# Stardust-lf/fhe-reliability-gpu

Measured on AMD Instinct MI355X. Metric: forward negacyclic NTT/s at N=2^16 (limb-polynomials per second), higher is better.
Workload: dtype f64

## Files before the change

fhe_reliability_gpu_amd/csrc/capi.cpp:

```cpp
#include "capi_internal.hpp"

int build_tables(fhe_ctx *ctx, int log_n, const u64 *q, int count, const u64 *fwd_rows, bool want_inverse, int force_path,
                 const u64 *psi_or_null, fhe_ntt_tables **out, const u64 *gs_scale)
{
    if (!ctx || !q || !out || count < 1 || log_n < 1 || log_n > NTT_MAX_LOGN) return fail(FHE_ERR_INVALID, "bad table arguments");
    const size_t N = (size_t)1 << log_n;
    std::unique_ptr<fhe_ntt_tables> t(new fhe_ntt_tables);
    t->ctx = ctx;
    t->log_n = log_n;
    t->count = count;
    t->q.assign(q, q + count);
    t->psi.assign(count, 0);
    t->path.resize(count);
    t->h_lp.resize(count);
    t->has_inverse = want_inverse;
    std::vector<Tw> tw((size_t)count * 2 * N);
    HIP_TRY(hipSetDevice(ctx->device));
    HIP_TRY(t->d_tw.alloc(tw.size() * sizeof(Tw)));
    std::vector<u64> inv;
    for (int l = 0; l < count; l++) {
        const int path = force_path >= 0 ? force_path : path_for(q[l]);
        if (path < 0 || (path == PATH_F64 && q[l] >= ((u64)1 << 50)) || q[l] >= ((u64)1 << 61) || q[l] < 2)
            return fail(FHE_ERR_UNSUPPORTED, "modulus must satisfy 2 <= q < 2^61 (FP64 path: q < 2^50)");
        t->path[l] = path;
        const u64 *row = fwd_rows + (size_t)l * N;
        Tw *f = tw.data() + (size_t)l * 2 * N, *b = f + N;
        for (size_t k = 0; k < N; k++) f[tw_stored_index(log_n, (u32)k)] = encode(path, row[k] % q[l], q[l]);
        bool inv_ok = false;
        if (gs_scale) {
            const u64 sc = gs_scale[l] % q[l];
            for (size_t k = 1; k < N; k++) b[tw_stored_index(log_n, (u32)k)] = encode(path, row[k] % q[l], q[l]);
            b[tw_stored_index(log_n, 0)] = encode(path, host::mul_mod(sc, row[1 % N] % q[l], q[l]), q[l]);
        } else if (want_inverse) inv_ok = batch_inverse(row, N, q[l], inv);
        if (gs_scale) {
        } else if (inv_ok) {
            inv[0] = host::mul_mod(host::inv_mod((u64)(N % q[l]), q[l]), inv[1 % N], q[l]);
            for (size_t k = 0; k < N; k++) b[tw_stored_index(log_n, (u32)k)] = encode(path, inv[k], q[l]);
        } else {
            for (size_t k = 0; k < N; k++) b[k] = f[k];
            t->has_inverse = false;
        }
        LimbParams &p = t->h_lp[l];
        std::memset(&p, 0, sizeof p);
        p.q = q[l];
        p.two_q = 2 * q[l];
        p.n = (double)q[l];
        p.ninv = 1.0 / p.n;
        const u64 ninv = gs_scale ? gs_scale[l] % q[l] : host::inv_mod((u64)(N % q[l]), q[l]);
        if (!ninv && want_inverse) t->has_inverse = false;
        p.inv_n = encode(path, ninv, q[l]);
        p.fwd = t->d_tw.as<Tw>() + (size_t)l * 2 * N;
        p.inv = p.fwd + N;
        u64 cr[3];
        host::const_ratio(q[l], cr);
        p.barrett_lo = cr[0];
        p.barrett_hi = cr[1];
        p.path = path;
        if (psi_or_null) t->psi[l] = psi_or_null[l];
    }
    HIP_TRY(hipMemcpy(t->d_tw.p, tw.data(), tw.size() * sizeof(Tw), hipMemcpyHostToDevice));
    HIP_TRY(t->d_lp.upload(t->h_lp));
    *out = t.release();
    return FHE_OK;
}

SubBatchCut sub_batch_cut(const fhe_ctx *ctx, int log_n, size_t n_poly, size_t len, size_t bufs)
{
    const size_t unit_bytes = ((size_t)8 << log_n) * bufs, total = n_poly * len * unit_bytes, chunk_bytes = ((size_t)ctx->chunk_mib << 20) * (bufs > 1 ? 2 : 1);
    const size_t floor_bytes = ((size_t)ctx->chunk_floor_mib << 20) * (bufs > 1 ? 3 : 1);
    if (!chunk_bytes || log_n < 13 || n_poly * len < 2 || total <= std::max(chunk_bytes + (chunk_bytes >> 1), floor_bytes)) return SubBatchCut{0, 0};
    const size_t pc = std::min(n_poly, std::max<size_t>(1, chunk_bytes / unit_bytes));
    const size_t lc = std::min(len, std::max<size_t>(1, chunk_bytes / (unit_bytes * pc)));
    if (pc == n_poly && lc == len) return SubBatchCut{0, 0};
    return SubBatchCut{pc, lc};
}
size_t sub_batch_polys(const fhe_ctx *ctx, int log_n, size_t n_poly, size_t len)
{
    const size_t unit_bytes = (size_t)8 << log_n, total = n_poly * len * unit_bytes, chunk_bytes = (size_t)ctx->chunk_mib << 20;
    if (!chunk_bytes || log_n < 13 || n_poly < 2 || total <= std::max(chunk_bytes + (chunk_bytes >> 1), (size_t)ctx->chunk_floor_mib << 20)) return 0;
    const size_t per = std::max<size_t>(1, chunk_bytes / (unit_bytes * len));
    return per < n_poly ? per : 0;
}

hipError_t handoff_scratch(fhe_ctx *ctx, hipStream_t st, size_t bytes, u64 **out)
{
    DevBuf *b;
    {
        std::lock_guard<std::mutex> lock(ctx->mu);
        auto &slot = ctx->pp_tmp[st];
        if (!slot) slot.reset(new DevBuf);
        b = slot.get();
    }
    *out = nullptr;
    if (b->bytes < bytes) {
        hipStreamCaptureStatus cap = hipStreamCaptureStatusNone;
        (void)hipStreamIsCapturing(st, &cap);
        if (cap != hipStreamCaptureStatusNone) return hipSuccess;
        hipError_t e = b->p ? hipStreamSynchronize(st) : hipSuccess;
        if (e == hipSuccess) e = b->alloc(bytes);
        if (e != hipSuccess) return e;
    }
    *out = b->as<u64>();
    return hipSuccess;
}

int side_stream(fhe_ctx *ctx, hipStream_t st, fhe_ctx::Side **out)
{
    *out = nullptr;
    hipStreamCaptureStatus cap = hipStreamCaptureStatusNone;
    if (hipStreamIsCapturing(st, &cap) != hipSuccess || cap != hipStreamCaptureStatusNone) return FHE_OK;
    fhe_ctx::Side *sd;
    {
        std::lock_guard<std::mutex> lock(ctx->mu);
        auto &slot = ctx->side[st];
        if (!slot) slot.reset(new fhe_ctx::Side);
        sd = slot.get();
    }
    if (!sd->s) {
        HIP_TRY(hipStreamCreateWithFlags(&sd->s, hipStreamNonBlocking));
        HIP_TRY(hipEventCreateWithFlags(&sd->fork, hipEventDisableTiming));
        HIP_TRY(hipEventCreateWithFlags(&sd->join, hipEventDisableTiming));
    }
    *out = sd;
    return FHE_OK;
}

int for_pieces(fhe_ctx *ctx, hipStream_t st, size_t n_pieces, size_t side_tmp_bytes, const std::function<hipError_t(hipStream_t, size_t, u64 *)> &fn)
{
    fhe_ctx::Side *sd = nullptr;
    hipStreamCaptureStatus cap = hipStreamCaptureStatusNone;
    if (ctx->split && n_pieces > 1 && hipStreamIsCapturing(st, &cap) == hipSuccess && cap == hipStreamCaptureStatusNone) {
        {
            std::lock_guard<std::mutex> lock(ctx->mu);
            auto &slot = ctx->side[st];
            if (!slot) slot.reset(new fhe_ctx::Side);
            sd = slot.get();
        }
        if (!sd->s) {
            HIP_TRY(hipStreamCreateWithFlags(&sd->s, hipStreamNonBlocking));
            HIP_TRY(hipEventCreateWithFlags(&sd->fork, hipEventDisableTiming));
            HIP_TRY(hipEventCreateWithFlags(&sd->join, hipEventDisableTiming));
        }
        if (sd->tmp.bytes < side_tmp_bytes) {
            HIP_TRY(hipStreamSynchronize(sd->s));
            HIP_TRY(sd->tmp.alloc(side_tmp_bytes));
        }
        HIP_TRY(hipEventRecord(sd->fork, st));
        HIP_TRY(hipStreamWaitEvent(sd->s, sd->fork, 0));
    }
    hipError_t e = hipSuccess;
    for (size_t i = 0; i < n_pieces && e == hipSuccess; ++i) {
        const bool on_side = sd && (i & 1);
        e = fn(on_side ? sd->s : st, i, on_side && side_tmp_bytes ? sd->tmp.as<u64>() : nullptr);
    }
    if (sd) {
        HIP_TRY(hipEventRecord(sd->join, sd->s));
        HIP_TRY(hipStreamWaitEvent(st, sd->join, 0));
    }
    return e == hipSuccess ? FHE_OK : hip_fail(e, "sub-batch launch");
}
int for_sub_batches(fhe_ctx *ctx, hipStream_t st, size_t n_poly, size_t per, size_t side_tmp_bytes,
                    const std::function<hipError_t(hipStream_t, size_t, size_t, u64 *)> &fn)
{
    return for_pieces(ctx, st, (n_poly + per - 1) / per, side_tmp_bytes,
                      [&](hipStream_t s, size_t i, u64 *side_tmp) { return fn(s, i * per, std::min(per, n_poly - i * per), side_tmp); });
}

int ntt_batch(fhe_ctx *ctx, u64 *d, const fhe_ntt_tables *t, size_t n_poly, size_t limbs, size_t start_idx, void *stream,
              bool inverse, const u64 *d_src, u32 galois, u64 *d_galois_copy)
{
    if (!ctx || !d) return fail(FHE_ERR_INVALID, "null argument");
    if (galois) {
        if (!inverse || !d_src || d_src == d || !(galois & 1)) return fail(FHE_ERR_INVALID, "the Galois map rides on an out-of-place inverse transform");
        if (ctx->mode == 1 || ctx->fault_idx >= 0 || ctx->packed_on || ctx->only_pass >= 0 || ctx->resident || t->log_n < 5) {
            HIP_TRY(hipSetDevice(ctx->device));
            u64 *to = d_galois_copy ? d_galois_copy : d;
            hipError_t e = launch_automorphism_ntt(pick(ctx, stream), to, d_src, (u32)(n_poly * limbs), t->log_n, galois);
            if (e != hipSuccess) return hip_fail(e, "launch_automorphism_ntt");
            d_src = d_galois_copy;
            galois = 0;
            d_galois_copy = nullptr;
        }
    }
    if (d_src && (ctx->mode == 1 || ctx->fault_idx >= 0 || ctx->packed_on || ctx->only_pass >= 0 || ctx->resident)) {
        HIP_TRY(hipSetDevice(ctx->device));
        if (d_src != d) HIP_TRY(hipMemcpyAsync(d, d_src, (n_poly * limbs << t->log_n) * 8, hipMemcpyDeviceToDevice, pick(ctx, stream)));
        d_src = nullptr;
    }
    int rc = check_range(t, n_poly, limbs, start_idx);
    if (rc) return rc;
    if (inverse && !t->has_inverse) return fail(FHE_ERR_UNSUPPORTED, "table set has no inverse (twiddle or N not invertible)");
    if (!n_poly || !limbs) return FHE_OK;
    HIP_TRY(hipSetDevice(ctx->device));
    hipStream_t st = pick(ctx, stream);
    const size_t N = (size_t)1 << t->log_n;
    TraceScope tr(ctx, st, "NTT");
    return for_each_run(t, limbs, start_idx, [&](size_t off, size_t len, int path) -> int {
        PassArgs a{d + off * N, t->d_lp.as<LimbParams>(), (u32)(start_idx + off), (u32)len, (u32)(n_poly * len), (u32)limbs};
        if (d_src) a.src = d_src + off * N;
        a.galois = galois;
        if (d_galois_copy) a.galois_copy = d_galois_copy + off * N;
        hipError_t e;
        if (ctx->mode == 1 && fused_supported(t->log_n)) {
            DevBuf *ctl;
            {
                std::lock_guard<std::mutex> lock(ctx->mu);
                auto &slot = ctx->fused_ctl[st];
                if (!slot) slot.reset(new DevBuf);
                ctl = slot.get();
            }
            const size_t need = fused_ctl_bytes(a.units);
            if (ctl->bytes < need) {
                HIP_TRY(hipStreamSynchronize(st));
                u32 carried = 0;
                if (ctl->p) HIP_TRY(hipMemcpy(&carried, ctl->as<u32>() + fused_error_word(), sizeof carried, hipMemcpyDeviceToHost));
                HIP_TRY(ctl->alloc(need * 2));
                HIP_TRY(hipMemset(ctl->p, 0, need * 2));
                if (carried) HIP_TRY(hipMemcpy(ctl->as<u32>() + fused_error_word(), &carried, sizeof carried, hipMemcpyHostToDevice));
            }
            e = launch_ntt_fused(st, a, t->log_n, inverse, path, ctl->as<u32>(), ctx->fused_dist, ctx->fused_wgs, ctx->fused_variant, ctx->fused_skip_teams);
        } else if (ctx->fault_idx >= 0 && t->log_n >= 13) {
            e = launch_ntt(st, a, t->log_n, inverse, path, ctx->geo, 0);
            if (e == hipSuccess) e = launch_flip_bit(st, d, (u64)ctx->fault_idx, ctx->fault_bit);
            if (e == hipSuccess) e = launch_ntt(st, a, t->log_n, inverse, path, ctx->geo, 1);
            ctx->fault_idx = -1;
        } else {
            if (ctx->packed_on && ctx->only_pass < 0 && ctx->geo == 1 && ntt_packed_supported(t->log_n, inverse, path)) {
                DevBuf *sc;
                {
                    std::lock_guard<std::mutex> lock(ctx->mu);
                    auto &slot = ctx->packed[st];
                    if (!slot) slot.reset(new DevBuf);
                    sc = slot.get();
                }
                const size_t need = (size_t)a.units * ntt_packed_scratch_words() * 8;
                if (sc->bytes < need) {
                    HIP_TRY(hipStreamSynchronize(st));
                    HIP_TRY(sc->alloc(need));
                }
                a.scratch = sc->as<u64>();
            }
            const bool plain = t->log_n >= 13 && ctx->only_pass < 0 && !a.scratch;
            const SubBatchCut cut = plain ? sub_batch_cut(ctx, t->log_n, n_poly, len) : SubBatchCut{0, 0};
            u64 *pp = nullptr;
            const bool want_pp = !galois && (ctx->pingpong < 0 ? cut.pc != 0 : ctx->pingpong != 0);
            const size_t pp_bytes = (cut.pc ? cut.pc * cut.lc : n_poly * limbs) * N * 8;
            if (want_pp && plain) HIP_TRY(handoff_scratch(ctx, st, pp_bytes, &pp));
            if (cut.pc) {
                const size_t npp = (n_poly + cut.pc - 1) / cut.pc, npl = (len + cut.lc - 1) / cut.lc;
                return for_pieces(ctx, st, npp * npl, pp ? pp_bytes : 0, [&](hipStream_t s, size_t i, u64 *side_tmp) {
                    const size_t l0 = (i / npp) * cut.lc, p0 = (i % npp) * cut.pc;
                    const size_t lc = std::min(cut.lc, len - l0), pc = std::min(cut.pc, n_poly - p0);
                    PassArgs c = a;
                    c.data = a.data + (p0 * limbs + l0) * N;
                    if (a.src) c.src = a.src + (p0 * limbs + l0) * N;
                    if (a.galois_copy) c.galois_copy = a.galois_copy + (p0 * limbs + l0) * N;
                    c.limb0 = a.limb0 + (u32)l0;
                    c.limbs = (u32)lc;
                    c.units = (u32)(pc * lc);
                    c.tmp = side_tmp ? side_tmp : pp;
                    c.tmp_stride = (u32)lc;
                    c.stream_hint = ctx->stream_hint != 0;
                    return launch_ntt(s, c, t->log_n, inverse, path, ctx->geo, -1, false);
                });
            } else {
                a.tmp = pp ? pp + off * N : nullptr;
                const bool streams = t->log_n < 13 && t->log_n >= 5 && ctx->stream_hint < 0 && ctx->only_pass < 0 &&
                                     (size_t)a.units * N * 8 > ((size_t)ctx->chunk_floor_mib << 20);
                a.stream_hint = ctx->stream_hint > 0 || streams;
                e = launch_ntt(st, a, t->log_n, inverse, path, ctx->geo, ctx->only_pass, ctx->resident);
            }
        }
        if (e != hipSuccess) return hip_fail(e, "launch_ntt");
        return FHE_OK;
    });
}

int pointwise(fhe_ctx *ctx, u64 *c, const u64 *a, const u64 *b, const fhe_ntt_tables *t, size_t n_poly, size_t limbs,
              size_t start_idx, void *stream, bool acc)
{
    if (!ctx || !c || !a || !b) return fail(FHE_ERR_INVALID, "null argument");
    int rc = check_range(t, n_poly, limbs, start_idx);
    if (rc) return rc;
    HIP_TRY(hipSetDevice(ctx->device));
    PointwiseArgs p{c, a, b, t->d_lp.as<LimbParams>(), (u32)start_idx, (u32)limbs, (u32)(n_poly * limbs), (u32)limbs, t->log_n};
    hipError_t e = launch_modmul(pick(ctx, stream), p, acc);
    if (e != hipSuccess) return hip_fail(e, "launch_modmul");
    return FHE_OK;
}

int cyclic_tables(fhe_ctx *ctx, int log_n, u64 mod, u64 root, int convention, u64 scale, fhe_ntt_tables **out)
{
    std::lock_guard<std::mutex> lock(ctx->mu);
    auto key = std::make_tuple(log_n, mod, root, convention * 2 + 1, scale);
    auto it = ctx->cyclic.find(key);
    if (it == ctx->cyclic.end()) {
        const u64 n = (u64)1 << log_n;
        std::vector<u64> tw(n);
        host::cyclic_table(mod, log_n, root, convention == 1, tw.data());
        fhe_ntt_tables *nt = nullptr;
        int rc = build_tables(ctx, log_n, &mod, 1, tw.data(), false, -1, nullptr, &nt, &scale);
        if (rc) return rc;
        it = ctx->cyclic.emplace(key, std::unique_ptr<fhe_ntt_tables>(nt)).first;
    }
    *out = it->second.get();
    return FHE_OK;
}

static bool cyclic_tower(u64 mod, int log_n, u64 root, bool nth_root_convention)
{
    const u64 n = (u64)1 << log_n;
    u64 prev = 0;
    for (int s = 0; s < log_n; s++) {
        const u64 len = (u64)2 << s;
        const u64 w = nth_root_convention ? host::pow_mod(root, n / len, mod) : host::pow_mod(root, (mod - 1) / len, mod);
        if (s == 0 ? w != (mod - 1) % mod : host::mul_mod(w, w, mod) != prev) return false;
        prev = w;
    }
    return true;
}
static bool cyclic_tower_cached(fhe_ctx *ctx, u64 mod, int log_n, u64 root, int convention)
{
    std::lock_guard<std::mutex> lock(ctx->mu);
    const auto key = std::make_tuple(log_n, mod, root, convention);
    auto it = ctx->cyclic_tower.find(key);
    if (it == ctx->cyclic_tower.end()) it = ctx->cyclic_tower.emplace(key, cyclic_tower(mod, log_n, root, convention == 1)).first;
    return it->second;
}

static int cyclic_small(fhe_ctx *ctx, u64 *d_data, u64 *d_scratch, int log_n, size_t n_vec, u64 mod, u64 root, int convention, u64 scale, bool do_scale,
                        void *stream)
{
    fhe_ntt_tables *t = nullptr;
    {
        std::lock_guard<std::mutex> lock(ctx->mu);
        auto key = std::make_tuple(log_n, mod, root, convention * 2, (u64)0);
        auto it = ctx->cyclic.find(key);
        if (it == ctx->cyclic.end()) {
            std::vector<u64> tw((size_t)1 << log_n);
            host::cyclic_table(mod, log_n, root, convention == 1, tw.data());
            fhe_ntt_tables *nt = nullptr;
            int rc = build_tables(ctx, log_n, &mod, 1, tw.data(), false, -1, nullptr, &nt);
            if (rc) return rc;
            it = ctx->cyclic.emplace(key, std::unique_ptr<fhe_ntt_tables>(nt)).first;
        }
        t = it->second.get();
    }
    HIP_TRY(hipSetDevice(ctx->device));
    hipStream_t st = pick(ctx, stream);
    PassArgs a{d_data, t->d_lp.as<LimbParams>(), 0u, 1u, (u32)n_vec, 1u};
    hipError_t e = launch_ntt(st, a, log_n, false, t->path[0]);
    if (e != hipSuccess) return hip_fail(e, "launch_ntt(cyclic)");
    e = launch_bitrev_scale(st, d_scratch, d_data, log_n, (u32)n_vec, mod_const(mod), scale, do_scale);
    if (e != hipSuccess) return hip_fail(e, "launch_bitrev_scale");
    HIP_TRY(hipMemcpyAsync(d_data, d_scratch, (n_vec << log_n) * sizeof(u64), hipMemcpyDeviceToDevice, st));
    return FHE_OK;
}

extern "C" {

int fhe_version(void) { return 100; }
const char *fhe_last_error(void) { return g_err.c_str(); }

int fhe_ctx_create(int device, fhe_ctx **out)
{
    if (!out) return fail(FHE_ERR_INVALID, "null out");
    int n = 0;
    HIP_TRY(hipGetDeviceCount(&n));
    if (device < 0 || device >= n) return fail(FHE_ERR_INVALID, "no such HIP device");
    HIP_TRY(hipSetDevice(device));
    std::unique_ptr<fhe_ctx> c(new fhe_ctx);
    c->device = device;
    HIP_TRY(hipStreamCreateWithFlags(&c->stream, hipStreamNonBlocking));
    if (const char *m = getenv("FHE_NTT_MODE")) c->mode = std::strcmp(m, "fused") == 0 ? 1 : 0;
    if (const char *v = getenv("FHE_FUSED_DIST")) c->fused_dist = (unsigned)std::max(1, atoi(v));
    if (const char *v = getenv("FHE_FUSED_WGS")) c->fused_wgs = (unsigned)std::max(1, atoi(v));
    if (const char *v = getenv("FHE_NTT_RESIDENT")) c->resident = atoi(v) != 0;
    if (const char *v = getenv("FHE_NTT_PACKED")) c->packed_on = atoi(v) != 0;
    if (const char *v = getenv("FHE_NTT_PINGPONG")) c->pingpong = atoi(v) < 0 ? -1 : atoi(v) ? 1 : 0;
    if (const char *v = getenv("FHE_NTT_SPLIT")) c->split = atoi(v) < 0 ? -1 : atoi(v) ? 1 : 0;
    if (const char *v = getenv("FHE_NTT_CHUNK_MIB")) c->chunk_mib = (unsigned)std::max(0, atoi(v));
    if (const char *v = getenv("FHE_KS_FUSED")) c->ks_fused = atoi(v) < 0 ? -1 : atoi(v) ? 1 : 0;
    if (const char *v = getenv("FHE_HMULT_FUSED_RESCALE")) c->hmult_fused_rescale = atoi(v) != 0;
    *out = c.release();
    return FHE_OK;
}

int fhe_ctx_destroy(fhe_ctx *ctx)
{
    if (!ctx) return FHE_OK;
    (void)hipSetDevice(ctx->device);
    (void)hipStreamSynchronize(ctx->stream);
    ctx->cyclic.clear();
    ctx->garner.clear();
    ctx->fused_ctl.clear();
    ctx->packed.clear();
    ctx->pp_tmp.clear();
    for (auto &kv : ctx->side)
        if (kv.second && kv.second->s) {
            (void)hipStreamSynchronize(kv.second->s);
            (void)hipEventDestroy(kv.second->fork);
            (void)hipEventDestroy(kv.second->join);
            (void)hipStreamDestroy(kv.second->s);
        }
    ctx->side.clear();
    (void)hipStreamDestroy(ctx->stream);
    delete ctx;
    return FHE_OK;
}

int fhe_ctx_set_option(fhe_ctx *ctx, const char *name, long value)
{
    if (!ctx || !name) return fail(FHE_ERR_INVALID, "null argument");
    if (!std::strcmp(name, "ntt_mode")) ctx->mode = value ? 1 : 0;
    else if (!std::strcmp(name, "fused_dist")) ctx->fused_dist = (unsigned)std::max(1l, value);
    else if (!std::strcmp(name, "fused_wgs")) ctx->fused_wgs = (unsigned)std::max(1l, value);
    else if (!std::strcmp(name, "fused_variant")) ctx->fused_variant = (int)value;
    else if (!std::strcmp(name, "tile_geo")) ctx->geo = value ? 1 : 0;
    else if (!std::strcmp(name, "ntt_resident")) ctx->resident = value != 0;
    else if (!std::strcmp(name, "ntt_packed")) ctx->packed_on = value != 0;
    else if (!std::strcmp(name, "ntt_stream")) ctx->stream_hint = value < 0 ? -1 : value ? 1 : 0;
    else if (!std::strcmp(name, "ntt_chunk_floor_mib")) ctx->chunk_floor_mib = (unsigned)std::max(0l, value);
    else if (!std::strcmp(name, "ntt_split")) ctx->split = value < 0 ? -1 : value ? 1 : 0;
    else if (!std::strcmp(name, "ntt_pingpong")) ctx->pingpong = value < 0 ? -1 : value ? 1 : 0;
    else if (!std::strcmp(name, "ntt_chunk_mib")) ctx->chunk_mib = (unsigned)std::max(0l, value);
    else if (!std::strcmp(name, "ks_fused")) ctx->ks_fused = value < 0 ? -1 : value ? 1 : 0;
    else if (!std::strcmp(name, "hmult_fused_rescale")) ctx->hmult_fused_rescale = value != 0;
    else if (!std::strcmp(name, "ntt_only_pass")) ctx->only_pass = value == 0 ? 0 : value == 1 ? 1 : -1;
    else if (!std::strcmp(name, "fused_skip_teams")) ctx->fused_skip_teams = (unsigned)value;
    else return fail(FHE_ERR_INVALID, "unknown option");
    return FHE_OK;
}

int fhe_ctx_check(fhe_ctx *ctx)
{
    if (!ctx) return fail(FHE_ERR_INVALID, "null ctx");
    HIP_TRY(hipSetDevice(ctx->device));
    std::lock_guard<std::mutex> lock(ctx->mu);
    for (auto &kv : ctx->fused_ctl) {
        if (!kv.second || !kv.second->p) continue;
        HIP_TRY(hipStreamSynchronize(kv.first));
        u32 flag = 0;
        HIP_TRY(hipMemcpy(&flag, kv.second->as<u32>() + fused_error_word(), sizeof flag, hipMemcpyDeviceToHost));
        if (flag) {
            HIP_TRY(hipMemset(kv.second->as<u32>() + fused_error_word(), 0, sizeof flag));
            return fail(FHE_ERR_HIP, "fused NTT: a bounded wait ran out in a launch since the last check (its results are invalid)");
        }
    }
    return FHE_OK;
}

int fhe_ctx_stream(fhe_ctx *ctx, void **stream_out)
{
    if (!ctx || !stream_out) return fail(FHE_ERR_INVALID, "null argument");
    *stream_out = ctx->stream;
    return FHE_OK;
}

int fhe_sync(fhe_ctx *ctx, void *stream)
{
    if (!ctx) return fail(FHE_ERR_INVALID, "null ctx");
    HIP_TRY(hipSetDevice(ctx->device));
    HIP_TRY(hipStreamSynchronize(pick(ctx, stream)));
    return FHE_OK;
}

int fhe_alloc(fhe_ctx *ctx, size_t bytes, void **dptr)
{
    if (!ctx || !dptr) return fail(FHE_ERR_INVALID, "null argument");
    HIP_TRY(hipSetDevice(ctx->device));
    hipError_t e = hipMalloc(dptr, bytes ? bytes : 16);
    if (e == hipErrorOutOfMemory) return fail(FHE_ERR_NOMEM, "hipMalloc: out of device memory");
    if (e != hipSuccess) return hip_fail(e, "hipMalloc");
    return FHE_OK;
}

int fhe_free(fhe_ctx *ctx, void *dptr)
{
    if (!ctx) return fail(FHE_ERR_INVALID, "null ctx");
    if (!dptr) return FHE_OK;
    HIP_TRY(hipSetDevice(ctx->device));
    HIP_TRY(hipFree(dptr));
    return FHE_OK;
}

int fhe_h2d(fhe_ctx *ctx, void *dst, const void *src, size_t bytes, void *stream)
{
    if (!ctx || (!dst && bytes) || (!src && bytes)) return fail(FHE_ERR_INVALID, "null argument");
    HIP_TRY(hipSetDevice(ctx->device));
    HIP_TRY(hipMemcpyAsync(dst, src, bytes, hipMemcpyHostToDevice, pick(ctx, stream)));
    return FHE_OK;
}
int fhe_d2h(fhe_ctx *ctx, void *dst, const void *src, size_t bytes, void *stream)
{
    if (!ctx || (!dst && bytes) || (!src && bytes)) return fail(FHE_ERR_INVALID, "null argument");
    HIP_TRY(hipSetDevice(ctx->device));
    HIP_TRY(hipMemcpyAsync(dst, src, bytes, hipMemcpyDeviceToHost, pick(ctx, stream)));
    return FHE_OK;
}
int fhe_d2d(fhe_ctx *ctx, void *dst, const void *src, size_t bytes, void *stream)
{
    if (!ctx || (!dst && bytes) || (!src && bytes)) return fail(FHE_ERR_INVALID, "null argument");
    HIP_TRY(hipSetDevice(ctx->device));
    HIP_TRY(hipMemcpyAsync(dst, src, bytes, hipMemcpyDeviceToDevice, pick(ctx, stream)));
    return FHE_OK;
}
int fhe_memset(fhe_ctx *ctx, void *dst, int byte, size_t bytes, void *stream)
{
    if (!ctx || (!dst && bytes)) return fail(FHE_ERR_INVALID, "null argument");
    HIP_TRY(hipSetDevice(ctx->device));
    HIP_TRY(hipMemsetAsync(dst, byte, bytes, pick(ctx, stream)));
    return FHE_OK;
}

int fhe_moduli_create(uint64_t N, const int *bits, int count, uint64_t *out_q)
{
    if (!bits || !out_q || count < 1 || N < 1 || (N & (N - 1)) || N > ((u64)1 << 59)) return fail(FHE_ERR_INVALID, "bad arguments");
    for (int i = 0; i < count; i++)
        if (bits[i] < 2 || bits[i] > 61) return fail(FHE_ERR_UNSUPPORTED, "bit sizes must be in [2, 61]");
    if (!host::create_moduli(N, bits, count, out_q)) return fail(FHE_ERR_INVALID, "not enough primes of the requested size");
    return FHE_OK;
}

int fhe_modulus_const_ratio(uint64_t q, uint64_t out[3])
{
    if (q < 2 || !out) return fail(FHE_ERR_INVALID, "bad arguments");
    host::const_ratio(q, out);
    return FHE_OK;
}

int fhe_min_primitive_root(uint64_t q, uint64_t order, uint64_t *out)
{
    if (!out) return fail(FHE_ERR_INVALID, "null out");
    if (order > ((u64)1 << 31)) return fail(FHE_ERR_UNSUPPORTED, "order above 2^31");
    if (!host::min_primitive_root(q, order, *out)) return fail(FHE_ERR_INVALID, "no primitive root of that order");
    return FHE_OK;
}

int fhe_root_powers(uint64_t q, int log_n, uint64_t *rp, uint64_t *rp_shoup)
{
    if (log_n < 1 || log_n > 30 || q < 2) return fail(FHE_ERR_INVALID, "bad arguments");
    u64 psi;
    if (!host::min_primitive_root(q, (u64)2 << log_n, psi)) return fail(FHE_ERR_INVALID, "q is not 1 mod 2N (or not prime)");
    const size_t N = (size_t)1 << log_n;
    std::vector<u64> t(N);
    host::root_powers(q, log_n, psi, t.data());
    for (size_t k = 0; k < N; k++) {
        if (rp) rp[k] = t[k];
        if (rp_shoup) rp_shoup[k] = (u64)(((unsigned __int128)t[k] << 64) / q);
    }
    return FHE_OK;
}

int fhe_ntt_tables_create(fhe_ctx *ctx, int log_n, const uint64_t *q, int count, fhe_ntt_tables **out)
{
    if (!ctx || !q || !out || count < 1 || log_n < 1 || log_n > NTT_MAX_LOGN) return fail(FHE_ERR_INVALID, "bad table arguments");
    const size_t N = (size_t)1 << log_n;
    std::vector<u64> rows((size_t)count * N), psi(count);
    for (int l = 0; l < count; l++) {
        if (q[l] < 2 || q[l] >= ((u64)1 << 61)) return fail(FHE_ERR_UNSUPPORTED, "modulus " + std::to_string(q[l]) + " outside [2, 2^61)");
        if (!host::min_primitive_root(q[l], (u64)2 * N, psi[l]))
            return fail(FHE_ERR_INVALID, "modulus " + std::to_string(q[l]) + " has no primitive 2N-th root");
        host::root_powers(q[l], log_n, psi[l], rows.data() + (size_t)l * N);
    }
    return build_tables(ctx, log_n, q, count, rows.data(), true, -1, psi.data(), out);
}

int fhe_ntt_tables_create_from_roots(fhe_ctx *ctx, int log_n, const uint64_t *q, int count, const uint64_t *root_powers,
                                     int force_path, fhe_ntt_tables **out)
{
    if (!root_powers) return fail(FHE_ERR_INVALID, "null root powers");
    if (force_path < -1 || force_path > 1) return fail(FHE_ERR_INVALID, "bad force_path");
    std::vector<u64> psi(count > 0 ? count : 0);
    if (log_n >= 1 && count >= 1)
        for (int l = 0; l < count; l++) psi[l] = root_powers[((size_t)l << log_n) + ((size_t)1 << (log_n - 1))];
    return build_tables(ctx, log_n, q, count, root_powers, true, force_path, psi.data(), out);
}
// ... 327 lines not shown
```

fhe_reliability_gpu_amd/csrc/capi_internal.hpp:

```cpp
#pragma once
#include "../../include/fhe_mi355x.h"

#include <hip/hip_runtime.h>

#include <algorithm>
#include <chrono>
#include <cstdio>
#include <cstdlib>
#include <cstring>
#include <functional>
#include <map>
#include <memory>
#include <mutex>
#include <string>
#include <tuple>
#include <vector>

#include "host_math.hpp"
#include "ntt_fused.hpp"
#include "ntt_launch.hpp"

using namespace fhe;



inline thread_local std::string g_err;

inline int fail(int code, const std::string &msg)
{
    g_err = msg;
    return code;
}
inline int hip_fail(hipError_t e, const char *what)
{
    g_err = std::string(what) + ": " + hipGetErrorString(e);
    return FHE_ERR_HIP;
}
#define HIP_TRY(expr)                                          \
    do {                                                       \
        hipError_t e_ = (expr);                                \
        if (e_ != hipSuccess) return hip_fail(e_, #expr);      \
    } while (0)

struct DevBuf {
    void *p = nullptr;
    size_t bytes = 0;
    ~DevBuf()
    {
        if (p) (void)hipFree(p);
    }
    hipError_t alloc(size_t n)
    {
        if (p) (void)hipFree(p);
        p = nullptr;
        bytes = n;
        return hipMalloc(&p, n ? n : 16);
    }
    template <class T> hipError_t upload(const std::vector<T> &v)
    {
        hipError_t e = alloc(v.size() * sizeof(T));
        if (e != hipSuccess) return e;
        return hipMemcpy(p, v.data(), v.size() * sizeof(T), hipMemcpyHostToDevice);
    }
    template <class T> T *as() const { return static_cast<T *>(p); }
};

struct fhe_ntt_tables {
    fhe_ctx *ctx = nullptr;
    int log_n = 0, count = 0;
    std::vector<u64> q, psi;
    std::vector<int> path;
    std::vector<LimbParams> h_lp;
    DevBuf d_lp, d_tw;
    bool has_inverse = true;
};

struct fhe_baseconv {
    int m = 0, k = 0;
    bool fast_ok = true;
    DevBuf mod_in, mod_out, dig, hor, fp_in, fp_out, fast_coef, fast_shoup, img_head, img_out, rows_id;
    DevBuf chk_dig, chk_hor;
    const fhe::Tw *shoup_dig = nullptr, *shoup_hor = nullptr;
    BaseConvPlanDev dev{};
};

struct GarnerTables {
    DevBuf mod, ratio, pref_lo, pref_hi, inv_pref;
};

struct fhe_ctx {
    int device = 0;
    hipStream_t stream = nullptr;
    std::mutex mu;
    std::map<hipStream_t, std::unique_ptr<DevBuf>> fused_ctl;
    std::map<hipStream_t, std::unique_ptr<DevBuf>> packed;
    bool packed_on = false;
    int mode = 0;
    unsigned fused_dist = 4, fused_wgs = 768;
    bool hmult_fused_rescale = true;
    unsigned fused_skip_teams = 0;
    bool trace_on = false;
    std::string trace;
    long long fault_idx = -1;
    int fault_bit = 0;
    int pfault_pass = -1, pfault_bit = 0;
    u32 pfault_block = 0, pfault_word = 0;
    PointHook pm_fault, pw_fault, bc_fault, gal_fault;
    StagedFault ksc_fault, rsc_fault, hrc_fault, bsgs_fault, bgv_ksc_fault, bgv_rsc_fault;
    PointHook seal_fault;
    PointHook carry_fault;
    int carry_skip = 0;
    DevBuf seal_part;
    DevBuf gal_sums;
    int geo = 1;
    bool resident = false;
    int pingpong = -1;
    std::map<hipStream_t, std::unique_ptr<DevBuf>> pp_tmp;
    struct Side { hipStream_t s = nullptr; hipEvent_t fork = nullptr, join = nullptr; DevBuf tmp; };
    std::map<hipStream_t, std::unique_ptr<Side>> side;
    int split = -1;
    int stream_hint = -1;
    unsigned chunk_floor_mib = 192;
    unsigned chunk_mib = 96;
    int ks_fused = -1;
    int only_pass = -1;
    int fused_variant = 7;
    std::map<std::tuple<int, u64, u64, int, u64>, std::unique_ptr<fhe_ntt_tables>> cyclic;
    std::map<std::tuple<int, u64, u64, int>, bool> cyclic_tower;
    std::map<std::vector<u64>, std::unique_ptr<GarnerTables>> garner;
};

struct fhe_abft {
    fhe_ctx *ctx = nullptr;
    const fhe_ntt_tables *t = nullptr;
    DevBuf w, what, ninv;
    DevBuf win, wout, wout8;
    DevBuf sum_in, sum_out;
    DevBuf umid, umid8;
    DevBuf sum_mid1, sum_mid2;
    DevBuf psum;
};

struct KsShard {
    int world = 1, rank = 0, clo = 0, cn = 0, slo = 0, sn = 0, cmax = 0, smax = 0;
};
void ks_shard_layout(int L, int K, int world, int rank, KsShard *s);

struct fhe_keyswitch {
    fhe_ctx *ctx = nullptr;
    const fhe_ntt_tables *t = nullptr;
    int L = 0, K = 0, dnum = 0, alpha = 0, log_n = 0;
    KsShard sh;
    bool sharded = false;
    int m_own = 0;
    u64 *g1 = nullptr, *g2 = nullptr;
    DevBuf up_rows, down_rows;
    bool up_f64 = false;
    bool own_path[2] = {false, false};
    bool up_trivial = false;
    u32 down_src_row = 0, down_src_stride = 0;
    DevBuf d_t_mod_Q;
    u32 n_up_jobs = 0;
    std::vector<BcJob> up_host;
    u64 plain_modulus = 0;
    std::vector<u64> t_inv_P, t_mod_Q;
    std::vector<fhe_baseconv *> up;
    fhe_baseconv *down = nullptr;
    DevBuf pinv;
    DevBuf coef, ext, acc, conv, rot;
    DevBuf up_jobs, down_jobs;
    int up_max_m = 0, up_max_k = 0;
    u32 up_m_mask = 0;
    bool up_batched = false;
    DevBuf ext_map[2];
    u32 ext_units[2] = {0, 0};
    fhe_baseconv *last = nullptr;
    int rs_n = 0;
    bool own_last = false;
    u64 *rs_bc = nullptr;
    DevBuf qlast_inv;
    DevBuf rs_last, rs_delta, rs_jobs;
    DevBuf hm, hm_pre;
    DevBuf pq_tw;
    DevBuf bsgs;
    DevBuf acc2, conv2, hsp2, hdown_jobs2;
    int cur = 0;
    DevBuf acc_multi;
    u64 *acc_ovr = nullptr;
    u64 *acc_cur() const { return acc_ovr ? acc_ovr : (cur ? acc2 : acc).as<u64>(); }
    u64 *conv_cur() const { return (cur ? conv2 : conv).as<u64>(); }
    u64 *hsp_cur() const { return (cur ? hsp2 : hsp).as<u64>(); }
    DevBuf hsp, hdown_rows, hdown_jobs;
    u64 t_inv_qlast = 0;
    DevBuf chk_bc_flags, chk_bc_map, chk_sum_in, chk_sum_out;
    ~fhe_keyswitch()
    {
        for (auto *b : up) fhe_baseconv_destroy(b);
        fhe_baseconv_destroy(down);
        fhe_baseconv_destroy(last);
    }
};

struct fhe_fourstep {
    fhe_ctx *ctx = nullptr;
    u64 n1 = 0, n2 = 0, mod = 0, g = 0;
    int log_n = 0;
    fhe_ntt_tables *t = nullptr;
    DevBuf tmp;
    bool big = false;
    int log1 = 0, log2 = 0, lo_bits = 0;
    DevBuf tw_lo, tw_hi, buf0, buf1;
    struct Checked {
        DevBuf u8, m8, v8, eu, em, ev, sums[4];
        std::unique_ptr<fhe_ntt_tables> small;
    };
    std::unique_ptr<Checked> chk;
    bool checked_ready = false;
};



inline hipStream_t pick(fhe_ctx *ctx, void *stream) { return stream ? static_cast<hipStream_t>(stream) : ctx->stream; }

inline int path_for(u64 q)
{
    if (q < 2) return -1;
    if (q < ((u64)1 << 50)) return PATH_F64;
    if (q < ((u64)1 << 61)) return PATH_U64;
    return -1;
}

inline Tw encode(int path, u64 w, u64 q) { return path == PATH_F64 ? ArithF64::encode(w, q) : ArithU64::encode(w, q); }

inline bool batch_inverse(const u64 *t, size_t n, u64 q, std::vector<u64> &out)
{
    out.assign(n, 0);
    if (n < 2) return true;
    std::vector<u64> pre(n);
    u64 acc = 1 % q;
    for (size_t i = 1; i < n; i++) {
        pre[i] = acc;
        acc = host::mul_mod(acc, t[i] % q, q);
    }
    u64 inv = host::inv_mod(acc, q);
    if (!inv && q != 1) return false;
    for (size_t i = n - 1; i >= 1; i--) {
        out[i] = host::mul_mod(inv, pre[i], q);
        inv = host::mul_mod(inv, t[i] % q, q);
    }
    return true;
}



template <class F> int for_each_run(const fhe_ntt_tables *t, size_t limbs, size_t start_idx, F f)
{
    size_t i = 0;
    while (i < limbs) {
        size_t j = i + 1;
        while (j < limbs && t->path[start_idx + j] == t->path[start_idx + i]) j++;
        int rc = f(i, j - i, t->path[start_idx + i]);
        if (rc != FHE_OK) return rc;
        i = j;
    }
    return FHE_OK;
}

struct TraceScope {
    fhe_ctx *ctx;
    hipStream_t st;
// ... 81 lines not shown
```

fhe_reliability_gpu_amd/csrc/fourstep_checked.hip:

```cpp
#include "ntt_launch.hpp"
#include "ntt_plan.hpp"
#include "abft_taps.hpp"

namespace fhe {

template <class PASS>
FHE_D void gs_lds_fault(const GsCheckArgs &g, int pass, typename PASS::elem *lds)
{
    if (g.fault_pass == pass && g.fault_block == blockIdx.x) {
        if (threadIdx.x == 0) reinterpret_cast<u64 *>(lds)[g.fault_word % (u32)PASS::LDS_ELEMS] ^= (u64)1 << g.fault_bit;
        __syncthreads();
    }
}

template <class PASS, int LOGN, bool WA, bool WB>
__global__ __launch_bounds__(NTT_THREADS) void k_gs_first_checked(PassArgs a, GsCheckArgs g)
{
    typedef typename PASS::Arith A;
    typedef GsTap<A, 0, PASS::P, PASS::S0, WA, WB> Tap;
    static_assert(PASS::NPHASE >= 3, "a staging phase and at least two register steps");
    __shared__ __attribute__((aligned(16))) typename PASS::elem lds[PASS::LDS_ELEMS];
    __shared__ u64 red[2][NTT_THREADS / 64];
    const u32 unit = blockIdx.x / PASS::TILES, tile = blockIdx.x % PASS::TILES;
    const size_t off = (size_t)unit << LOGN;
    const LimbParams &p = a.lp[a.limb0];
    const typename A::Ctx ctx = A::make_ctx(p);
    const TwPtr tw = as_global(p.inv);
    const Tw inv_n = p.inv_n;
    const int tid = threadIdx.x;
    const u32 row0 = tile * PASS::TROWS;
    u64 *base = a.data + off;
    const u64 *from = a.src + off;
    Tap tap{as_global(g.u), as_global(g.m), as_global(g.v), (const u64 FHE_GLOBAL *)g.u8, (const u64 FHE_GLOBAL *)g.m8, row0, g.logp,
            typename A::elem(0), typename A::elem(0), 0, 0};
    PASS::template phase<0>(tid, base, lds, tw, row0, ctx, inv_n, &tap, from, 0u, nullptr, a.stream_hint != 0);
    __syncthreads();
    PASS::template phase<1>(tid, base, lds, tw, row0, ctx, inv_n, &tap);
    __syncthreads();
    gs_lds_fault<PASS>(g, 0, lds);
    PASS::template phase<2>(tid, base, lds, tw, row0, ctx, inv_n, &tap);
    if constexpr (PASS::NPHASE > 3) {
        __syncthreads();
        PASS::template phase<3>(tid, base, lds, tw, row0, ctx, inv_n, &tap);
    }
    if constexpr (WA) block_sum_mod(A::canonical(tap.acc_a, ctx), p.q, g.sum_a + (size_t)unit * PASS::TILES + tile, red[0]);
    if constexpr (WB) block_sum_mod(A::canonical(tap.acc_b, ctx), p.q, g.sum_b + (size_t)unit * PASS::TILES + tile, red[1]);
}

template <class PASS, int LOGN, int P, bool WA, bool WB>
__global__ __launch_bounds__(NTT_THREADS) void k_gs_second_checked(PassArgs a, GsCheckArgs g)
{
    typedef typename PASS::Arith A;
    typedef GsTap<A, 1, P, LOGN - P, WA, WB> Tap;
    static_assert(PASS::NPHASE == 2 || PASS::NPHASE == 3, "two or three register steps");
    __shared__ __attribute__((aligned(16))) typename PASS::elem lds[PASS::LDS_ELEMS];
    __shared__ u64 red[2][NTT_THREADS / 64];
    u32 limb;
    u64 *base = col_tile<PASS, LOGN>(blockIdx.x, a, limb);
    const u32 unit = blockIdx.x / PASS::TILES, tile = blockIdx.x % PASS::TILES;
    const u32 pos0 = (u32)((base - a.data) & (((size_t)1 << LOGN) - 1));
    const LimbParams &p = a.lp[limb];
    const typename A::Ctx ctx = A::make_ctx(p);
    const TwPtr tw = as_global(p.inv);
    const Tw inv_n = p.inv_n;
    const int tid = threadIdx.x;
    const u64 *from = a.src + (base - a.data);
    Tap tap{as_global(g.u), as_global(g.m), as_global(g.v), (const u64 FHE_GLOBAL *)g.u8, (const u64 FHE_GLOBAL *)g.m8, pos0, g.logp,
            typename A::elem(0), typename A::elem(0), 0, 0};
    PASS::template phase<0>(tid, base, lds, tw, 0u, ctx, inv_n, &tap, from);
    __syncthreads();
    gs_lds_fault<PASS>(g, 1, lds);
    PASS::template phase<1>(tid, base, lds, tw, 0u, ctx, inv_n, &tap);
    if constexpr (PASS::NPHASE > 2) {
        __syncthreads();
        PASS::template phase<2>(tid, base, lds, tw, 0u, ctx, inv_n, &tap);
    }
    if constexpr (WA) block_sum_mod(A::canonical(tap.acc_a, ctx), p.q, g.sum_a + (size_t)unit * PASS::TILES + tile, red[0]);
    if constexpr (WB) block_sum_mod(A::canonical(tap.acc_b, ctx), p.q, g.sum_b + (size_t)unit * PASS::TILES + tile, red[1]);
}

template <class A, int LOGN>
static hipError_t launch_gs_checked_t(hipStream_t st, const PassArgs &a, u64 *tmp, const GsCheckArgs &c1, const GsCheckArgs &c2, bool phases, int which)
{
    typedef GsPasses<A, LOGN> GP;
    typedef typename GP::First First;
    const dim3 g1(a.units * First::TILES), th(NTT_THREADS);
    if constexpr (!GP::TWO) {
        if (which == 1) return hipSuccess;
        hipLaunchKernelGGL((k_gs_first_checked<First, LOGN, true, true>), g1, th, 0, st, a, c1);
        return hipGetLastError();
    } else {
        if (!tmp) return hipErrorInvalidValue;
        constexpr int P = First::P;
        typedef typename GP::Second Col;
        typedef typename GP::SecondNt ColNt;
        PassArgs first = a, second = a;
        first.data = tmp;
        second.src = tmp;
        const dim3 g2(a.units * Col::TILES);
        if (which != 1) {
            if (phases) hipLaunchKernelGGL((k_gs_first_checked<First, LOGN, true, true>), g1, th, 0, st, first, c1);
            else hipLaunchKernelGGL((k_gs_first_checked<First, LOGN, true, false>), g1, th, 0, st, first, c1);
        }
        if (which != 0) {
            if (a.stream_hint) {
                if (phases) hipLaunchKernelGGL((k_gs_second_checked<ColNt, LOGN, P, true, true>), g2, th, 0, st, second, c2);
                else hipLaunchKernelGGL((k_gs_second_checked<ColNt, LOGN, P, false, true>), g2, th, 0, st, second, c2);
            } else {
                if (phases) hipLaunchKernelGGL((k_gs_second_checked<Col, LOGN, P, true, true>), g2, th, 0, st, second, c2);
                else hipLaunchKernelGGL((k_gs_second_checked<Col, LOGN, P, false, true>), g2, th, 0, st, second, c2);
            }
        }
        return hipGetLastError();
    }
}

template <int LOGN> static void gs_checked_tiles_t(u32 *t1, u32 *t2)
{
    typedef GsPasses<ArithF64, LOGN> GP;
    *t1 = GP::First::TILES;
    if constexpr (GP::TWO) *t2 = GP::Second::TILES;
    else *t2 = 1;
}

void ntt_gs_checked_tiles(int logn, u32 *t1, u32 *t2)
{
    *t1 = *t2 = 1;
    switch (logn) {
#define FHE_CASE(L) case L: gs_checked_tiles_t<L>(t1, t2); break;
        FHE_CASE(5) FHE_CASE(6) FHE_CASE(7) FHE_CASE(8) FHE_CASE(9) FHE_CASE(10) FHE_CASE(11) FHE_CASE(12) FHE_CASE(13)
        FHE_CASE(14) FHE_CASE(15) FHE_CASE(16) FHE_CASE(17) FHE_CASE(18) FHE_CASE(19) FHE_CASE(20)
#undef FHE_CASE
    default: break;
    }
}

hipError_t launch_ntt_gs_checked(hipStream_t st, const PassArgs &a, u64 *tmp, const GsCheckArgs &c1, const GsCheckArgs &c2, int logn, int path,
                                 bool phases, int which)
{
    if (a.units == 0) return hipSuccess;
    if (!a.src || a.map || a.limbs != 1 || !ntt_gs_supported(logn) || (phases && logn < 13)) return hipErrorInvalidValue;
    switch (logn) {
#define FHE_CASE(L) \
    case L: return path == PATH_F64 ? launch_gs_checked_t<ArithF64, L>(st, a, tmp, c1, c2, phases, which) : launch_gs_checked_t<ArithU64, L>(st, a, tmp, c1, c2, phases, which);
        FHE_CASE(5) FHE_CASE(6) FHE_CASE(7) FHE_CASE(8) FHE_CASE(9) FHE_CASE(10) FHE_CASE(11) FHE_CASE(12) FHE_CASE(13)
        FHE_CASE(14) FHE_CASE(15) FHE_CASE(16) FHE_CASE(17) FHE_CASE(18) FHE_CASE(19) FHE_CASE(20)
#undef FHE_CASE
    default: return hipErrorInvalidValue;
    }
}

}
```

fhe_reliability_gpu_amd/csrc/ntt_core.hpp:

```cpp
#pragma once
#include "modarith.hpp"

namespace fhe {

FHE_HD u32 brev_bits(u32 v, int bits)
{
    if (bits <= 0) return 0;
#if defined(__clang__)
    return __builtin_bitreverse32(v) >> (32 - bits);
#else
    u32 r = 0;
    for (int b = 0; b < bits; b++) r |= ((v >> b) & 1u) << (bits - 1 - b);
    return r;
#endif
}

FHE_HD constexpr int cmax(int a, int b) { return a > b ? a : b; }
FHE_HD constexpr int cmin(int a, int b) { return a < b ? a : b; }

FHE_HD constexpr u32 reduce_mask(int stage0, int nstages, int first, int next)
{
    u32 mask = 0;
    for (int u = 0; u < nstages; u++) {
        int s = stage0 + u;
// ... 82 lines not shown
{
    constexpr int R = 1 << K;
    InvLazyPlan<K> p{};
    int b[R] = {};
    for (int r = 0; r < R; r++) b[r] = in8 * 128;
    const int limit = INV_LAZY_LIMIT8 * 128, folded = 513;
    for (int v = 0; v < K; v++) {
        const int u = K - 1 - v, half = R >> (u + 1);
        u32 m = 0;
        for (int blk = 0; blk < (1 << u); blk++)
            for (int j = 0; j < half; j++) {
                const int i0 = blk * 2 * half + j, i1 = i0 + half;
                if (b[i0] + b[i1] > limit) {
                    const int big = b[i0] >= b[i1] ? i0 : i1;
                    b[big] = folded;
                    m |= 1u << big;
                    if (b[i0] + b[i1] > limit) {
                        const int other = big == i0 ? i1 : i0;
                        b[other] = folded;
                        m |= 1u << other;
                    }
                }
                const int sum = b[i0] + b[i1], prod = 513 + (sum + 3) / 4;
                b[i0] = (fold_last && u == 0) ? prod : sum;
                b[i1] = prod;
            }
        p.before[v] = m;
    }
    int mx = 0;
    for (int r = 0; r < R; r++) {
        if (b[r] > exit8 * 128) {
            b[r] = folded;
            p.at_exit |= 1u << r;
        }
        mx = b[r] > mx ? b[r] : mx;
    }
    p.out8 = (mx + 127) / 128;
    return p;
}
template <class ST> FHE_HD constexpr int inv_lazy_step_in8(int in8, int se)
{
    int b = in8;
    for (int i = 0; i < se; i++) {
        const int k = ST::k(ST::NSTEP - 1 - i);
        b = k == 1 ? inv_lazy_plan<1>(b, INV_LAZY_EXIT8, false).out8 : k == 2 ? inv_lazy_plan<2>(b, INV_LAZY_EXIT8, false).out8
          : k == 3 ? inv_lazy_plan<3>(b, INV_LAZY_EXIT8, false).out8 : k == 4 ? inv_lazy_plan<4>(b, INV_LAZY_EXIT8, false).out8
                                                                             : inv_lazy_plan<5>(b, INV_LAZY_EXIT8, false).out8;
    }
    return b;
}
template <class ST> FHE_HD constexpr int inv_lazy_pass_out8(int in8) { return inv_lazy_step_in8<ST>(in8, ST::NSTEP); }

template <class A, int K, int SBLK, bool FOLD, int IN8, int EXIT8>
FHE_D void radix_inv_lazy(typename A::elem (&x)[1 << K], TwPtr tw, int s, u32 prefix, const typename A::Ctx &c, const Tw *inv_n)
{
    constexpr int R = 1 << K;
    constexpr InvLazyPlan<K> plan = inv_lazy_plan<K>(IN8, EXIT8, FOLD);
#pragma unroll
    for (int v = 0; v < K; v++) {
        const int u = K - 1 - v;
#pragma unroll
        for (int r = 0; r < R; r++)
            if ((plan.before[v] >> r) & 1) A::reduce(x[r], c);
        const int half = R >> (u + 1);
        if (FOLD && u == 0) {
            const Tw wn = tw[0];
#pragma unroll
            for (int j = 0; j < half; j++) A::bfly_inv_scaled(x[j], x[j + half], *inv_n, wn, c);
            continue;
        }
#pragma unroll
        for (int b = 0; b < (1 << u); b++) {
            const Tw w = tw[tw_index(SBLK, s + u, (prefix << u) + b)];
#pragma unroll
            for (int j = 0; j < half; j++) A::bfly_inv(x[b * 2 * half + j], x[b * 2 * half + j + half], w, c);
        }
    }
#pragma unroll
    for (int r = 0; r < R; r++)
        if ((plan.at_exit >> r) & 1) A::reduce(x[r], c);
}

template <int K0_, int K1_, int K2_>
struct Steps {
    static constexpr int K0 = K0_, K1 = K1_, K2 = K2_;
    static constexpr int P = K0_ + K1_ + K2_;
    static constexpr int NSTEP = (K0_ > 0) + (K1_ > 0) + (K2_ > 0);
    static constexpr int KMAX = cmax(K0_, cmax(K1_, K2_));
    FHE_HD static constexpr int k(int e) { return e == 0 ? K0_ : e == 1 ? K1_ : K2_; }
    FHE_HD static constexpr int done(int e) { return e == 0 ? 0 : e == 1 ? K0_ : K0_ + K1_; }
};

enum IoMode { IO_CANONICAL = 0, IO_LAZY = 1 };

template <class A, int R, int IN_MODE>
FHE_D void convert_in(typename A::elem (&x)[R], u64 (&raw)[R], const typename A::Ctx &c)
{
    if (IN_MODE == IO_LAZY) {
#pragma unroll
        for (int r = 0; r < R; r++) x[r] = A::load_lazy(raw[r]);
    } else {
        bool bad = false;
#pragma unroll
        for (int r = 0; r < R; r++) bad |= !A::in_range(raw[r], c);
        if (__builtin_expect(bad, 0)) {
#pragma unroll
            for (int r = 0; r < R; r++) raw[r] = A::in_range(raw[r], c) ? raw[r] : reduce_any_u64(raw[r], c.q);
        }
#pragma unroll
        for (int r = 0; r < R; r++) x[r] = A::from_canonical(raw[r]);
    }
}

template <class A, int OUT_MODE, bool INVERSE, bool SCALED = false>
FHE_D u64 convert_out(typename A::elem x, const typename A::Ctx &c, const Tw &inv_n)
{
    if (OUT_MODE == IO_LAZY) return A::store_lazy(x);
    if (INVERSE && !SCALED) return A::canonical(A::mulmod(x, inv_n, c), c);
    return A::canonical(x, c);
}

constexpr int PK_BITS = 50;
constexpr int PK_WORDS = 13;
constexpr int PK_BLOCK_WORDS = 16 * PK_WORDS;
constexpr u64 PK_MASK = ((u64)1 << PK_BITS) - 1;

FHE_HD void pk_pack(const u64 (&v)[16], u64 (&w)[PK_WORDS])
{
#pragma unroll
    for (int j = 0; j < PK_WORDS; j++) w[j] = 0;
#pragma unroll
    for (int k = 0; k < 16; k++) {
        const int j = (PK_BITS * k) >> 6, t = (PK_BITS * k) & 63;
        w[j] |= v[k] << t;
        if (t > 64 - PK_BITS) w[j + 1] |= v[k] >> (64 - t);
    }
}
template <class P> FHE_HD u64 pk_extract(P w, u32 idx)
{
    const u32 bit = PK_BITS * idx, j = bit >> 6, t = bit & 63;
    const u64 lo = w[j], hi = w[j + 1 < PK_WORDS ? j + 1 : j];
    const u64 v = t > 64 - PK_BITS ? (lo >> t) | (hi << (64 - t)) : lo >> t;
    return v & PK_MASK;
}

template <class T, class = void> struct tap_preloads { static constexpr bool value = false; };
template <class T> struct tap_preloads<T, decltype((void)T::PRELOAD)> { static constexpr bool value = T::PRELOAD; };
struct NoTap {
    static constexpr bool ACTIVE = false;
    static constexpr bool MID = false;
    static constexpr bool STORES = false;
};

template <class A, class ST, int LOGN, int S0, int TC, int NTHREADS, bool INVERSE, int IN_MODE, int OUT_MODE, u32 RED,
          int SBLK, int COHERENT_IN = 0, bool STREAM = false>
struct ColPass {
    typedef A Arith;
    typedef typename A::elem elem;
    static constexpr int THREADS = NTHREADS;
    static constexpr int P = ST::P;
    static constexpr int NPTS = 1 << P;
    static constexpr int LOGSTRIDE = LOGN - S0 - P;
    static constexpr u32 STRIDE = 1u << LOGSTRIDE;
    static constexpr int PADC = (TC < 32 && (NPTS * TC + ((NPTS + 15) / 16) * TC) * 8 <= 65536) ? TC : 0;
    static constexpr int LDS_ELEMS = NPTS * TC + ((NPTS + 15) / 16) * PADC;
    static constexpr int TCOLS = TC;
    static constexpr int NSTEP = ST::NSTEP;
    static constexpr int NPHASE = ST::NSTEP;
    static constexpr int TILES = (1 << (LOGN - P)) / TC;

    static FHE_HD u32 lidx(u32 g, u32 col) { return g * TC + col + (g >> 4) * PADC; }

    template <int E, class TAP = NoTap>
    static FHE_D void phase(int tid, u64 *__restrict__ base, elem *__restrict__ lds, TwPtr tw, u32 hi_prefix,
                            const typename A::Ctx &c, const Tw &inv_n, TAP *tap = nullptr, const u64 *src = nullptr)
    {
        constexpr int F = INVERSE ? ST::NSTEP - 1 - E : E;
        constexpr int K = ST::k(F);
        constexpr int R = 1 << K;
        constexpr int DONE = ST::done(F);
        constexpr int LOGS = P - DONE - K;
        constexpr u32 S = 1u << LOGS;
        constexpr int NSETS = NPTS / R;
        constexpr bool FIRST = E == 0, LAST = E == ST::NSTEP - 1;
        constexpr int U0 = INVERSE ? (P - DONE - K) : DONE;
        FHE_ASSUME(tid >= 0 && tid < NTHREADS);
#pragma unroll 1
        for (int u = tid; u < NSETS * TC; u += NTHREADS) {
            const u32 col = (u32)u % TC, su = (u32)u / TC;
            const u32 a = DONE == 0 ? 0u : su >> LOGS, cc = DONE == 0 ? su : su & (S - 1);
            const u32 g0 = ((a << K) << LOGS) + cc;
            elem x[R];
            if (FIRST) {
                u64 raw[R];
                const u64 *ldb = src ? src : base;
#pragma unroll
                for (int r = 0; r < R; r++) {
                    const u64 *from = ldb + (size_t)(g0 + ((u32)r << LOGS)) * STRIDE + col;
                    raw[r] = COHERENT_IN == 1 ? load_coherent_u64(from) : (COHERENT_IN == 2 || (STREAM && IN_MODE == IO_CANONICAL)) ? load_stream_u64(from) : *from;
                }
                if constexpr (tap_preloads<TAP>::value) {
                    u64 extra[R];
#pragma unroll
                    for (int r = 0; r < R; r++) extra[r] = tap->load((g0 + ((u32)r << LOGS)) * STRIDE + col);
                    convert_in<A, R, IN_MODE>(x, raw, c);
                    tap->prepare(extra, c);
#pragma unroll
                    for (int r = 0; r < R; r++) tap->apply(x[r], extra[r], c);
                } else {
                    convert_in<A, R, IN_MODE>(x, raw, c);
                    if constexpr (TAP::ACTIVE) {
#pragma unroll
                        for (int r = 0; r < R; r++) tap->in((g0 + ((u32)r << LOGS)) * STRIDE + col, x[r], c);
                    }
                }
            } else {
#pragma unroll
                for (int r = 0; r < R; r++) x[r] = lds[lidx(g0 + ((u32)r << LOGS), col)];
            }
            const u32 prefix = (hi_prefix << DONE) | a;
            constexpr bool FOLD = INVERSE && LAST && OUT_MODE == IO_CANONICAL && S0 + DONE == 0;
            if constexpr (INVERSE && (RED & INV_LAZY) != 0 && A::PATH == PATH_F64) {
                constexpr int IN8 = inv_lazy_step_in8<ST>((int)(RED & 0xFFu), E);
                constexpr int EX8 = (LAST && OUT_MODE == IO_CANONICAL) ? INV_LAZY_LIMIT8 : INV_LAZY_EXIT8;
                radix_inv_lazy<A, K, SBLK, FOLD, IN8, EX8>(x, tw, S0 + DONE, prefix, c, &inv_n);
            } else if (INVERSE) radix_inv<A, K, RED, U0, SBLK, FOLD>(x, tw, S0 + DONE, prefix, c, &inv_n);
            else radix_fwd<A, K, RED, U0, SBLK>(x, tw, S0 + DONE, prefix, c);
            if (LAST) {
                if constexpr (TAP::ACTIVE) {
                    if constexpr (TAP::MID) {
#pragma unroll
                        for (int r = 0; r < R; r++) tap->mid((g0 + ((u32)r << LOGS)) * STRIDE + col, x[r], c);
                    }
                }
#pragma unroll
                for (int r = 0; r < R; r++) {
                    u64 *dst = base + (size_t)(g0 + ((u32)r << LOGS)) * STRIDE + col;
                    const u64 out = convert_out<A, OUT_MODE, INVERSE, FOLD>(x[r], c, inv_n);
                    if constexpr (TAP::ACTIVE && !TAP::STORES && OUT_MODE == IO_CANONICAL) tap->out((g0 + ((u32)r << LOGS)) * STRIDE + col, out, c);
                    if (STREAM && OUT_MODE == IO_CANONICAL) store_stream_u64(dst, out);
                    else *dst = out;
                }
            } else {
#pragma unroll
                for (int r = 0; r < R; r++) lds[lidx(g0 + ((u32)r << LOGS), col)] = x[r];
            }
        }
    }
    static constexpr bool PACKABLE = !INVERSE && A::PATH == PATH_F64 && TC == 16 && NTHREADS == 256 && NPTS == 256 && ST::NSTEP == 2 &&
                                     ST::k(1) == 4 && PK_BLOCK_WORDS * 16 <= LDS_ELEMS;
    static FHE_D void phase_last_packed(int tid, elem *__restrict__ lds, TwPtr tw, u32 hi_prefix, const typename A::Ctx &c, u64 (&chunk)[PK_WORDS])
    {
        constexpr int F = ST::NSTEP - 1, K = ST::k(F), R = 1 << K, DONE = ST::done(F);
        static_assert(R == 16 && P - DONE - K == 0, "one thread = 16 consecutive points of one column");
        const u32 col = (u32)tid % TC, a = (u32)tid / TC, g0 = a << K;
        elem x[R];
#pragma unroll
        for (int r = 0; r < R; r++) x[r] = lds[lidx(g0 + (u32)r, col)];
        radix_fwd<A, K, RED, DONE, SBLK>(x, tw, S0 + DONE, (hi_prefix << DONE) | a, c);
        u64 v[R];
#pragma unroll
        for (int r = 0; r < R; r++) v[r] = A::canonical(x[r], c);
        pk_pack(v, chunk);
    }
    static FHE_D void pack_stage(int tid, u64 *__restrict__ stage, const u64 (&chunk)[PK_WORDS])
    {
        u64 *dst = stage + (size_t)tid * PK_WORDS;
#pragma unroll
        for (int j = 0; j < PK_WORDS; j++) dst[j] = chunk[j];
    }
    static FHE_D void pack_copy_out(int tid, const u64 *__restrict__ stage, u64 *__restrict__ tile_scratch)
    {
        for (int i = tid; i < 16 * PK_BLOCK_WORDS / 2; i += NTHREADS) {
            tile_scratch[2 * i] = stage[2 * i];
            tile_scratch[2 * i + 1] = stage[2 * i + 1];
        }
    }
};

FHE_HD u32 galois_slot(u32 j, int logn, u32 k)
{
    const u32 e = 2 * brev_bits(j, logn) + 1;
    const u32 e2 = (u32)(((u64)e * k) & ((2ull << logn) - 1ull));
    return brev_bits((e2 - 1) >> 1, logn);
}

FHE_HD constexpr u32 row_pad(u32 g) { return g + ((g >> 4) << 1); }

template <class A, class ST, int LOGN, int TR, int NTHREADS, bool INVERSE, int IN_MODE, int OUT_MODE, u32 RED,
          int SBLK, int COHERENT_IN = 0, bool STREAM = false, bool STAGE_BOTH = false, int ROWMODE = 0>
struct RowPass {
    typedef A Arith;
    typedef typename A::elem elem;
    static constexpr int THREADS = NTHREADS;
    static constexpr int P = ST::P;
    static constexpr int NPTS = 1 << P;
    static constexpr int S0 = LOGN - P;
    static constexpr int ROW_LDS = NPTS + 2 * ((NPTS + 15) / 16);
    static constexpr int LDS_ELEMS = ROW_LDS * TR;
    static constexpr int TROWS = TR;
    static constexpr int NSTEP = ST::NSTEP;
    static constexpr bool STAGED = NPTS >= 32;
    static constexpr bool STAGE_IN = STAGED && (INVERSE || STAGE_BOTH), STAGE_OUT = STAGED && (!INVERSE || STAGE_BOTH);
    static constexpr int NPHASE = ST::NSTEP + (STAGE_IN ? 1 : 0) + (STAGE_OUT ? 1 : 0);
    static constexpr int TILES = (1 << S0) / TR;
    static_assert(ROWMODE == 0 || (INVERSE && NPTS >= 32), "the gathering first launch belongs to the inverse-structured network");

    static FHE_HD u32 net_row(u32 row0, u32 row)
    {
        if (ROWMODE == 0) return row0 + row;
        return brev_bits(row0 + row, S0);
    }
    static FHE_D void gather_in(int tid, const u64 *__restrict__ src, u32 row0, elem *__restrict__ lds, bool nt_src)
    {
#pragma unroll 8
        for (int i = tid; i < TR * NPTS; i += NTHREADS) {
            const u32 ki = (u32)i % TR, rho = (u32)i / TR;
            const u32 k = brev_bits(rho, P);
            const u64 *from = src + ((size_t)rho << S0) + row0 + ki;
            const u64 v = nt_src ? load_stream_u64(from) : *from;
            lds[ki * ROW_LDS + row_pad(k)] = __builtin_bit_cast(elem, v);
        }
    }

    static FHE_D void copy_in(int tid, const u64 *__restrict__ base, elem *__restrict__ lds)
    {
#pragma unroll 2
        for (int i = tid; i < TR * NPTS / 2; i += NTHREADS) {
            const u32 row = (u32)i / (NPTS / 2), g = ((u32)i % (NPTS / 2)) * 2;
            const u64 *src = base + (size_t)row * NPTS + g;
            u64 v0, v1;
            if (COHERENT_IN == 1) {
                v0 = load_coherent_u64(src);
                v1 = load_coherent_u64(src + 1);
            } else if (COHERENT_IN == 2 || (STREAM && IN_MODE == IO_CANONICAL)) {
                v0 = load_stream_u64(src);
                v1 = load_stream_u64(src + 1);
            } else {
                v0 = src[0];
                v1 = src[1];
            }
            elem *dst = lds + row * ROW_LDS + row_pad(g);
            dst[0] = __builtin_bit_cast(elem, v0);
            dst[1] = __builtin_bit_cast(elem, v1);
        }
    }
    static FHE_D void copy_in_galois(int tid, const u64 *__restrict__ src_limb, u32 row0, elem *__restrict__ lds, u32 k, u64 *__restrict__ copy)
    {
#pragma unroll 8
        for (int i = tid; i < TR * NPTS; i += NTHREADS) {
            const u32 row = (u32)i / NPTS, g = (u32)i % NPTS;
            const u64 v = src_limb[galois_slot((row0 + row) * NPTS + g, LOGN, k)];
            lds[row * ROW_LDS + row_pad(g)] = __builtin_bit_cast(elem, v);
            if (copy) copy[i] = v;
        }
    }
    template <class TAP = NoTap>
    static FHE_D void copy_out(int tid, u64 *__restrict__ base, const elem *__restrict__ lds, const typename A::Ctx &c, TAP *tap = nullptr)
    {
#pragma unroll 2
        for (int i = tid; i < TR * NPTS / 2; i += NTHREADS) {
            const u32 row = (u32)i / (NPTS / 2), g = ((u32)i % (NPTS / 2)) * 2;
            const elem *src = lds + row * ROW_LDS + row_pad(g);
            u64 *dst = base + (size_t)row * NPTS + g;
            if constexpr (TAP::ACTIVE) {
                if constexpr (TAP::STORES) {
                    tap->store(row * NPTS + g, __builtin_bit_cast(u64, src[0]), __builtin_bit_cast(u64, src[1]));
                    continue;
                } else {
                    tap->out(row * NPTS + g, __builtin_bit_cast(u64, src[0]), c);
                    tap->out(row * NPTS + g + 1, __builtin_bit_cast(u64, src[1]), c);
                }
            }
            if (STREAM && OUT_MODE == IO_CANONICAL) {
                store_stream_u64(dst, __builtin_bit_cast(u64, src[0]));
                store_stream_u64(dst + 1, __builtin_bit_cast(u64, src[1]));
            } else {
                dst[0] = __builtin_bit_cast(u64, src[0]);
                dst[1] = __builtin_bit_cast(u64, src[1]);
            }
        }
    }

    template <int E, class TAP = NoTap, class TWS = TwPtr>
    static FHE_D void phase(int tid, u64 *__restrict__ base, elem *__restrict__ lds, const TWS &tw, u32 row0,
                            const typename A::Ctx &c, const Tw &inv_n, TAP *tap = nullptr, const u64 *src = nullptr, u32 galois = 0,
                            u64 *galois_copy = nullptr, bool nt_src = false)
    {
        if constexpr (STAGE_IN && E == 0) {
            if constexpr (ROWMODE == 1) gather_in(tid, src, row0, lds, nt_src);
            else if (galois && src) copy_in_galois(tid, src - (size_t)row0 * NPTS, row0, lds, galois, galois_copy);
            else copy_in(tid, src ? src : base, lds);
        } else if constexpr (STAGE_OUT && E == NPHASE - 1) {
            copy_out<TAP>(tid, base, lds, c, tap);
        } else {
            constexpr int SE = STAGE_IN ? E - 1 : E;
            constexpr int F = INVERSE ? ST::NSTEP - 1 - SE : SE;
            constexpr int K = ST::k(F);
            constexpr int R = 1 << K;
            constexpr int DONE = ST::done(F);
            constexpr int LOGS = P - DONE - K;
            constexpr u32 S = 1u << LOGS;
            constexpr int NSETS = NPTS / R;
            constexpr bool FIRST = SE == 0, LAST = SE == ST::NSTEP - 1;
            constexpr bool FROM_GLOBAL = FIRST && !STAGE_IN;
            constexpr bool TO_GLOBAL = LAST && !STAGE_OUT;
            constexpr int U0 = INVERSE ? (P - DONE - K) : DONE;
            FHE_ASSUME(tid >= 0 && tid < NTHREADS);
#pragma unroll 1
            for (int u = tid; u < NSETS * TR; u += NTHREADS) {
                const u32 row = (u32)u / NSETS, su = (u32)u % NSETS;
                const u32 a = su >> LOGS, cc = su & (S - 1);
                const u32 g0 = ((a << K) << LOGS) + cc;
                u64 *__restrict__ grow = base + (size_t)(ROWMODE == 1 ? net_row(row0, row) : row) * NPTS;
                elem *__restrict__ lrow = lds + row * ROW_LDS;
                elem x[R];
                if (FIRST) {
                    u64 raw[R];
#pragma unroll
                    for (int r = 0; r < R; r++) {
                        if (FROM_GLOBAL) {
                            const u64 *from = (src ? src + (size_t)row * NPTS : grow) + g0 + ((u32)r << LOGS);
                            raw[r] = COHERENT_IN == 1 ? load_coherent_u64(from) : (COHERENT_IN == 2 || (STREAM && IN_MODE == IO_CANONICAL)) ? load_stream_u64(from) : *from;
                        } else {
                            raw[r] = __builtin_bit_cast(u64, lrow[row_pad(g0 + ((u32)r << LOGS))]);
                        }
                    }
                    convert_in<A, R, IN_MODE>(x, raw, c);
                    if constexpr (TAP::ACTIVE && (FROM_GLOBAL || STAGE_IN)) {
#pragma unroll
                        for (int r = 0; r < R; r++) tap->in(row * NPTS + g0 + ((u32)r << LOGS), x[r], c);
                    }
                } else {
#pragma unroll
                    for (int r = 0; r < R; r++) x[r] = lrow[row_pad(g0 + ((u32)r << LOGS))];
                }
                const u32 prefix = (net_row(row0, row) << DONE) | a;
                constexpr bool FOLD = INVERSE && LAST && OUT_MODE == IO_CANONICAL && S0 + DONE == 0;
                if constexpr (INVERSE && (RED & INV_LAZY) != 0 && A::PATH == PATH_F64) {
                    constexpr int IN8 = inv_lazy_step_in8<ST>((int)(RED & 0xFFu), SE);
                    constexpr int EX8 = (LAST && OUT_MODE == IO_CANONICAL) ? INV_LAZY_LIMIT8 : INV_LAZY_EXIT8;
                    radix_inv_lazy<A, K, SBLK, FOLD, IN8, EX8>(x, tw, S0 + DONE, prefix, c, &inv_n);
                } else if constexpr (INVERSE) radix_inv<A, K, RED, U0, SBLK, FOLD>(x, tw, S0 + DONE, prefix, c, &inv_n);
                else radix_fwd<A, K, RED, U0, SBLK>(x, tw, S0 + DONE, prefix, c);
                if (LAST) {
                    if constexpr (TAP::ACTIVE && TAP::MID) {
                        if constexpr (TO_GLOBAL && OUT_MODE == IO_LAZY) {
#pragma unroll
                            for (int r = 0; r < R; r++) tap->mid(row * NPTS + g0 + ((u32)r << LOGS), x[r], c);
                        }
                    }
#pragma unroll
                    for (int r = 0; r < R; r++) {
                        const u64 out = convert_out<A, OUT_MODE, INVERSE, FOLD>(x[r], c, inv_n);
                        if (TO_GLOBAL) {
                            if constexpr (TAP::ACTIVE && !TAP::STORES && OUT_MODE == IO_CANONICAL) tap->out(row * NPTS + g0 + ((u32)r << LOGS), out, c);
                            if (STREAM && OUT_MODE == IO_CANONICAL) store_stream_u64(grow + g0 + ((u32)r << LOGS), out);
                            else grow[g0 + ((u32)r << LOGS)] = out;
                        }
                        else lrow[row_pad(g0 + ((u32)r << LOGS))] = __builtin_bit_cast(elem, out);
                    }
                } else {
#pragma unroll
                    for (int r = 0; r < R; r++) lrow[row_pad(g0 + ((u32)r << LOGS))] = x[r];
                }
            }
        }
    }
    static constexpr bool PACKABLE = !INVERSE && A::PATH == PATH_F64 && TR == 16 && NTHREADS == 256 && NPTS == 256 && ST::NSTEP == 2 &&
                                     ST::k(0) == 4 && PK_BLOCK_WORDS * 16 <= LDS_ELEMS;
    static FHE_D void unpack_copy_in(int tid, u64 *__restrict__ stage, const u64 *__restrict__ unit_scratch, u32 P_)
    {
        for (int i = tid; i < 16 * PK_BLOCK_WORDS / 2; i += NTHREADS) {
            const u32 C = (u32)i / (PK_BLOCK_WORDS / 2), o = (u32)i % (PK_BLOCK_WORDS / 2);
            const u64 *src = unit_scratch + ((size_t)C * 16 + P_) * PK_BLOCK_WORDS + 2 * o;
            stage[2 * i] = src[0];
            stage[2 * i + 1] = src[1];
        }
    }
    static FHE_D void phase_first_packed(int tid, const u64 *__restrict__ stage, TwPtr tw, u32 row0, const typename A::Ctx &c, elem (&x)[16])
    {
        constexpr int K = ST::k(0), LOGS = P - K;
        static_assert(K == 4 && LOGS == 4, "one thread = 16 points 16 apart");
        const u32 row = (u32)tid / 16, cc = (u32)tid % 16;
#pragma unroll
        for (int r = 0; r < 16; r++) x[r] = A::from_canonical(pk_extract(stage + ((size_t)r * 16 + cc) * PK_WORDS, row));
        radix_fwd<A, K, RED, 0, SBLK>(x, tw, S0, row0 + row, c);
    }
    static FHE_D void phase_first_store(int tid, elem *__restrict__ lds, const elem (&x)[16])
    {
        const u32 row = (u32)tid / 16, cc = (u32)tid % 16;
        elem *__restrict__ lrow = lds + row * ROW_LDS;
#pragma unroll
        for (int r = 0; r < 16; r++) lrow[row_pad(cc + ((u32)r << 4))] = x[r];
    }
};

}
```

fhe_reliability_gpu_amd/csrc/ntt_fused.hip:

```cpp
#include "ntt_fused.hpp"
#include "ntt_launch.hpp"

namespace fhe {

__device__ __forceinline__ u32 ld_ctl(const u32 *p) { return __hip_atomic_load(p, __ATOMIC_RELAXED, __HIP_MEMORY_SCOPE_AGENT); }
__device__ __forceinline__ void st_ctl(u32 *p, u32 v) { __hip_atomic_store(p, v, __ATOMIC_RELAXED, __HIP_MEMORY_SCOPE_AGENT); }
__device__ __forceinline__ u32 add_ctl(u32 *p, u32 v) { return __hip_atomic_fetch_add(p, v, __ATOMIC_RELAXED, __HIP_MEMORY_SCOPE_AGENT); }

#ifndef FUSED_WAVES_PER_SIMD
#define FUSED_WAVES_PER_SIMD 3
#endif
constexpr u32 FUSED_SPIN_LIMIT = 1u << 22;

template <class PASS, int LOGN, bool INV, bool IS_COL>
__device__ __forceinline__ void run_tile(const PassArgs &a, u32 unit, u32 tile, typename PASS::elem *lds)
{
    typedef typename PASS::Arith A;
    u32 limb, row0 = 0;
    u64 *base;
    if constexpr (IS_COL) base = col_tile_of<PASS, LOGN>(unit, tile, a, limb);
    else base = row_tile_of<PASS, LOGN>(unit, tile, a, limb, row0);
    const LimbParams &p = a.lp[limb];
    const typename A::Ctx ctx = A::make_ctx(p);
    const TwPtr tw = as_global(INV ? p.inv : p.fwd);
// ... 41 lines not shown
    u32 *ctl = f.ctl;
    u32 *err = ctl + fused_error_word();
    u32 *ticket = ctl + fused_ticket_word(xcc);
    u32 *done = ctl + fused_base() + xcc * f.maxg;
    u32 *fin = ctl + fused_base() + FUSED_TEAMS * f.maxg;
    const u32 units = f.pa.units;
    const u32 my_limbs = fused_team_limbs(units, xcc);
    const u32 last_group = my_limbs + f.dist;
    constexpr u32 NONE = 0xFFFFFFFFu;

    u32 t_next = 0;
    if (threadIdx.x == 0) t_next = add_ctl(ticket, 1u);

    for (;;) {
        if (threadIdx.x == 0) {
            const u32 t = t_next;
            const FusedTicket k = fused_decode(t, FP::T1, FP::T2, f.dist);
            u32 unit = NONE, stop = 0;
            if (k.group >= last_group) {
                stop = 1;
            } else {
                if (k.phase != 0 && k.slot < my_limbs) {
                    unit = xcc + FUSED_TEAMS * k.slot;
                    if (k.phase == 2) {
                        bool ready = false;
                        for (u32 i = 0; i < FUSED_SPIN_LIMIT && !ready; i++) {
                            ready = ld_ctl(done + k.slot) == FP::T1;
                            if (!ready) __builtin_amdgcn_s_sleep(2);
                        }
                        if (!ready) {
                            st_ctl(err, 1u);
                            stop = 1;
                        }
                    }
                }
                t_next = add_ctl(ticket, 1u);
            }
            sh[0] = (u32)k.phase;
            sh[1] = unit;
            sh[2] = k.tile;
            sh[3] = stop;
            sh[4] = k.slot;
        }
        __syncthreads();
        const u32 phase = __builtin_amdgcn_readfirstlane(sh[0]), unit = __builtin_amdgcn_readfirstlane(sh[1]),
                  tile = __builtin_amdgcn_readfirstlane(sh[2]), stop = __builtin_amdgcn_readfirstlane(sh[3]),
                  slot = __builtin_amdgcn_readfirstlane(sh[4]);
        if (stop) break;
        if (unit != NONE) {
            if (phase == 1) {
                first_pass_tile<FP, LOGN, INV>(f.pa, unit, tile, lds);
                asm volatile("s_waitcnt vmcnt(0)" ::: "memory");
                __syncthreads();
                if (threadIdx.x == 0) add_ctl(done + slot, 1u);
            } else {
                if constexpr (HANDOFF == HANDOFF_ACQUIRE) {
                    __builtin_amdgcn_fence(__ATOMIC_ACQUIRE, "agent");
                    asm volatile("s_waitcnt vmcnt(0)" ::: "memory");
                    __syncthreads();
                }
                second_pass_tile<FP, LOGN, INV>(f.pa, unit, tile, lds);
                if (threadIdx.x == 0) add_ctl(fin + unit, 1u);
            }
        }
        __syncthreads();
    }
}

template <class A, int LOGN, bool INV>
__global__ __launch_bounds__(NTT_THREADS, FUSED_WAVES_PER_SIMD) void k_ntt_fixup(FusedArgs f)
{
    typedef FusedPasses<A, LOGN, INV, HANDOFF_ACQUIRE, false> FP;
    __shared__ __attribute__((aligned(16))) typename A::elem lds[FP::LDS_ELEMS];
    u32 *ctl = f.ctl;
    const u32 *fin = ctl + fused_base() + FUSED_TEAMS * f.maxg;
    for (u32 unit = blockIdx.x; unit < f.pa.units; unit += gridDim.x) {
        const u32 n = __builtin_amdgcn_readfirstlane(ld_ctl(fin + unit));
        if (n == FP::T2) continue;
        if (n != 0) {
            if (threadIdx.x == 0) st_ctl(ctl + fused_error_word(), 2u);
            continue;
        }
        for (u32 tile = 0; tile < FP::T1; tile++) {
            first_pass_tile<FP, LOGN, INV>(f.pa, unit, tile, lds);
            __syncthreads();
        }
        asm volatile("s_waitcnt vmcnt(0)" ::: "memory");
        __builtin_amdgcn_fence(__ATOMIC_ACQUIRE, "agent");
        asm volatile("s_waitcnt vmcnt(0)" ::: "memory");
        __syncthreads();
        for (u32 tile = 0; tile < FP::T2; tile++) {
            second_pass_tile<FP, LOGN, INV>(f.pa, unit, tile, lds);
            __syncthreads();
        }
    }
}

template <class A, int LOGN, bool INV, int HANDOFF, bool STREAM, bool FAT = false>
static hipError_t launch_variant(hipStream_t st, const FusedArgs &f, u32 wgs)
{
    typedef FusedPasses<A, LOGN, INV, HANDOFF, STREAM, FAT> FP;
    const u64 tickets = ((u64)f.pa.units + (u64)FUSED_TEAMS * f.dist) * (FP::T1 + FP::T2);
    const u32 grid = (u32)(tickets < wgs ? tickets : wgs);
    hipLaunchKernelGGL((k_ntt_fused<A, LOGN, INV, HANDOFF, STREAM, FAT>), dim3(grid), dim3(FP::NT), 0, st, f);
    hipError_t e = hipGetLastError();
    if (e != hipSuccess) return e;
    const u32 fix = f.pa.units < 64 ? f.pa.units : 64;
    hipLaunchKernelGGL((k_ntt_fixup<A, LOGN, INV>), dim3(fix), dim3(NTT_THREADS), 0, st, f);
    return hipGetLastError();
}

template <class A, int LOGN, bool INV>
static hipError_t launch_fused_t(hipStream_t st, const FusedArgs &f, u32 wgs, int variant)
{
    if constexpr (LOGN == 16) {
        switch (variant) {
        case HANDOFF_SC1 * 2: return launch_variant<A, LOGN, INV, HANDOFF_SC1, false>(st, f, wgs);
        case HANDOFF_SC1 * 2 + 1: return launch_variant<A, LOGN, INV, HANDOFF_SC1, true>(st, f, wgs);
        case HANDOFF_NT * 2: return launch_variant<A, LOGN, INV, HANDOFF_NT, false>(st, f, wgs);
        case HANDOFF_NT * 2 + 1: return launch_variant<A, LOGN, INV, HANDOFF_NT, true>(st, f, wgs);
        case HANDOFF_ACQUIRE * 2: return launch_variant<A, LOGN, INV, HANDOFF_ACQUIRE, false>(st, f, wgs);
        case 8 + HANDOFF_SC1 * 2: return launch_variant<A, LOGN, INV, HANDOFF_SC1, false, true>(st, f, wgs);
        case 8 + HANDOFF_NT * 2: return launch_variant<A, LOGN, INV, HANDOFF_NT, false, true>(st, f, wgs);
        case 8 + HANDOFF_ACQUIRE * 2: return launch_variant<A, LOGN, INV, HANDOFF_ACQUIRE, false, true>(st, f, wgs);
        default: return launch_variant<A, LOGN, INV, HANDOFF_ACQUIRE, true>(st, f, wgs);
        }
    } else {
        return launch_variant<A, LOGN, INV, HANDOFF_ACQUIRE, true>(st, f, wgs);
    }
}

template <class A>
static hipError_t launch_fused_size(hipStream_t st, const FusedArgs &f, int logn, bool inverse, u32 wgs, int variant)
{
    switch (logn) {
#define FHE_CASE(L) \
    case L:         \
        return inverse ? launch_fused_t<A, L, true>(st, f, wgs, variant) : launch_fused_t<A, L, false>(st, f, wgs, variant);
        FHE_CASE(13) FHE_CASE(14) FHE_CASE(15) FHE_CASE(16) FHE_CASE(17)
#undef FHE_CASE
    default:
        return hipErrorInvalidValue;
    }
}

bool fused_supported(int logn) { return logn >= 13 && logn <= 17; }

size_t fused_ctl_bytes(u32 units) { return fused_ctl_words(units) * sizeof(u32); }

hipError_t launch_ntt_fused(hipStream_t st, const PassArgs &a, int logn, bool inverse, int path, u32 *ctl, u32 dist, u32 wgs,
                            int variant, u32 skip_teams)
{
    if (a.units == 0) return hipSuccess;
    if (!fused_supported(logn) || dist < 1) return hipErrorInvalidValue;
    hipError_t e = hipMemsetAsync(ctl, 0, (size_t)fused_error_word() * sizeof(u32), st);
    if (e != hipSuccess) return e;
    e = hipMemsetAsync(ctl + fused_base(), 0, fused_ctl_bytes(a.units) - (size_t)fused_base() * sizeof(u32), st);
    if (e != hipSuccess) return e;
    FusedArgs f{a, ctl, fused_maxg(a.units), dist, skip_teams};
    return path == PATH_F64 ? launch_fused_size<ArithF64>(st, f, logn, inverse, wgs, variant)
                            : launch_fused_size<ArithU64>(st, f, logn, inverse, wgs, variant);
}

}
```

fhe_reliability_gpu_amd/csrc/ntt_kernels.hip:

```cpp
#include "ntt_launch.hpp"
#include "ntt_plan.hpp"
#include "abft_taps.hpp"

#include <cstdlib>
#include <type_traits>

namespace fhe {

template <class PASS, bool IS_COL> struct PASS_TCOLS { static constexpr int value = 0; };
template <class PASS> struct PASS_TCOLS<PASS, true> { static constexpr int value = PASS::TCOLS; };

template <class PASS, int LOGN, bool IS_COL>
FHE_D const u64 *pass_source(const PassArgs &a, const u64 *base, u32 row0)
{
    if (!a.src) return nullptr;
    const u32 unit = blockIdx.x / PASS::TILES, tile = blockIdx.x % PASS::TILES;
    const size_t toff = IS_COL ? (size_t)tile * PASS_TCOLS<PASS, IS_COL>::value : (size_t)row0 * PASS::NPTS;
    if (a.map) {
        const u32 s = a.map[unit].src;
        if (s != 0xFFFFFFFFu) return a.src + ((size_t)s << LOGN) + toff;
    } else if (a.src_bcast) {
        const u32 polys = a.units / a.limbs;
        return a.src + (size_t)(unit % polys) * a.src_bcast + toff;
    }
    if (a.src_stride) {
        const u32 polys = a.units / a.limbs;
        return a.src + (((size_t)(unit % polys) * a.src_stride + unit / polys) << LOGN) + toff;
    }
    return a.src + (base - a.data);
}

template <class PASS, int LOGN, bool INV, bool IS_COL>
__global__ __launch_bounds__(NTT_THREADS) void k_ntt_pass(PassArgs a)
{
    typedef typename PASS::Arith A;
    __shared__ __attribute__((aligned(16))) typename PASS::elem lds[PASS::LDS_ELEMS > 0 ? PASS::LDS_ELEMS : 1];
    u32 limb, row0 = 0;
    u64 *base;
    if constexpr (IS_COL) base = col_tile<PASS, LOGN>(blockIdx.x, a, limb);
    else base = row_tile<PASS, LOGN>(blockIdx.x, a, limb, row0);
    const LimbParams &p = a.lp[limb];
    const typename A::Ctx ctx = A::make_ctx(p);
    const TwPtr tw = as_global(INV ? p.inv : p.fwd);
    const Tw inv_n = p.inv_n;
    const int tid = threadIdx.x;
    const u64 *from = pass_source<PASS, LOGN, IS_COL>(a, base, row0);
    if constexpr (!IS_COL && INV) {
        PASS::template phase<0>(tid, base, lds, tw, row0, ctx, inv_n, (NoTap *)nullptr, from, a.galois, a.galois_copy ? a.galois_copy + (base - a.data) : nullptr);
    } else {
        PASS::template phase<0>(tid, base, lds, tw, row0, ctx, inv_n, (NoTap *)nullptr, from);
    }
    if constexpr (PASS::NPHASE > 1) {
        __syncthreads();
        PASS::template phase<1>(tid, base, lds, tw, row0, ctx, inv_n);
    }
    if constexpr (PASS::NPHASE > 2) {
        __syncthreads();
        PASS::template phase<2>(tid, base, lds, tw, row0, ctx, inv_n);
    }
    if constexpr (PASS::NPHASE > 3) {
        __syncthreads();
        PASS::template phase<3>(tid, base, lds, tw, row0, ctx, inv_n);
    }
}

template <class PASS, int LOGN>
__global__ __launch_bounds__(NTT_THREADS) void k_ntt_gs_first(PassArgs a)
{
    typedef typename PASS::Arith A;
    __shared__ __attribute__((aligned(16))) typename PASS::elem lds[PASS::LDS_ELEMS];
    const u32 unit = blockIdx.x / PASS::TILES, tile = blockIdx.x % PASS::TILES;
    const u32 polys = a.units / a.limbs, l = unit / polys, poly = unit % polys;
    const size_t off = ((size_t)poly * a.poly_stride + l) << LOGN;
    const LimbParams &p = a.lp[a.limb0 + l];
    const typename A::Ctx ctx = A::make_ctx(p);
    const TwPtr tw = as_global(p.inv);
    const Tw inv_n = p.inv_n;
    const int tid = threadIdx.x;
    const u32 row0 = tile * PASS::TROWS;
    u64 *base = a.data + off;
    const u64 *from = a.src + off;
    PASS::template phase<0>(tid, base, lds, tw, row0, ctx, inv_n, (NoTap *)nullptr, from, 0u, nullptr, a.stream_hint != 0);
    __syncthreads();
    PASS::template phase<1>(tid, base, lds, tw, row0, ctx, inv_n);
    if constexpr (PASS::NPHASE > 2) {
        __syncthreads();
        PASS::template phase<2>(tid, base, lds, tw, row0, ctx, inv_n);
    }
    if constexpr (PASS::NPHASE > 3) {
        __syncthreads();
        PASS::template phase<3>(tid, base, lds, tw, row0, ctx, inv_n);
    }
}

template <class PASS, int LOGN, bool INV, bool IS_COL>
static hipError_t launch_pass(hipStream_t st, const PassArgs &a)
{
    const u32 blocks = a.units * PASS::TILES;
    static const u32 extra_lds = getenv("FHE_DBG_EXTRA_LDS") ? (u32)atoi(getenv("FHE_DBG_EXTRA_LDS")) : 0;
    hipLaunchKernelGGL((k_ntt_pass<PASS, LOGN, INV, IS_COL>), dim3(blocks), dim3(NTT_THREADS), extra_lds, st, a);
    return hipGetLastError();
}

template <class PASS, int LOGN>
__global__ __launch_bounds__(NTT_THREADS) void k_ntt_col_packed(PassArgs a)
{
    typedef typename PASS::Arith A;
    static_assert(PASS::PACKABLE, "geometry without a packed form");
    __shared__ __attribute__((aligned(16))) typename PASS::elem lds[PASS::LDS_ELEMS];
    u32 limb;
    u64 *base = col_tile<PASS, LOGN>(blockIdx.x, a, limb);
    const u32 unit = blockIdx.x / PASS::TILES, tile = blockIdx.x % PASS::TILES;
    const LimbParams &p = a.lp[limb];
    const typename A::Ctx ctx = A::make_ctx(p);
    const TwPtr tw = as_global(p.fwd);
    const int tid = threadIdx.x;
    PASS::template phase<0>(tid, base, lds, tw, 0u, ctx, p.inv_n);
    __syncthreads();
    u64 chunk[PK_WORDS];
    PASS::phase_last_packed(tid, lds, tw, 0u, ctx, chunk);
    __syncthreads();
    u64 *stage = reinterpret_cast<u64 *>(lds);
    PASS::pack_stage(tid, stage, chunk);
    __syncthreads();
    PASS::pack_copy_out(tid, stage, a.scratch + ((size_t)unit * 256 + (size_t)tile * 16) * PK_BLOCK_WORDS);
}

template <class PASS, int LOGN>
__global__ __launch_bounds__(NTT_THREADS) void k_ntt_row_packed(PassArgs a)
{
    typedef typename PASS::Arith A;
    static_assert(PASS::PACKABLE && PASS::NPHASE == 3, "geometry without a packed form");
    __shared__ __attribute__((aligned(16))) typename PASS::elem lds[PASS::LDS_ELEMS];
    u32 limb, row0 = 0;
    u64 *base = row_tile<PASS, LOGN>(blockIdx.x, a, limb, row0);
    const u32 unit = blockIdx.x / PASS::TILES, tile = blockIdx.x % PASS::TILES;
    const LimbParams &p = a.lp[limb];
    const typename A::Ctx ctx = A::make_ctx(p);
    const TwPtr tw = as_global(p.fwd);
    const int tid = threadIdx.x;
    u64 *stage = reinterpret_cast<u64 *>(lds);
    PASS::unpack_copy_in(tid, stage, a.scratch + (size_t)unit * 256 * PK_BLOCK_WORDS, tile);
    __syncthreads();
    typename PASS::elem x[16];
    PASS::phase_first_packed(tid, stage, tw, row0, ctx, x);
    __syncthreads();
    PASS::phase_first_store(tid, lds, x);
    __syncthreads();
    PASS::template phase<1>(tid, base, lds, tw, row0, ctx, p.inv_n);
    __syncthreads();
    PASS::template phase<2>(tid, base, lds, tw, row0, ctx, p.inv_n);
}

template <class A, int LOGN, bool INV, int GEO> constexpr bool packed_ok()
{
    typedef Passes<A, LOGN, INV, GEO> PS;
    if constexpr (PS::G::TWO_PASS && !INV && A::PATH == PATH_F64) return PS::Col::PACKABLE && PS::Row::PACKABLE;
    return false;
}

template <class PASS, int LOGN, bool INV>
__global__ __launch_bounds__(PASS::THREADS) void k_ntt_resident(PassArgs a)
{
    typedef typename PASS::Arith A;
    extern __shared__ __attribute__((aligned(16))) unsigned char resident_lds[];
    typename PASS::elem *lds = reinterpret_cast<typename PASS::elem *>(resident_lds);
    u32 limb, row0 = 0;
    u64 *base = row_tile<PASS, LOGN>(blockIdx.x, a, limb, row0);
    const LimbParams &p = a.lp[limb];
    const typename A::Ctx ctx = A::make_ctx(p);
    const TwPtr tw = as_global(INV ? p.inv : p.fwd);
    const Tw inv_n = p.inv_n;
    const int tid = threadIdx.x;
    static_assert(PASS::NPHASE == 4 || PASS::NPHASE == 5, "three register steps and one or two copy phases");
    PASS::template phase<0>(tid, base, lds, tw, row0, ctx, inv_n);
    __syncthreads();
    PASS::template phase<1>(tid, base, lds, tw, row0, ctx, inv_n);
    __syncthreads();
    PASS::template phase<2>(tid, base, lds, tw, row0, ctx, inv_n);
    __syncthreads();
    PASS::template phase<3>(tid, base, lds, tw, row0, ctx, inv_n);
    if constexpr (PASS::NPHASE > 4) {
        __syncthreads();
        PASS::template phase<4>(tid, base, lds, tw, row0, ctx, inv_n);
    }
}

template <class A, int LOGN, bool INV>
static hipError_t launch_resident(hipStream_t st, const PassArgs &a)
{
    typedef typename ResidentPass<A, LOGN, INV>::Pass PASS;
    constexpr size_t bytes = (size_t)PASS::LDS_ELEMS * sizeof(typename PASS::elem);
    static_assert(bytes <= 160 * 1024, "limb does not fit a CU's LDS");
    static bool raised = false;
    if (!raised) {
        hipError_t e = hipFuncSetAttribute(reinterpret_cast<const void *>(&k_ntt_resident<PASS, LOGN, INV>),
                                           hipFuncAttributeMaxDynamicSharedMemorySize, (int)bytes);
        if (e != hipSuccess) return e;
        raised = true;
    }
    hipLaunchKernelGGL((k_ntt_resident<PASS, LOGN, INV>), dim3(a.units * PASS::TILES), dim3(PASS::THREADS), bytes, st, a);
    return hipGetLastError();
}

template <class A, int LOGN, bool INV, int GEO>
static hipError_t launch_transform(hipStream_t st, const PassArgs &a, int which, bool resident)
{
    typedef Passes<A, LOGN, INV, GEO> PS;
    if constexpr (ResidentPlan<LOGN>::OK) {
        if (resident && which == -1) return launch_resident<A, LOGN, INV>(st, a);
    }
    if constexpr (packed_ok<A, LOGN, INV, GEO>()) {
        if (a.scratch && which == -1) {
            hipLaunchKernelGGL((k_ntt_col_packed<typename PS::Col, LOGN>), dim3(a.units * PS::Col::TILES), dim3(NTT_THREADS), 0, st, a);
            hipLaunchKernelGGL((k_ntt_row_packed<typename PS::Row, LOGN>), dim3(a.units * PS::Row::TILES), dim3(NTT_THREADS), 0, st, a);
            return hipGetLastError();
        }
    }
    PassArgs first = a, second = a;
    second.src = nullptr;
    second.galois = 0;
    second.galois_copy = nullptr;
    if (a.tmp && which == -1) {
        if (!first.src) first.src = a.data;
        first.data = a.tmp;
        second.src = a.tmp;
        if (a.tmp_stride) {
            first.src_stride = a.poly_stride;
            first.poly_stride = a.tmp_stride;
            second.src_stride = a.tmp_stride;
        }
    }
    if constexpr (!PS::G::TWO_PASS) {
        if (which == 1) return hipSuccess;
        if (a.stream_hint && !a.src) return launch_pass<typename PS::SingleNt, LOGN, INV, false>(st, a);
        return launch_pass<typename PS::Single, LOGN, INV, false>(st, a);
    } else if (GEO == 1 && a.stream_hint) {
        if constexpr (GEO == 1) {
            hipError_t e = which == 1 ? hipSuccess
                                      : INV ? launch_pass<typename PS::RowNt, LOGN, INV, false>(st, first) : launch_pass<typename PS::ColNt, LOGN, INV, true>(st, first);
            if (e != hipSuccess || which == 0) return e;
            return INV ? launch_pass<typename PS::ColNt, LOGN, INV, true>(st, second) : launch_pass<typename PS::RowNt, LOGN, INV, false>(st, second);
        }
        return hipErrorInvalidValue;
    } else if constexpr (!INV) {
        hipError_t e = which == 1 ? hipSuccess : launch_pass<typename PS::Col, LOGN, INV, true>(st, first);
        if (e != hipSuccess || which == 0) return e;
        return launch_pass<typename PS::Row, LOGN, INV, false>(st, second);
    } else {
        hipError_t e = hipSuccess;
        if (which != 1) {
            bool done = false;
            if constexpr (LOGN == 17 && GEO == 1) {
                typedef RowPass<A, typename PS::PL::Row, LOGN, 4, NTT_THREADS, true, IO_CANONICAL, IO_LAZY, PS::RED_FIRST, PS::SB> RowSmall;
                if (a.units * PS::Row::TILES >= 768u && a.units * PS::Row::TILES <= 2048u) {
                    e = launch_pass<RowSmall, LOGN, INV, false>(st, first);
                    done = true;
                }
            }
            if (!done) e = launch_pass<typename PS::Row, LOGN, INV, false>(st, first);
        }
        if (e != hipSuccess || which == 0) return e;
        return launch_pass<typename PS::Col, LOGN, INV, true>(st, second);
    }
}

template <class A, int LOGN>
static hipError_t launch_gs_t(hipStream_t st, const PassArgs &a, u64 *tmp)
{
    constexpr int GEO = LOGN >= 13 ? 1 : 0;
    typedef Passes<A, LOGN, true, GEO> PS;
    constexpr bool TWO = PS::G::TWO_PASS;
    typedef RowPass<A, typename PS::PL::Row, LOGN, TWO ? PS::G::TR : 1, NTT_THREADS, true, IO_CANONICAL, TWO ? IO_LAZY : IO_CANONICAL, PS::RED_FIRST,
                    PS::SB, 0, false, false, 1> First;
    if constexpr (!TWO) {
        hipLaunchKernelGGL((k_ntt_gs_first<First, LOGN>), dim3(a.units * First::TILES), dim3(NTT_THREADS), 0, st, a);
        return hipGetLastError();
    } else {
        if (!tmp) return hipErrorInvalidValue;
        PassArgs first = a, second = a;
        first.data = tmp;
        second.src = tmp;
        hipLaunchKernelGGL((k_ntt_gs_first<First, LOGN>), dim3(a.units * First::TILES), dim3(NTT_THREADS), 0, st, first);
        if (a.stream_hint && GEO == 1) {
            if constexpr (GEO == 1) return launch_pass<typename PS::ColNt, LOGN, true, true>(st, second);
        }
        return launch_pass<typename PS::Col, LOGN, true, true>(st, second);
    }
}

bool ntt_gs_supported(int logn) { return logn >= 5 && logn <= NTT_MAX_LOGN; }

hipError_t launch_ntt_gs(hipStream_t st, const PassArgs &a, u64 *tmp, int logn, int path)
{
    if (a.units == 0) return hipSuccess;
    if (!a.src || a.map || !ntt_gs_supported(logn)) return hipErrorInvalidValue;
    switch (logn) {
#define FHE_CASE(L) \
    case L: return path == PATH_F64 ? launch_gs_t<ArithF64, L>(st, a, tmp) : launch_gs_t<ArithU64, L>(st, a, tmp);
        FHE_CASE(5) FHE_CASE(6) FHE_CASE(7) FHE_CASE(8) FHE_CASE(9) FHE_CASE(10) FHE_CASE(11) FHE_CASE(12) FHE_CASE(13)
        FHE_CASE(14) FHE_CASE(15) FHE_CASE(16) FHE_CASE(17) FHE_CASE(18) FHE_CASE(19) FHE_CASE(20)
#undef FHE_CASE
    default: return hipErrorInvalidValue;
    }
}

template <class A>
static hipError_t launch_size(hipStream_t st, const PassArgs &a, int logn, bool inverse, int geo, int which, bool resident)
{
    if (logn == 16 && geo == 0)
        return inverse ? launch_transform<A, 16, true, 0>(st, a, which, false) : launch_transform<A, 16, false, 0>(st, a, which, false);
    switch (logn) {
#define FHE_CASE(L)                                                        \
    case L:                                                                \
        return inverse ? launch_transform<A, L, true, (L >= 13 ? 1 : 0)>(st, a, which, resident) : launch_transform<A, L, false, (L >= 13 ? 1 : 0)>(st, a, which, resident);
        FHE_CASE(1) FHE_CASE(2) FHE_CASE(3) FHE_CASE(4) FHE_CASE(5) FHE_CASE(6) FHE_CASE(7) FHE_CASE(8)
        FHE_CASE(9) FHE_CASE(10) FHE_CASE(11) FHE_CASE(12) FHE_CASE(13) FHE_CASE(14) FHE_CASE(15) FHE_CASE(16)
        FHE_CASE(17) FHE_CASE(18) FHE_CASE(19) FHE_CASE(20)
#undef FHE_CASE
    default:
        return hipErrorInvalidValue;
    }
}

struct AbftArgs {
    const Tw *win;
    const Tw *wout;
    const u64 *wout8;
    int logp;
    u64 *sum_in;
    u64 *sum_out;
};

template <class PASS, int LOGN, bool IS_COL, bool IN, bool OUT, bool INV = false>
__global__ __launch_bounds__(NTT_THREADS) void k_ntt_pass_abft(PassArgs a, AbftArgs ab)
{
    typedef typename PASS::Arith A;
    typedef std::conditional_t<INV, InvChecksumTap<A, IN, OUT>, ChecksumTap<A, IN, OUT>> Tap;
    __shared__ __attribute__((aligned(16))) typename PASS::elem lds[PASS::LDS_ELEMS > 0 ? PASS::LDS_ELEMS : 1];
    __shared__ u64 red[2][NTT_THREADS / 64];
    u32 limb, row0 = 0;
    u64 *base;
    if constexpr (IS_COL) base = col_tile<PASS, LOGN>(blockIdx.x, a, limb);
    else base = row_tile<PASS, LOGN>(blockIdx.x, a, limb, row0);
    const u32 unit = blockIdx.x / PASS::TILES, polys = a.units / a.limbs;
    const u32 l = unit / polys, poly = unit % polys, slot = poly * a.poly_stride + l;
    const u32 pos0 = (u32)((base - a.data) & (((size_t)1 << LOGN) - 1));
    const LimbParams &p = a.lp[limb];
    const typename A::Ctx ctx = A::make_ctx(p);
    const TwPtr tw = as_global(INV ? p.inv : p.fwd);
    const Tw inv_n = p.inv_n;
    const int tid = threadIdx.x;
    Tap tap{as_global(ab.win) + ((size_t)limb << LOGN) + pos0, as_global(ab.wout) + ((size_t)limb << LOGN) + pos0,
                                (const u64 FHE_GLOBAL *)ab.wout8 + ((size_t)limb << LOGN) + pos0, pos0, ab.logp,
                                typename A::elem(0), typename A::elem(0), 0, 0};
    const u64 *from = pass_source<PASS, LOGN, IS_COL>(a, base, row0);
    PASS::template phase<0>(tid, base, lds, tw, row0, ctx, inv_n, &tap, from);
    if constexpr (PASS::NPHASE > 1) {
        __syncthreads();
        PASS::template phase<1>(tid, base, lds, tw, row0, ctx, inv_n, &tap);
    }
    if constexpr (PASS::NPHASE > 2) {
        __syncthreads();
        PASS::template phase<2>(tid, base, lds, tw, row0, ctx, inv_n, &tap);
    }
    if constexpr (PASS::NPHASE > 3) {
        __syncthreads();
        PASS::template phase<3>(tid, base, lds, tw, row0, ctx, inv_n, &tap);
    }
    const u32 tile = blockIdx.x % PASS::TILES;
    if constexpr (IN) block_sum_mod(A::canonical(tap.acc_in, ctx), p.q, ab.sum_in + (size_t)slot * PASS::TILES + tile, red[0]);
    if constexpr (OUT) block_sum_mod(A::canonical(tap.acc_out, ctx), p.q, ab.sum_out + (size_t)slot * PASS::TILES + tile, red[1]);
}

template <class A, int LOGN>
static hipError_t launch_checked(hipStream_t st, const PassArgs &a, const AbftArgs &ab, int which)
{
    constexpr int GEO = LOGN >= 13 ? 1 : 0;
    typedef Passes<A, LOGN, false, GEO> PS;
    if constexpr (!PS::G::TWO_PASS) {
        if (which == 1) return hipSuccess;
        hipLaunchKernelGGL((k_ntt_pass_abft<typename PS::Single, LOGN, false, true, true>), dim3(a.units * PS::Single::TILES), dim3(NTT_THREADS), 0, st, a, ab);
    } else {
        PassArgs first = a, second = a;
        if (a.tmp && which == -1) {
            first.src = a.data;
            first.data = a.tmp;
            second.src = a.tmp;
        }
        if (a.stream_hint && GEO == 1) {
            if (which != 1) hipLaunchKernelGGL((k_ntt_pass_abft<typename PS::ColNt, LOGN, true, true, false>), dim3(a.units * PS::Col::TILES), dim3(NTT_THREADS), 0, st, first, ab);
            if (which != 0) hipLaunchKernelGGL((k_ntt_pass_abft<typename PS::RowNt, LOGN, false, false, true>), dim3(a.units * PS::Row::TILES), dim3(NTT_THREADS), 0, st, second, ab);
            return hipGetLastError();
        }
        if (which != 1) hipLaunchKernelGGL((k_ntt_pass_abft<typename PS::Col, LOGN, true, true, false>), dim3(a.units * PS::Col::TILES), dim3(NTT_THREADS), 0, st, first, ab);
        if (which != 0) hipLaunchKernelGGL((k_ntt_pass_abft<typename PS::Row, LOGN, false, false, true>), dim3(a.units * PS::Row::TILES), dim3(NTT_THREADS), 0, st, second, ab);
    }
    return hipGetLastError();
}

template <class A, int LOGN>
static hipError_t launch_checked_inv(hipStream_t st, const PassArgs &a, const AbftArgs &ab, int which)
{
    constexpr int GEO = LOGN >= 13 ? 1 : 0;
    typedef Passes<A, LOGN, true, GEO> PS;
    if constexpr (!PS::G::TWO_PASS) {
        if (which == 1) return hipSuccess;
        hipLaunchKernelGGL((k_ntt_pass_abft<typename PS::Single, LOGN, false, true, true, true>), dim3(a.units * PS::Single::TILES), dim3(NTT_THREADS), 0, st, a, ab);
    } else {
        PassArgs first = a, second = a;
        if (a.tmp && which == -1) {
            first.src = a.data;
            first.data = a.tmp;
            second.src = a.tmp;
        }
        if (a.stream_hint && GEO == 1) {
            if (which != 1) hipLaunchKernelGGL((k_ntt_pass_abft<typename PS::RowNt, LOGN, false, true, false, true>), dim3(a.units * PS::Row::TILES), dim3(NTT_THREADS), 0, st, first, ab);
            if (which != 0) hipLaunchKernelGGL((k_ntt_pass_abft<typename PS::ColNt, LOGN, true, false, true, true>), dim3(a.units * PS::Col::TILES), dim3(NTT_THREADS), 0, st, second, ab);
            return hipGetLastError();
        }
        if (which != 1) hipLaunchKernelGGL((k_ntt_pass_abft<typename PS::Row, LOGN, false, true, false, true>), dim3(a.units * PS::Row::TILES), dim3(NTT_THREADS), 0, st, first, ab);
        if (which != 0) hipLaunchKernelGGL((k_ntt_pass_abft<typename PS::Col, LOGN, true, false, true, true>), dim3(a.units * PS::Col::TILES), dim3(NTT_THREADS), 0, st, second, ab);
    }
    return hipGetLastError();
}

template <class PASS, int LOGN, bool IS_COL, int PASSID>
__global__ __launch_bounds__(NTT_THREADS) void k_ntt_pass_phase(PassArgs a, PhaseArgs ph)
{
    typedef typename PASS::Arith A;
    static_assert(PASS::NPHASE >= 2, "per-phase checks are for the two-launch sizes");
    __shared__ __attribute__((aligned(16))) typename PASS::elem lds[PASS::LDS_ELEMS];
    __shared__ u64 red[2][NTT_THREADS / 64];
    u32 limb, row0 = 0;
    u64 *base;
    if constexpr (IS_COL) base = col_tile<PASS, LOGN>(blockIdx.x, a, limb);
    else base = row_tile<PASS, LOGN>(blockIdx.x, a, limb, row0);
    const u32 unit = blockIdx.x / PASS::TILES, polys = a.units / a.limbs;
    const u32 l = unit / polys, poly = unit % polys, slot = poly * a.poly_stride + l;
    const u32 pos0 = (u32)((base - a.data) & (((size_t)1 << LOGN) - 1));
    const LimbParams &p = a.lp[limb];
    const typename A::Ctx ctx = A::make_ctx(p);
    const TwPtr tw = as_global(p.fwd);
    const Tw inv_n = p.inv_n;
    const int tid = threadIdx.x;
    const size_t woff = ((size_t)limb << LOGN) + pos0;
    PhaseTap<A, PASSID> tap{as_global(ph.win) + woff, as_global(ph.umid) + woff, as_global(ph.wout) + woff, (const u64 FHE_GLOBAL *)ph.umid8 + woff,
                            (const u64 FHE_GLOBAL *)ph.wout8 + woff, pos0, ph.logp, typename A::elem(0), typename A::elem(0), 0, 0};
    const u64 *from = pass_source<PASS, LOGN, IS_COL>(a, base, row0);
    PASS::template phase<0>(tid, base, lds, tw, row0, ctx, inv_n, &tap, from);
    __syncthreads();
    if (ph.fault_pass == PASSID && ph.fault_block == blockIdx.x) {
        if (tid == 0) reinterpret_cast<u64 *>(lds)[ph.fault_word % (u32)PASS::LDS_ELEMS] ^= (u64)1 << ph.fault_bit;
        __syncthreads();
    }
    PASS::template phase<1>(tid, base, lds, tw, row0, ctx, inv_n, &tap);
    if constexpr (PASS::NPHASE > 2) {
        __syncthreads();
        PASS::template phase<2>(tid, base, lds, tw, row0, ctx, inv_n, &tap);
    }
    if constexpr (PASS::NPHASE > 3) {
        __syncthreads();
        PASS::template phase<3>(tid, base, lds, tw, row0, ctx, inv_n, &tap);
    }
    const u32 tile = blockIdx.x % PASS::TILES;
    block_sum_mod(A::canonical(tap.acc_a, ctx), p.q, ph.sum_a + (size_t)slot * PASS::TILES + tile, red[0]);
    block_sum_mod(A::canonical(tap.acc_b, ctx), p.q, ph.sum_b + (size_t)slot * PASS::TILES + tile, red[1]);
}

template <class A, int LOGN>
static hipError_t launch_phases_t(hipStream_t st, const PassArgs &a, const PhaseArgs &p1, const PhaseArgs &p2, int which)
{
    typedef Passes<A, LOGN, false, 1> PS;
    if constexpr (PS::G::TWO_PASS) {
        PassArgs first = a, second = a;
        if (a.tmp && which == -1) {
            first.src = a.data;
            first.data = a.tmp;
            second.src = a.tmp;
        }
        if (a.stream_hint) {
            if (which != 1) hipLaunchKernelGGL((k_ntt_pass_phase<typename PS::ColNt, LOGN, true, 0>), dim3(a.units * PS::Col::TILES), dim3(NTT_THREADS), 0, st, first, p1);
            if (which != 0) hipLaunchKernelGGL((k_ntt_pass_phase<typename PS::RowNt, LOGN, false, 1>), dim3(a.units * PS::Row::TILES), dim3(NTT_THREADS), 0, st, second, p2);
            return hipGetLastError();
        }
        if (which != 1) hipLaunchKernelGGL((k_ntt_pass_phase<typename PS::Col, LOGN, true, 0>), dim3(a.units * PS::Col::TILES), dim3(NTT_THREADS), 0, st, first, p1);
        if (which != 0) hipLaunchKernelGGL((k_ntt_pass_phase<typename PS::Row, LOGN, false, 1>), dim3(a.units * PS::Row::TILES), dim3(NTT_THREADS), 0, st, second, p2);
        return hipGetLastError();
    }
    return hipErrorInvalidValue;
}

bool ntt_phases_supported(int logn) { return logn >= 13 && logn <= NTT_MAX_LOGN; }

int ntt_column_stages(int logn)
{
    switch (logn) {
#define FHE_CASE(L) case L: return Plan<L>::Col::P;
        FHE_CASE(1) FHE_CASE(2) FHE_CASE(3) FHE_CASE(4) FHE_CASE(5) FHE_CASE(6) FHE_CASE(7) FHE_CASE(8) FHE_CASE(9) FHE_CASE(10)
        FHE_CASE(11) FHE_CASE(12) FHE_CASE(13) FHE_CASE(14) FHE_CASE(15) FHE_CASE(16) FHE_CASE(17) FHE_CASE(18) FHE_CASE(19) FHE_CASE(20)
#undef FHE_CASE
    default: return 0;
    }
}

hipError_t launch_ntt_phases(hipStream_t st, const PassArgs &a, const PhaseArgs &p1, const PhaseArgs &p2, int logn, int path, int which)
{
    if (a.units == 0) return hipSuccess;
    if (a.map || !ntt_phases_supported(logn)) return hipErrorInvalidValue;
    switch (logn) {
#define FHE_CASE(L) \
    case L: return path == PATH_F64 ? launch_phases_t<ArithF64, L>(st, a, p1, p2, which) : launch_phases_t<ArithU64, L>(st, a, p1, p2, which);
        FHE_CASE(13) FHE_CASE(14) FHE_CASE(15) FHE_CASE(16) FHE_CASE(17) FHE_CASE(18) FHE_CASE(19) FHE_CASE(20)
#undef FHE_CASE
    default: return hipErrorInvalidValue;
    }
}

bool ntt_checked_supported(int logn) { return logn >= 5 && logn <= NTT_MAX_LOGN; }

template <int LOGN> static void checked_tiles_t(u32 *tin, u32 *tout, bool inverse)
{
    typedef Passes<ArithF64, LOGN, false, (LOGN >= 13 ? 1 : 0)> PS;
    typedef Passes<ArithF64, LOGN, true, (LOGN >= 13 ? 1 : 0)> PI;
    if constexpr (!PS::G::TWO_PASS) *tin = *tout = inverse ? PI::Single::TILES : PS::Single::TILES;
    else if (inverse) {
        *tin = PI::Row::TILES;
        *tout = PI::Col::TILES;
    } else {
        *tin = PS::Col::TILES;
        *tout = PS::Row::TILES;
    }
}
void ntt_checked_tiles(int logn, u32 *tin, u32 *tout, bool inverse)
{
    *tin = *tout = 1;
    switch (logn) {
#define FHE_CASE(L) case L: checked_tiles_t<L>(tin, tout, inverse); break;
        FHE_CASE(5) FHE_CASE(6) FHE_CASE(7) FHE_CASE(8) FHE_CASE(9) FHE_CASE(10) FHE_CASE(11) FHE_CASE(12) FHE_CASE(13)
        FHE_CASE(14) FHE_CASE(15) FHE_CASE(16) FHE_CASE(17) FHE_CASE(18) FHE_CASE(19) FHE_CASE(20)
#undef FHE_CASE
    default: break;
    }
}

hipError_t launch_ntt_checked(hipStream_t st, const PassArgs &a, const Tw *win, const Tw *wout, const u64 *wout8, u64 *sum_in, u64 *sum_out,
                              int logn, int path, int which, bool inverse)
{
    if (a.units == 0) return hipSuccess;
    if (a.map) return hipErrorInvalidValue;
    const AbftArgs ab{win, wout, wout8, logn / 2, sum_in, sum_out};
    switch (logn) {
#define FHE_CASE(L)                                                                                                               \
    case L:                                                                                                                       \
        if (inverse) return path == PATH_F64 ? launch_checked_inv<ArithF64, L>(st, a, ab, which) : launch_checked_inv<ArithU64, L>(st, a, ab, which); \
        return path == PATH_F64 ? launch_checked<ArithF64, L>(st, a, ab, which) : launch_checked<ArithU64, L>(st, a, ab, which);
        FHE_CASE(5) FHE_CASE(6) FHE_CASE(7) FHE_CASE(8) FHE_CASE(9) FHE_CASE(10) FHE_CASE(11) FHE_CASE(12) FHE_CASE(13)
        FHE_CASE(14) FHE_CASE(15) FHE_CASE(16) FHE_CASE(17) FHE_CASE(18) FHE_CASE(19) FHE_CASE(20)
#undef FHE_CASE
    default: return hipErrorInvalidValue;
    }
}

struct PolymulArgs {
    PassArgs a;
    const u64 *b;
    u64 *c;
};

template <class FR, int E = 0, class TWS = TwPtr>
FHE_D void fwd_steps(int tid, u64 *base, typename FR::elem *lds, const TWS &tw, u32 row0, const typename FR::Arith::Ctx &ctx, const Tw &inv_n)
{
    if constexpr (E < FR::NSTEP) {
        if (E > 0) __syncthreads();
        FR::template phase<E, NoTap, TWS>(tid, base, lds, tw, row0, ctx, inv_n);
        fwd_steps<FR, E + 1, TWS>(tid, base, lds, tw, row0, ctx, inv_n);
    }
}
template <class IR, int E = 1>
FHE_D void inv_steps(int tid, u64 *base, typename IR::elem *lds, TwPtr tw, u32 row0, const typename IR::Arith::Ctx &ctx, const Tw &inv_n)
{
    if constexpr (E < IR::NPHASE) {
        __syncthreads();
        IR::template phase<E>(tid, base, lds, tw, row0, ctx, inv_n);
        inv_steps<IR, E + 1>(tid, base, lds, tw, row0, ctx, inv_n);
    }
}
template <class A, int LOGN, int GEO>
__global__ __launch_bounds__(NTT_THREADS) void k_polymul_mid(PolymulArgs pa)
{
    typedef typename MidPasses<A, LOGN, GEO>::Fwd FR;
    typedef typename MidPasses<A, LOGN, GEO>::Inv IR;
    static_assert(FR::STAGED && IR::STAGED && FR::LDS_ELEMS == IR::LDS_ELEMS, "fused product needs the staged row pass");
    typedef typename FR::elem elem;
    constexpr int PAIRS = FR::TROWS * FR::NPTS / 2;
    constexpr int PER = (PAIRS + NTT_THREADS - 1) / NTT_THREADS;
    __shared__ __attribute__((aligned(16))) elem lds[FR::LDS_ELEMS];
    u32 limb, row0;
    u64 *ta = row_tile<FR, LOGN>(blockIdx.x, pa.a, limb, row0);
    const size_t off = (size_t)(ta - pa.a.data);
    const LimbParams &p = pa.a.lp[limb];
    const typename A::Ctx ctx = A::make_ctx(p);
    const Tw inv_n = p.inv_n;
    const int tid = threadIdx.x;

    fwd_steps<FR>(tid, ta, lds, as_global(p.fwd), row0, ctx, inv_n);
    __syncthreads();
    elem ra[PER][2];
#pragma unroll
    for (int k = 0; k < PER; k++) {
        const int i = tid + k * NTT_THREADS;
        if (PAIRS % NTT_THREADS == 0 || i < PAIRS) {
            const u32 row = (u32)i / (FR::NPTS / 2), g = ((u32)i % (FR::NPTS / 2)) * 2;
            const elem *src = lds + row * FR::ROW_LDS + row_pad(g);
            ra[k][0] = src[0];
            ra[k][1] = src[1];
        }
    }
    __syncthreads();
    fwd_steps<FR>(tid, const_cast<u64 *>(pa.b) + off, lds, as_global(p.fwd), row0, ctx, inv_n);
    __syncthreads();
#pragma unroll
    for (int k = 0; k < PER; k++) {
        const int i = tid + k * NTT_THREADS;
        if (PAIRS % NTT_THREADS == 0 || i < PAIRS) {
            const u32 row = (u32)i / (FR::NPTS / 2), g = ((u32)i % (FR::NPTS / 2)) * 2;
            elem *dst = lds + row * FR::ROW_LDS + row_pad(g);
            if constexpr (A::PATH == PATH_F64) {
                dst[0] = A::mulvar_lazy(ra[k][0], dst[0], ctx);
                dst[1] = A::mulvar_lazy(ra[k][1], dst[1], ctx);
            } else {
                dst[0] = A::mulvar_lazy(ra[k][0], dst[0], p);
                dst[1] = A::mulvar_lazy(ra[k][1], dst[1], p);
            }
        }
    }
    inv_steps<IR>(tid, pa.c + off, lds, as_global(p.inv), row0, ctx, inv_n);
}

template <class A, int LOGN>
static hipError_t launch_mid(hipStream_t st, const PolymulArgs &pa)
{
    constexpr int GEO = LOGN >= 13 ? 1 : 0;
    typedef typename MidPasses<A, LOGN, GEO>::Fwd FR;
    hipLaunchKernelGGL((k_polymul_mid<A, LOGN, GEO>), dim3(pa.a.units * FR::TILES), dim3(NTT_THREADS), 0, st, pa);
    return hipGetLastError();
}

bool polymul_fused_supported(int logn) { return logn >= 5 && logn <= NTT_MAX_LOGN; }

hipError_t launch_polymul(hipStream_t st, const PassArgs &a, u64 *b, u64 *c, int logn, int path)
{
    if (a.units == 0) return hipSuccess;
    if (!polymul_fused_supported(logn)) return hipErrorInvalidValue;
    hipError_t e;
    PassArgs pb = a, pc = a;
    pb.data = b;
    pc.data = c;
    if (logn >= 13) {
        if ((e = launch_ntt(st, a, logn, false, path, 1, 0)) != hipSuccess) return e;
        if (b != a.data && (e = launch_ntt(st, pb, logn, false, path, 1, 0)) != hipSuccess) return e;
    }
    const PolymulArgs pa{a, b, c};
    switch (logn) {
#define FHE_CASE(L)                                                                                     \
    case L:                                                                                             \
        e = path == PATH_F64 ? launch_mid<ArithF64, L>(st, pa) : launch_mid<ArithU64, L>(st, pa);       \
        break;
        FHE_CASE(5) FHE_CASE(6) FHE_CASE(7) FHE_CASE(8) FHE_CASE(9) FHE_CASE(10) FHE_CASE(11) FHE_CASE(12) FHE_CASE(13)
        FHE_CASE(14) FHE_CASE(15) FHE_CASE(16) FHE_CASE(17) FHE_CASE(18) FHE_CASE(19) FHE_CASE(20)
#undef FHE_CASE
    default:
        return hipErrorInvalidValue;
    }
    if (e != hipSuccess) return e;
    if (logn >= 13) return launch_ntt(st, pc, logn, true, path, 1, 1);
    return hipSuccess;
}

template <class A>
struct SubScaleTap {
    static constexpr bool ACTIVE = true;
    static constexpr bool MID = false;
    static constexpr bool STORES = true;
    const u64 *acc, *add;
    u64 *out;
    u64 scal, q, r0, r1, pre;
    double n, ninv;
    const u64 *add_limb;
    u32 pos0, galois;
    int logn;
    const u64 *acc_limb;
    u64 scal2;
    template <class E, class C> FHE_D void in(u32, E, const C &) {}
    FHE_D u64 one_int(u64 a, u64 x, u64 t, bool has_add) const
    {
        const u64 av = a < q ? a : barrett128(a, 0, q, r0, r1);
        if (pre) x = barrett128(x * pre, mulhi64(x, pre), q, r0, r1);
        const u64 d = av >= x ? av - x : av + q - x;
        u64 v = barrett128(d * scal, mulhi64(d, scal), q, r0, r1);
        if (has_add) {
            v += t < q ? t : barrett128(t, 0, q, r0, r1);
            v = v >= q ? v - q : v;
        }
        if (scal2) v = barrett128(v * scal2, mulhi64(v, scal2), q, r0, r1);
        return v;
    }
    FHE_D u64 one_f64(u64 a, u64 x, u64 t, bool has_add) const
    {
        const typename ArithF64::Ctx c{n, ninv, q};
        double xv = ArithF64::from_canonical(x);
        if (pre) {
            const double pw = ArithF64::from_canonical(pre);
            xv = ArithF64::mulmod_w(xv, pw, pw * ninv, c);
        }
        const double d = ArithF64::from_canonical(a) - xv;
        const double sw = ArithF64::from_canonical(scal);
        double v = ArithF64::mulmod_w(d, sw, sw * ninv, c);
        if (has_add) v += ArithF64::from_canonical(t);
        if (scal2) {
            const double s2 = ArithF64::from_canonical(scal2);
            v = ArithF64::mulmod_w(v, s2, s2 * ninv, c);
        }
        return ArithF64::canonical(v, c);
    }
    FHE_D void store(u32 idx, u64 x0, u64 x1)
    {
        ulonglong2 a;
        if (acc_limb) a = ulonglong2{acc_limb[galois_slot(pos0 + idx, logn, galois)], acc_limb[galois_slot(pos0 + idx + 1, logn, galois)]};
        else a = *reinterpret_cast<const ulonglong2 *>(acc + idx);
        ulonglong2 t = ulonglong2{0, 0};
        if (add) {
            if (galois) t = ulonglong2{add_limb[galois_slot(pos0 + idx, logn, galois)], add_limb[galois_slot(pos0 + idx + 1, logn, galois)]};
            else t = *reinterpret_cast<const ulonglong2 *>(add + idx);
        }
        ulonglong2 r;
        bool fp = A::PATH == PATH_F64;
        if (A::PATH == PATH_F64) fp = !__builtin_expect((a.x >= q) | (a.y >= q) | (t.x >= q) | (t.y >= q), 0);
        if (fp) {
            r.x = one_f64(a.x, x0, t.x, add != nullptr);
            r.y = one_f64(a.y, x1, t.y, add != nullptr);
        } else {
            r.x = one_int(a.x, x0, t.x, add != nullptr);
            r.y = one_int(a.y, x1, t.y, add != nullptr);
        }
        *reinterpret_cast<ulonglong2 *>(out + idx) = r;
    }
};

template <class A>
struct AddSrcTap {
    static constexpr bool ACTIVE = true;
    static constexpr bool MID = false;
    static constexpr bool STORES = false;
    static constexpr bool PRELOAD = true;
    const u64 *y;
    Tw w;
    FHE_D u64 load(u32 idx) const { return y[idx]; }
    template <int R> FHE_D void prepare(u64 (&e)[R], const typename A::Ctx &c) const
    {
        if constexpr (A::PATH == PATH_F64) {
            bool big = false;
#pragma unroll
            for (int r = 0; r < R; r++) big |= (e[r] >> 52) != 0;
            if (__builtin_expect(big, 0)) {
#pragma unroll
                for (int r = 0; r < R; r++) e[r] = (e[r] >> 52) ? reduce_any_u64(e[r], c.q) : e[r];
            }
        }
    }
    FHE_D void apply(typename A::elem &x, u64 v, const typename A::Ctx &c) const
    {
        if constexpr (A::PATH == PATH_F64) {
            x += A::mulmod(A::from_canonical(v), w, c);
            A::reduce(x, c);
        } else {
            x += A::mulmod(v, w, c);
        }
    }
};

template <class PASS, int LOGN>
__global__ __launch_bounds__(NTT_THREADS) void k_ntt_col_addsrc(PassArgs a, ColAddSrc s)
{
    typedef typename PASS::Arith A;
    __shared__ __attribute__((aligned(16))) typename PASS::elem lds[PASS::LDS_ELEMS > 0 ? PASS::LDS_ELEMS : 1];
    u32 limb;
    u64 *base = col_tile<PASS, LOGN>(blockIdx.x, a, limb);
    const u32 unit = blockIdx.x / PASS::TILES, tile = blockIdx.x % PASS::TILES, polys = a.units / a.limbs;
    const LimbParams &p = a.lp[limb];
    const typename A::Ctx ctx = A::make_ctx(p);
    const TwPtr tw = as_global(p.fwd);
    const Tw inv_n = p.inv_n;
    const int tid = threadIdx.x;
    AddSrcTap<A> tap{s.y + (size_t)(unit % polys) * s.y_stride + (size_t)tile * PASS::TCOLS, s.w[limb]};
    const u64 *from = pass_source<PASS, LOGN, true>(a, base, 0u);
    PASS::template phase<0>(tid, base, lds, tw, 0u, ctx, inv_n, &tap, from);
    if constexpr (PASS::NPHASE > 1) {
        __syncthreads();
        PASS::template phase<1>(tid, base, lds, tw, 0u, ctx, inv_n);
    }
    if constexpr (PASS::NPHASE > 2) {
        __syncthreads();
        PASS::template phase<2>(tid, base, lds, tw, 0u, ctx, inv_n);
    }
}

template <class PASS, int LOGN>
__global__ __launch_bounds__(NTT_THREADS) void k_ntt_row_subscale(PassArgs a, RowEpiArgs ep)
{
    typedef typename PASS::Arith A;
    static_assert(PASS::STAGE_OUT, "the epilogue sits in the staged copy-out phase");
    __shared__ __attribute__((aligned(16))) typename PASS::elem lds[PASS::LDS_ELEMS];
    u32 limb, row0 = 0;
    u64 *base = row_tile<PASS, LOGN>(blockIdx.x, a, limb, row0);
    const u32 unit = blockIdx.x / PASS::TILES, polys = a.units / a.limbs, l = unit / polys, h = unit % polys;
    const LimbParams &p = a.lp[limb];
    const typename A::Ctx ctx = A::make_ctx(p);
    const TwPtr tw = as_global(p.fwd);
    const Tw inv_n = p.inv_n;
    const int tid = threadIdx.x;
    const size_t eoff = ((size_t)l << LOGN) + (size_t)row0 * PASS::NPTS;
    SubScaleTap<A> tap{ep.a + (size_t)h * ep.a_stride + eoff, ep.add[h] ? ep.add[h] + eoff : nullptr, ep.out[h] + eoff, ep.scal[l], p.q, p.barrett_lo, p.barrett_hi,
                       ep.pre ? ep.pre[l] : 0, p.n, p.ninv, ep.add[h] ? ep.add[h] + ((size_t)l << LOGN) : nullptr, row0 * (u32)PASS::NPTS, ep.galois, LOGN,
                       ep.galois && ep.galois_a ? ep.a + (size_t)h * ep.a_stride + ((size_t)l << LOGN) : nullptr, ep.scal2 ? ep.scal2[l] : 0};
    const u64 *from = pass_source<PASS, LOGN, false>(a, base, row0);
    PASS::template phase<0>(tid, base, lds, tw, row0, ctx, inv_n, &tap, from);
    if constexpr (PASS::NPHASE > 1) {
        __syncthreads();
        PASS::template phase<1>(tid, base, lds, tw, row0, ctx, inv_n, &tap);
    }
    if constexpr (PASS::NPHASE > 2) {
        __syncthreads();
        PASS::template phase<2>(tid, base, lds, tw, row0, ctx, inv_n, &tap);
    }
    if constexpr (PASS::NPHASE > 3) {
        __syncthreads();
        PASS::template phase<3>(tid, base, lds, tw, row0, ctx, inv_n, &tap);
    }
}

template <class A, int LOGN>
static hipError_t launch_subscale_t(hipStream_t st, const PassArgs &a, const RowEpiArgs &ep, const ColAddSrc *add_src)
{
    constexpr int GEO = LOGN >= 13 ? 1 : 0;
    typedef Passes<A, LOGN, false, GEO> PS;
    if constexpr (!PS::G::TWO_PASS) {
        if (add_src) return hipErrorInvalidValue;
        hipLaunchKernelGGL((k_ntt_row_subscale<typename PS::Single, LOGN>), dim3(a.units * PS::Single::TILES), dim3(NTT_THREADS), 0, st, a, ep);
    } else {
        hipError_t e;
        if (add_src) {
            hipLaunchKernelGGL((k_ntt_col_addsrc<typename PS::Col, LOGN>), dim3(a.units * PS::Col::TILES), dim3(NTT_THREADS), 0, st, a, *add_src);
            e = hipGetLastError();
        } else {
            e = launch_pass<typename PS::Col, LOGN, false, true>(st, a);
        }
        if (e != hipSuccess) return e;
        PassArgs second = a;
        second.src = nullptr;
        hipLaunchKernelGGL((k_ntt_row_subscale<typename PS::Row, LOGN>), dim3(a.units * PS::Row::TILES), dim3(NTT_THREADS), 0, st, second, ep);
    }
    return hipGetLastError();
}

bool ntt_subscale_supported(int logn) { return logn >= 5 && logn <= NTT_MAX_LOGN; }

hipError_t launch_ntt_subscale(hipStream_t st, const PassArgs &a, const RowEpiArgs &ep, int logn, int path, const ColAddSrc *add_src)
{
    if (a.units == 0) return hipSuccess;
    if (a.map || !ntt_subscale_supported(logn) || a.units / a.limbs > 3) return hipErrorInvalidValue;
    switch (logn) {
#define FHE_CASE(L) \
    case L: return path == PATH_F64 ? launch_subscale_t<ArithF64, L>(st, a, ep, add_src) : launch_subscale_t<ArithU64, L>(st, a, ep, add_src);
        FHE_CASE(5) FHE_CASE(6) FHE_CASE(7) FHE_CASE(8) FHE_CASE(9) FHE_CASE(10) FHE_CASE(11) FHE_CASE(12) FHE_CASE(13)
        FHE_CASE(14) FHE_CASE(15) FHE_CASE(16) FHE_CASE(17) FHE_CASE(18) FHE_CASE(19) FHE_CASE(20)
#undef FHE_CASE
    default: return hipErrorInvalidValue;
    }
}

template <class A, int LOGN, int GEO>
__global__ __launch_bounds__(NTT_THREADS, 2) void k_ks_rowmac(KsMacArgs a)
{
    typedef MidPasses<A, LOGN, GEO> MP;
    typedef typename std::conditional<LOGN == 16 && GEO == 1,
                                      RowPass<A, Steps<3, 3, 2>, LOGN, MP::TR, NTT_THREADS, false, IO_LAZY, IO_LAZY, MP::F::RED_SECOND, MP::SB>,
                                      typename MP::Fwd>::type FR;
    static_assert(FR::STAGED, "fused inner product needs the staged row pass");
    typedef typename FR::elem elem;
    constexpr int PAIRS = FR::TROWS * FR::NPTS / 2;
    constexpr int PER = (PAIRS + NTT_THREADS - 1) / NTT_THREADS;
    __shared__ __attribute__((aligned(16))) elem lds[FR::LDS_ELEMS];
    const u32 jj = blockIdx.x / FR::TILES, tile = blockIdx.x % FR::TILES;
    const u32 tl = jj < a.cn ? a.clo + jj : jj + a.sp_shift;
    const LimbParams &p = a.lp[tl];
    if (p.path != A::PATH) return;
    const typename A::Ctx ctx = A::make_ctx(p);
    const Tw inv_n = p.inv_n;
    const TwPtr tw = as_global(p.fwd);
    const int tid = threadIdx.x;
    const u32 row0 = tile * FR::TROWS;
    const size_t toff = (size_t)row0 * FR::NPTS;
    elem s0[PER][2], s1[PER][2];
#pragma unroll
    for (int k = 0; k < PER; k++) s0[k][0] = s0[k][1] = s1[k][0] = s1[k][1] = elem(0);
    int terms = 0;
    for (u32 d = 0; d < a.dnum; d++) {
        const u32 lo = d * a.alpha, hi = lo + a.alpha < a.L ? lo + a.alpha : a.L;
        const bool own = jj < a.cn && tl >= lo && tl < hi;
        if (!own) {
            u64 *src = const_cast<u64 *>(a.ext) + (((size_t)d * a.M + jj) << LOGN) + toff;
            if (d) __syncthreads();
            fwd_steps<FR>(tid, src, lds, tw, row0, ctx, inv_n);
            __syncthreads();
        }
        const u64 *k0 = a.evk + ((((size_t)d * 2) * a.M + jj) << LOGN) + toff, *k1 = k0 + ((size_t)a.M << LOGN);
        ++terms;
#pragma unroll
        for (int k = 0; k < PER; k++) {
            const int i = tid + k * NTT_THREADS;
            if (PAIRS % NTT_THREADS == 0 || i < PAIRS) {
                const u32 row = (u32)i / (FR::NPTS / 2), g = ((u32)i % (FR::NPTS / 2)) * 2;
                const size_t off = (size_t)row * FR::NPTS + g;
                ulonglong2 cw = ulonglong2{0, 0};
                if (own) cw = *reinterpret_cast<const ulonglong2 *>(a.c + ((size_t)jj << LOGN) + toff + off);
                typedef u64 u64x2 __attribute__((ext_vector_type(2)));
                const u64x2 v0 = __builtin_nontemporal_load(reinterpret_cast<const u64x2 *>(k0 + off)), v1 = __builtin_nontemporal_load(reinterpret_cast<const u64x2 *>(k1 + off));
                ulonglong2 w0 = ulonglong2{v0.x, v0.y}, w1 = ulonglong2{v1.x, v1.y};
                if (__builtin_expect((cw.x >= p.q) | (cw.y >= p.q) | (w0.x >= p.q) | (w0.y >= p.q) | (w1.x >= p.q) | (w1.y >= p.q), 0)) {
                    cw.x = barrett128(cw.x, 0, p.q, p.barrett_lo, p.barrett_hi);
                    cw.y = barrett128(cw.y, 0, p.q, p.barrett_lo, p.barrett_hi);
                    w0.x = barrett128(w0.x, 0, p.q, p.barrett_lo, p.barrett_hi);
                    w0.y = barrett128(w0.y, 0, p.q, p.barrett_lo, p.barrett_hi);
                    w1.x = barrett128(w1.x, 0, p.q, p.barrett_lo, p.barrett_hi);
                    w1.y = barrett128(w1.y, 0, p.q, p.barrett_lo, p.barrett_hi);
                }
                elem x0, x1;
                if (own) {
                    x0 = A::from_canonical(cw.x);
                    x1 = A::from_canonical(cw.y);
                } else {
                    const elem *src = lds + row * FR::ROW_LDS + row_pad(g);
                    x0 = src[0];
                    x1 = src[1];
                }
                const elem y00 = A::from_canonical(w0.x), y01 = A::from_canonical(w0.y), y10 = A::from_canonical(w1.x), y11 = A::from_canonical(w1.y);
                if constexpr (A::PATH == PATH_F64) {
                    A::lazy_acc(s0[k][0], A::mulvar_lazy(x0, y00, ctx), terms, ctx);
                    A::lazy_acc(s0[k][1], A::mulvar_lazy(x1, y01, ctx), terms, ctx);
                    A::lazy_acc(s1[k][0], A::mulvar_lazy(x0, y10, ctx), terms, ctx);
                    A::lazy_acc(s1[k][1], A::mulvar_lazy(x1, y11, ctx), terms, ctx);
                } else {
                    A::lazy_acc(s0[k][0], A::mulvar_lazy(x0, y00, p), terms, ctx);
                    A::lazy_acc(s0[k][1], A::mulvar_lazy(x1, y01, p), terms, ctx);
                    A::lazy_acc(s1[k][0], A::mulvar_lazy(x0, y10, p), terms, ctx);
                    A::lazy_acc(s1[k][1], A::mulvar_lazy(x1, y11, p), terms, ctx);
                }
            }
#if defined(__HIP_DEVICE_COMPILE__)
            if ((k & 3) == 3) __builtin_amdgcn_sched_barrier(0);
#endif
        }
    }
    u64 *o0 = a.acc + ((size_t)jj << LOGN) + toff, *o1 = o0 + ((size_t)a.M << LOGN);
#pragma unroll
    for (int k = 0; k < PER; k++) {
        const int i = tid + k * NTT_THREADS;
        if (PAIRS % NTT_THREADS == 0 || i < PAIRS) {
            const u32 row = (u32)i / (FR::NPTS / 2), g = ((u32)i % (FR::NPTS / 2)) * 2;
            const size_t off = (size_t)row * FR::NPTS + g;
            ulonglong2 r0, r1;
            r0.x = A::canonical(s0[k][0], ctx);
            r0.y = A::canonical(s0[k][1], ctx);
            r1.x = A::canonical(s1[k][0], ctx);
            r1.y = A::canonical(s1[k][1], ctx);
            *reinterpret_cast<ulonglong2 *>(o0 + off) = r0;
            *reinterpret_cast<ulonglong2 *>(o1 + off) = r1;
        }
    }
}

template <int LOGN>
struct RowMacLt {
    typedef ArithF64 A;
    typedef MidPasses<A, LOGN, 1> MP;
    typedef typename MP::PL PL;
    static constexpr int PR = PL::Row::P, NPTS = 1 << PR, S0 = LOGN - PR, TR = MP::TR;
    typedef typename std::conditional<PR == 8, Steps<3, 3, 2>, typename PL::Row>::type ST;
    static constexpr u32 red_every4()
    {
        u32 m = 0;
        for (int u = 0; u < PR; u += 4) m |= 1u << u;
        return m;
    }
    typedef RowPass<A, ST, LOGN, TR, NTT_THREADS, false, IO_LAZY, IO_LAZY, red_every4(), MP::SB, 0, false, true> FR;
    static constexpr int TW_PER_ROW = NPTS - 1, TW_ELEMS = TR * TW_PER_ROW;
    static constexpr size_t LDS_BYTES = ((size_t)FR::LDS_ELEMS + TW_ELEMS) * 8;
    static_assert(TR * NPTS == 16 * NTT_THREADS, "sixteen points per thread");
};

template <class FR, int E, class TWS>
FHE_D void lt_steps(int tid, typename FR::elem *lds, const TWS &tw, u32 row0, const typename FR::Arith::Ctx &ctx, const Tw &inv_n)
{
    if constexpr (E <= FR::NSTEP) {
        FR::template phase<E, NoTap, TWS>(tid, nullptr, lds, tw, row0, ctx, inv_n);
        __syncthreads();
        lt_steps<FR, E + 1, TWS>(tid, lds, tw, row0, ctx, inv_n);
    }
}

template <int LOGN>
__global__ __launch_bounds__(NTT_THREADS, 2) void k_ks_rowmac_lt(KsMacArgs a)
{
    typedef RowMacLt<LOGN> RM;
    typedef typename RM::FR FR;
    typedef ArithF64 A;
    typedef double elem;
    typedef u64 u64x2 __attribute__((ext_vector_type(2)));
    constexpr int PAIRS = FR::TROWS * FR::NPTS / 2;
    constexpr int PER = PAIRS / NTT_THREADS;
    static_assert(PER == 8, "sixteen points per thread");
    extern __shared__ __attribute__((aligned(16))) unsigned char rowmac_lds[];
// ... 55 lines not shown
    }
    const RowTwLds tws{twl, ctx.ninv, row0, RM::S0, RM::TW_PER_ROW};
    elem s0[PER][2], s1[PER][2];
#pragma unroll
    for (int k = 0; k < PER; k++) s0[k][0] = s0[k][1] = s1[k][0] = s1[k][1] = 0.0;
    int terms = 0;
    const u64 q = p.q;
    for (u32 d = 0; d < a.dnum; d++) {
        const bool own = d == own_d;
        const u64 *k0 = a.evk + ((((size_t)d * 2) * a.M + jj) << LOGN) + toff, *k1 = k0 + ((size_t)a.M << LOGN);
        u64x2 kv0[PER], kv1[PER];
#pragma unroll
        for (int k = 0; k < PER; k++) {
            kv0[k] = __builtin_nontemporal_load(reinterpret_cast<const u64x2 *>(k0 + goff[k]));
            kv1[k] = __builtin_nontemporal_load(reinterpret_cast<const u64x2 *>(k1 + goff[k]));
        }
        elem x[PER][2];
        if (own) {
            const u64 *src = a.c + ((size_t)jj << LOGN) + toff;
            u64x2 cw[PER];
#pragma unroll
            for (int k = 0; k < PER; k++) cw[k] = *reinterpret_cast<const u64x2 *>(src + goff[k]);
            bool bad = false;
#pragma unroll
            for (int k = 0; k < PER; k++) bad |= (cw[k].x >= q) | (cw[k].y >= q);
            if (__builtin_expect(bad, 0)) {
#pragma unroll
                for (int k = 0; k < PER; k++) {
                    cw[k].x = barrett128(cw[k].x, 0, q, p.barrett_lo, p.barrett_hi);
                    cw[k].y = barrett128(cw[k].y, 0, q, p.barrett_lo, p.barrett_hi);
                }
            }
#pragma unroll
            for (int k = 0; k < PER; k++) {
                x[k][0] = A::from_canonical(cw[k].x);
                x[k][1] = A::from_canonical(cw[k].y);
            }
        } else {
            __syncthreads();
#pragma unroll
            for (int k = 0; k < PER; k++) *reinterpret_cast<u64x2 *>(lds + loff[k]) = tv[k];
            u32 nd = d + 1;
            nd += nd == own_d ? 1u : 0u;
            if (nd < a.dnum) {
                const u64 *src = tile_of(nd);
#pragma unroll
                for (int k = 0; k < PER; k++) tv[k] = *reinterpret_cast<const u64x2 *>(src + goff[k]);
            }
            __syncthreads();
            lt_steps<FR, 1, RowTwLds>(tid, lds, tws, row0, ctx, inv_n);
#pragma unroll
            for (int k = 0; k < PER; k++) {
                const double2 v = *reinterpret_cast<const double2 *>(lds + loff[k]);
                x[k][0] = v.x;
                x[k][1] = v.y;
            }
        }
        {
            bool bad = false;
#pragma unroll
            for (int k = 0; k < PER; k++) bad |= (kv0[k].x >= q) | (kv0[k].y >= q) | (kv1[k].x >= q) | (kv1[k].y >= q);
            if (__builtin_expect(bad, 0)) {
#pragma unroll
                for (int k = 0; k < PER; k++) {
                    kv0[k].x = barrett128(kv0[k].x, 0, q, p.barrett_lo, p.barrett_hi);
                    kv0[k].y = barrett128(kv0[k].y, 0, q, p.barrett_lo, p.barrett_hi);
                    kv1[k].x = barrett128(kv1[k].x, 0, q, p.barrett_lo, p.barrett_hi);
                    kv1[k].y = barrett128(kv1[k].y, 0, q, p.barrett_lo, p.barrett_hi);
                }
            }
        }
        ++terms;
#pragma unroll
        for (int k = 0; k < PER; k++) {
            A::lazy_acc(s0[k][0], A::mulvar_lazy(x[k][0], A::from_canonical(kv0[k].x), ctx), terms, ctx);
            A::lazy_acc(s0[k][1], A::mulvar_lazy(x[k][1], A::from_canonical(kv0[k].y), ctx), terms, ctx);
            A::lazy_acc(s1[k][0], A::mulvar_lazy(x[k][0], A::from_canonical(kv1[k].x), ctx), terms, ctx);
            A::lazy_acc(s1[k][1], A::mulvar_lazy(x[k][1], A::from_canonical(kv1[k].y), ctx), terms, ctx);
        }
    }
    u64 *o0 = a.acc + ((size_t)jj << LOGN) + toff, *o1 = o0 + ((size_t)a.M << LOGN);
#pragma unroll
    for (int k = 0; k < PER; k++) {
        *reinterpret_cast<u64x2 *>(o0 + goff[k]) = u64x2{A::canonical(s0[k][0], ctx), A::canonical(s0[k][1], ctx)};
        *reinterpret_cast<u64x2 *>(o1 + goff[k]) = u64x2{A::canonical(s1[k][0], ctx), A::canonical(s1[k][1], ctx)};
    }
}

template <int LOGN>
static hipError_t launch_rowmac_lt(hipStream_t st, const KsMacArgs &a)
{
    typedef RowMacLt<LOGN> RM;
    static_assert(RM::LDS_BYTES <= 80 * 1024, "two workgroups per CU");
    static bool raised = false;
    if (!raised) {
        hipError_t e = hipFuncSetAttribute(reinterpret_cast<const void *>(&k_ks_rowmac_lt<LOGN>), hipFuncAttributeMaxDynamicSharedMemorySize, (int)RM::LDS_BYTES);
        if (e != hipSuccess) return e;
        raised = true;
    }
    hipLaunchKernelGGL((k_ks_rowmac_lt<LOGN>), dim3(a.M * RM::FR::TILES), dim3(NTT_THREADS), RM::LDS_BYTES, st, a);
    return hipSuccess;
}

bool ks_rowmac_supported(int logn) { return logn >= 5 && logn <= NTT_MAX_LOGN; }

template <class A, int LOGN>
static void launch_rowmac_t(hipStream_t st, const KsMacArgs &a)
{
    constexpr int GEO = LOGN >= 13 ? 1 : 0;
    typedef typename MidPasses<A, LOGN, GEO>::Fwd FR;
    static const int variant = getenv("FHE_KS_ROWMAC") ? atoi(getenv("FHE_KS_ROWMAC")) : 1;
    if constexpr (LOGN >= 13 && A::PATH == PATH_F64) {
        if (variant) {
            (void)launch_rowmac_lt<LOGN>(st, a);
            return;
        }
    }
    hipLaunchKernelGGL((k_ks_rowmac<A, LOGN, GEO>), dim3(a.M * FR::TILES), dim3(NTT_THREADS), 0, st, a);
}

hipError_t launch_ks_rowmac(hipStream_t st, const KsMacArgs &a, bool has_f64, bool has_u64)
{
    if (!a.M) return hipSuccess;
    if (!ks_rowmac_supported(a.logn)) return hipErrorInvalidValue;
    switch (a.logn) {
#define FHE_CASE(L)                                              \
    case L:                                                      \
        if (has_f64) launch_rowmac_t<ArithF64, L>(st, a);        \
        if (has_u64) launch_rowmac_t<ArithU64, L>(st, a);        \
        break;
        FHE_CASE(5) FHE_CASE(6) FHE_CASE(7) FHE_CASE(8) FHE_CASE(9) FHE_CASE(10) FHE_CASE(11) FHE_CASE(12) FHE_CASE(13)
        FHE_CASE(14) FHE_CASE(15) FHE_CASE(16) FHE_CASE(17) FHE_CASE(18) FHE_CASE(19) FHE_CASE(20)
#undef FHE_CASE
    default:
        return hipErrorInvalidValue;
    }
    return hipGetLastError();
}

bool ntt_packed_supported(int logn, bool inverse, int path)
{
    return logn == 16 && !inverse && path == PATH_F64 && packed_ok<ArithF64, 16, false, 1>();
}
size_t ntt_packed_scratch_words() { return (size_t)256 * PK_BLOCK_WORDS; }

hipError_t launch_ntt(hipStream_t st, const PassArgs &a, int logn, bool inverse, int path, int geo, int which, bool resident)
{
    if (a.units == 0) return hipSuccess;
    if (a.src || a.tmp) {
        if (a.scratch) return hipErrorInvalidValue;
        geo = 1;
        resident = false;
    }
    return path == PATH_F64 ? launch_size<ArithF64>(st, a, logn, inverse, geo, which, resident)
                            : launch_size<ArithU64>(st, a, logn, inverse, geo, which, resident);
}

}
```

fhe_reliability_gpu_amd/csrc/ntt_plan.hpp:

```cpp
#pragma once
#include "ntt_core.hpp"

namespace fhe {

constexpr int NTT_THREADS = 256;
constexpr int NTT_MAX_LOGN = 20;

template <int LOGN> struct Plan;
#define FHE_PLAN(LOGN_, C0, C1, C2, R0, R1, R2)                      \
    template <> struct Plan<LOGN_> {                                 \
        typedef Steps<C0, C1, C2> Col;                               \
        typedef Steps<R0, R1, R2> Row;                               \
        static_assert(Col::P + Row::P == LOGN_, "bad plan");         \
    };
FHE_PLAN(1, 0, 0, 0, 1, 0, 0)
FHE_PLAN(2, 0, 0, 0, 2, 0, 0)
FHE_PLAN(3, 0, 0, 0, 3, 0, 0)
FHE_PLAN(4, 0, 0, 0, 4, 0, 0)
FHE_PLAN(5, 0, 0, 0, 3, 2, 0)
FHE_PLAN(6, 0, 0, 0, 3, 3, 0)
FHE_PLAN(7, 0, 0, 0, 4, 3, 0)
FHE_PLAN(8, 0, 0, 0, 4, 4, 0)
FHE_PLAN(9, 0, 0, 0, 3, 3, 3)
FHE_PLAN(10, 0, 0, 0, 4, 3, 3)
FHE_PLAN(11, 0, 0, 0, 4, 4, 3)
FHE_PLAN(12, 0, 0, 0, 4, 4, 4)
FHE_PLAN(13, 3, 2, 0, 4, 4, 0)
FHE_PLAN(14, 3, 3, 0, 4, 4, 0)
FHE_PLAN(15, 4, 3, 0, 4, 4, 0)
FHE_PLAN(16, 4, 4, 0, 4, 4, 0)
FHE_PLAN(17, 4, 4, 0, 3, 3, 3)
FHE_PLAN(18, 4, 4, 0, 4, 3, 3)
FHE_PLAN(19, 4, 4, 0, 4, 4, 3)
FHE_PLAN(20, 4, 4, 0, 4, 4, 4)
#undef FHE_PLAN


template <int LOGN> struct BlkStage {
    typedef typename Plan<LOGN>::Row R;
    static constexpr int value = LOGN - R::k(R::NSTEP - 1);
};
inline int blk_stage_rt(int logn)
{
    switch (logn) {
#define FHE_B(L) case L: return BlkStage<L>::value;
        FHE_B(1) FHE_B(2) FHE_B(3) FHE_B(4) FHE_B(5) FHE_B(6) FHE_B(7) FHE_B(8) FHE_B(9) FHE_B(10)
        FHE_B(11) FHE_B(12) FHE_B(13) FHE_B(14) FHE_B(15) FHE_B(16) FHE_B(17) FHE_B(18) FHE_B(19) FHE_B(20)
#undef FHE_B
    default: return logn;
    }
}
inline u32 tw_stored_index(int logn, u32 k)
{
    if (k == 0) return 0;
    const int sigma = 31 - __builtin_clz(k);
    return tw_index(blk_stage_rt(logn), sigma, k - (1u << sigma));
}

template <int LOGN, int GEO = 0> struct PlanGeom {
    typedef Plan<LOGN> PL;
    static constexpr int PC = PL::Col::P, PR = PL::Row::P;
    static constexpr bool TWO_PASS = PC > 0;
    static constexpr int TC = !TWO_PASS ? 1 : GEO == 0 ? cmin(64, 8192 >> PC) : (PC <= 8 ? 16 : 8);
    static constexpr int TR = !TWO_PASS ? 1 : PR <= 8 ? 16 : PR == 9 ? 8 : PR == 10 ? 4 : PR == 11 ? 2 : 1;
};

struct UnitRef {
    u32 off, limb;
    u32 src = 0xFFFFFFFFu;
};

struct PassArgs {
    u64 *data;
    const LimbParams *lp;
    u32 limb0;
    u32 limbs;
    u32 units;
    u32 poly_stride;
    const UnitRef *map = nullptr;
    u64 *scratch = nullptr;
    u64 *tmp = nullptr;
    u64 src_bcast = 0;
    const u64 *src = nullptr;
    u32 stream_hint = 0;
    u32 src_stride = 0;
    u32 tmp_stride = 0;
    u32 galois = 0;
    u64 *galois_copy = nullptr;
};

template <class A, int LOGN, bool INVERSE, int GEO = 0>
struct Passes {
    typedef PlanGeom<LOGN, GEO> G;
    typedef typename G::PL PL;
    static constexpr bool LAZY_INV = INVERSE && A::PATH == PATH_F64;
    static constexpr u32 RED_FIRST = LAZY_INV ? (INV_LAZY | 8u)
                                     : INVERSE ? reduce_mask(0, G::PR, A::INV_FIRST, A::INV_NEXT)
                                               : reduce_mask(0, G::TWO_PASS ? G::PC : G::PR, A::FWD_FIRST, A::FWD_NEXT);
    static constexpr u32 RED_SECOND = LAZY_INV ? (INV_LAZY | (u32)inv_lazy_pass_out8<typename PL::Row>(8))
                                      : INVERSE ? reduce_mask(G::PR, G::PC, A::INV_FIRST, A::INV_NEXT)
                                                : reduce_mask(G::PC, G::PR, A::FWD_FIRST, A::FWD_NEXT);
    static constexpr int SB = BlkStage<LOGN>::value;
    typedef RowPass<A, typename PL::Row, LOGN, 1, NTT_THREADS, INVERSE, IO_CANONICAL, IO_CANONICAL, RED_FIRST, SB> Single;
    typedef RowPass<A, typename PL::Row, LOGN, 1, NTT_THREADS, INVERSE, IO_CANONICAL, IO_CANONICAL, RED_FIRST, SB, 0, true> SingleNt;
    typedef ColPass<A, typename PL::Col, LOGN, 0, G::TC, NTT_THREADS, INVERSE, INVERSE ? IO_LAZY : IO_CANONICAL,
                    INVERSE ? IO_CANONICAL : IO_LAZY, INVERSE ? RED_SECOND : RED_FIRST, SB> Col;
    typedef RowPass<A, typename PL::Row, LOGN, G::TR, NTT_THREADS, INVERSE, INVERSE ? IO_CANONICAL : IO_LAZY,
                    INVERSE ? IO_LAZY : IO_CANONICAL, INVERSE ? RED_FIRST : RED_SECOND, SB> Row;
    typedef ColPass<A, typename PL::Col, LOGN, 0, G::TC, NTT_THREADS, INVERSE, INVERSE ? IO_LAZY : IO_CANONICAL,
                    INVERSE ? IO_CANONICAL : IO_LAZY, INVERSE ? RED_SECOND : RED_FIRST, SB, 0, true> ColNt;
    typedef RowPass<A, typename PL::Row, LOGN, G::TR, NTT_THREADS, INVERSE, INVERSE ? IO_CANONICAL : IO_LAZY,
                    INVERSE ? IO_LAZY : IO_CANONICAL, INVERSE ? RED_FIRST : RED_SECOND, SB, 0, true> RowNt;
};

template <class A, int LOGN>
struct GsPasses {
    static constexpr int GEO = LOGN >= 13 ? 1 : 0;
    typedef Passes<A, LOGN, true, GEO> PS;
    static constexpr bool TWO = PS::G::TWO_PASS;
    typedef RowPass<A, typename PS::PL::Row, LOGN, TWO ? PS::G::TR : 1, NTT_THREADS, true, IO_CANONICAL, TWO ? IO_LAZY : IO_CANONICAL, PS::RED_FIRST,
                    PS::SB, 0, false, false, 1> First;
    typedef typename PS::Col Second;
    typedef typename PS::ColNt SecondNt;
};

template <class A, int LOGN, int GEO>
struct MidPasses {
    typedef Passes<A, LOGN, false, GEO> F;
    typedef Passes<A, LOGN, true, GEO> I;
    typedef typename F::PL PL;
    static constexpr bool TWO = F::G::TWO_PASS;
    static constexpr int TR = TWO ? F::G::TR : 1;
    static constexpr int SB = BlkStage<LOGN>::value;
    typedef RowPass<A, typename PL::Row, LOGN, TR, NTT_THREADS, false, TWO ? IO_LAZY : IO_CANONICAL, IO_LAZY, TWO ? F::RED_SECOND : F::RED_FIRST, SB> Fwd;
    typedef RowPass<A, typename PL::Row, LOGN, TR, NTT_THREADS, true, IO_LAZY, TWO ? IO_LAZY : IO_CANONICAL, I::RED_FIRST, SB> Inv;
};

template <int LOGN> struct ResidentPlan {
    static constexpr bool OK = false;
    typedef Steps<1, 0, 0> S;
    static constexpr int THREADS = NTT_THREADS;
};
template <> struct ResidentPlan<13> {
    static constexpr bool OK = true;
    typedef Steps<5, 4, 4> S;
    static constexpr int THREADS = 256;
};
template <> struct ResidentPlan<14> {
    static constexpr bool OK = true;
    typedef Steps<5, 5, 4> S;
    static constexpr int THREADS = 512;
};
template <class A, int LOGN, bool INVERSE>
struct ResidentPass {
    typedef ResidentPlan<LOGN> RP;
    static_assert(!RP::OK || LOGN - RP::S::k(RP::S::NSTEP - 1) == BlkStage<LOGN>::value, "last register step must match the table layout");
    static constexpr u32 RED = INVERSE ? reduce_mask(0, LOGN, A::INV_FIRST, A::INV_NEXT) : reduce_mask(0, LOGN, A::FWD_FIRST, A::FWD_NEXT);
    typedef RowPass<A, typename RP::S, LOGN, 1, RP::THREADS, INVERSE, IO_CANONICAL, IO_CANONICAL, RED, BlkStage<LOGN>::value> Pass;
};

template <class CP, int LOGN>
FHE_D u64 *col_tile_of(u32 unit, u32 tile, const PassArgs &a, u32 &limb)
{
    const u32 poly = unit / a.limbs, l = unit % a.limbs;
    limb = a.limb0 + l;
    return a.data + (((size_t)poly * a.poly_stride + l) << LOGN) + (size_t)tile * CP::TCOLS;
}
template <class RP, int LOGN>
FHE_D u64 *row_tile_of(u32 unit, u32 tile, const PassArgs &a, u32 &limb, u32 &row0)
{
    const u32 poly = unit / a.limbs, l = unit % a.limbs;
    limb = a.limb0 + l;
    row0 = tile * RP::TROWS;
    return a.data + (((size_t)poly * a.poly_stride + l) << LOGN) + (size_t)row0 * RP::NPTS;
}
template <class CP, int LOGN>
FHE_D u64 *col_tile(u32 block, const PassArgs &a, u32 &limb)
{
    const u32 unit = block / CP::TILES, tile = block % CP::TILES;
    if (a.map) {
        const UnitRef m = a.map[unit];
        limb = m.limb;
        return a.data + ((size_t)m.off << LOGN) + (size_t)tile * CP::TCOLS;
    }
    const u32 polys = a.units / a.limbs;
    const u32 l = unit / polys, poly = unit % polys;
    limb = a.limb0 + l;
    return a.data + (((size_t)poly * a.poly_stride + l) << LOGN) + (size_t)tile * CP::TCOLS;
}
template <class RP, int LOGN>
FHE_D u64 *row_tile(u32 block, const PassArgs &a, u32 &limb, u32 &row0)
{
    const u32 unit = block / RP::TILES, tile = block % RP::TILES;
    row0 = tile * RP::TROWS;
    if (a.map) {
        const UnitRef m = a.map[unit];
        limb = m.limb;
        return a.data + ((size_t)m.off << LOGN) + (size_t)row0 * RP::NPTS;
    }
    const u32 polys = a.units / a.limbs;
    const u32 l = unit / polys, poly = unit % polys;
    limb = a.limb0 + l;
    return a.data + (((size_t)poly * a.poly_stride + l) << LOGN) + (size_t)row0 * RP::NPTS;
}

}
```

fhe_reliability_gpu_amd/csrc/polymul_checked.hip:

```cpp
#include "ntt_launch.hpp"
#include "ntt_plan.hpp"
#include "abft_taps.hpp"

#include <type_traits>

namespace fhe {

template <class FR, int E = 0, class TAP>
FHE_D void fwd_steps_tap(int tid, u64 *base, typename FR::elem *lds, TwPtr tw, u32 row0, const typename FR::Arith::Ctx &ctx, const Tw &inv_n, TAP *tap)
{
    if constexpr (E < FR::NSTEP) {
        if (E > 0) __syncthreads();
        FR::template phase<E, TAP>(tid, base, lds, tw, row0, ctx, inv_n, tap);
        fwd_steps_tap<FR, E + 1>(tid, base, lds, tw, row0, ctx, inv_n, tap);
    }
}
template <class IR, int E = 1, class TAP>
FHE_D void inv_steps_tap(int tid, u64 *base, typename IR::elem *lds, TwPtr tw, u32 row0, const typename IR::Arith::Ctx &ctx, const Tw &inv_n, TAP *tap)
{
    if constexpr (E < IR::NPHASE) {
        __syncthreads();
        IR::template phase<E, TAP>(tid, base, lds, tw, row0, ctx, inv_n, tap);
        inv_steps_tap<IR, E + 1>(tid, base, lds, tw, row0, ctx, inv_n, tap);
    }
}

struct PolymulChkArgs {
    PassArgs a;
    const u64 *b;
    u64 *c;
    const Tw *win, *wout;
    const u64 *wout8;
    int logp;
    PolymulSums s;
    const u64 *fault_at;
    int fault_bit;
};

template <class A, int LOGN, int GEO>
__global__ __launch_bounds__(NTT_THREADS) void k_polymul_mid_checked(PolymulChkArgs k)
{
    typedef MidPasses<A, LOGN, GEO> MP;
    typedef typename MP::Fwd FR;
    typedef typename MP::Inv IR;
    static_assert(FR::STAGED && IR::STAGED && FR::LDS_ELEMS == IR::LDS_ELEMS, "fused product needs the staged row pass");
    typedef typename FR::elem elem;
    typedef ChecksumTap<A, true, false> InTap;
    typedef InvChecksumTap<A, false, true> OutTap;
    constexpr int PAIRS = FR::TROWS * FR::NPTS / 2;
    constexpr int PER = (PAIRS + NTT_THREADS - 1) / NTT_THREADS;
    const PolymulChkArgs &pa = k;
    __shared__ __attribute__((aligned(16))) elem lds[FR::LDS_ELEMS];
    __shared__ u64 red[6][NTT_THREADS / 64];
    u32 limb, row0;
    u64 *ta = row_tile<FR, LOGN>(blockIdx.x, pa.a, limb, row0);
    const size_t off = (size_t)(ta - pa.a.data);
    const LimbParams &p = pa.a.lp[limb];
    const typename A::Ctx ctx = A::make_ctx(p);
    const Tw inv_n = p.inv_n;
    const int tid = threadIdx.x;
    const u32 unit = blockIdx.x / FR::TILES, tile = blockIdx.x % FR::TILES, polys = pa.a.units / pa.a.limbs;
    const size_t slot = (size_t)(unit % polys) * pa.a.poly_stride + unit / polys;
    const u32 pos0 = (u32)(off & (((size_t)1 << LOGN) - 1));
    const size_t woff = ((size_t)limb << LOGN) + pos0;
    InTap tin_a{as_global(k.win) + woff, as_global(k.wout) + woff, (const u64 FHE_GLOBAL *)k.wout8 + woff, pos0, k.logp, elem(0), elem(0), 0, 0};
    InTap tin_b = tin_a;
    OutTap tout_c{as_global(k.win) + woff, as_global(k.wout) + woff, (const u64 FHE_GLOBAL *)k.wout8 + woff, pos0, k.logp, elem(0), elem(0), 0, 0};
    const int fk = k.fault_at && k.fault_at >= ta && k.fault_at < ta + FR::TROWS * FR::NPTS ? (int)(k.fault_at - ta) : -1;

    if constexpr (MP::TWO) fwd_steps_tap<FR>(tid, ta, lds, as_global(p.fwd), row0, ctx, inv_n, (NoTap *)nullptr);
    else fwd_steps_tap<FR>(tid, ta, lds, as_global(p.fwd), row0, ctx, inv_n, &tin_a);
    __syncthreads();
    elem ra[PER][2];
#pragma unroll
    for (int j = 0; j < PER; j++) {
        const int i = tid + j * NTT_THREADS;
        if (PAIRS % NTT_THREADS == 0 || i < PAIRS) {
            const u32 row = (u32)i / (FR::NPTS / 2), g = ((u32)i % (FR::NPTS / 2)) * 2;
            const elem *src = lds + row * FR::ROW_LDS + row_pad(g);
            ra[j][0] = src[0];
            ra[j][1] = src[1];
        }
    }
    __syncthreads();
    if constexpr (MP::TWO) fwd_steps_tap<FR>(tid, const_cast<u64 *>(pa.b) + off, lds, as_global(p.fwd), row0, ctx, inv_n, (NoTap *)nullptr);
    else fwd_steps_tap<FR>(tid, const_cast<u64 *>(pa.b) + off, lds, as_global(p.fwd), row0, ctx, inv_n, &tin_b);
    __syncthreads();
    ProductSums<A> ps{elem(0), elem(0), elem(0), 0};
    const u64 FHE_GLOBAL *w8 = (const u64 FHE_GLOBAL *)k.wout8 + woff;
    const TwPtr wt = as_global(k.wout) + woff;
#pragma unroll
    for (int j = 0; j < PER; j++) {
        const int i = tid + j * NTT_THREADS;
        if (PAIRS % NTT_THREADS == 0 || i < PAIRS) {
            const u32 row = (u32)i / (FR::NPTS / 2), g = ((u32)i % (FR::NPTS / 2)) * 2;
            const u32 e = row * FR::NPTS + g;
            elem *dst = lds + row * FR::ROW_LDS + row_pad(g);
            if constexpr (A::PATH == PATH_F64) {
                ps.add(ra[j][0], dst[0], A::from_canonical(w8[e]), ctx);
                ps.add(ra[j][1], dst[1], A::from_canonical(w8[e + 1]), ctx);
                dst[0] = A::mulvar_lazy(ra[j][0], dst[0], ctx);
                dst[1] = A::mulvar_lazy(ra[j][1], dst[1], ctx);
            } else {
                ps.add(ra[j][0], dst[0], wt[e], ctx, p);
                ps.add(ra[j][1], dst[1], wt[e + 1], ctx, p);
                dst[0] = A::mulvar_lazy(ra[j][0], dst[0], p);
                dst[1] = A::mulvar_lazy(ra[j][1], dst[1], p);
            }
            if (__builtin_expect(fk >= 0, 0) && (u32)i == (u32)fk >> 1) {
                elem &x = dst[fk & 1];
                x = A::from_canonical((A::canonical(x, ctx) ^ ((u64)1 << k.fault_bit)) % p.q);
            }
        }
    }
    if constexpr (MP::TWO) inv_steps_tap<IR>(tid, pa.c + off, lds, as_global(p.inv), row0, ctx, inv_n, (NoTap *)nullptr);
    else inv_steps_tap<IR>(tid, pa.c + off, lds, as_global(p.inv), row0, ctx, inv_n, &tout_c);
    const size_t at = slot * FR::TILES + tile;
    block_sum_mod(A::canonical(ps.acc_a, ctx), p.q, k.s.aout + at, red[0]);
    block_sum_mod(A::canonical(ps.acc_b, ctx), p.q, k.s.bout + at, red[1]);
    block_sum_mod(A::canonical(ps.acc_ab, ctx), p.q, k.s.cin + at, red[2]);
    if constexpr (!MP::TWO) {
        block_sum_mod(A::canonical(tin_a.acc_in, ctx), p.q, k.s.ain + at, red[3]);
        block_sum_mod(A::canonical(tin_b.acc_in, ctx), p.q, k.s.bin + at, red[4]);
        block_sum_mod(A::canonical(tout_c.acc_out, ctx), p.q, k.s.cout + at, red[5]);
    }
}

template <class A, int LOGN>
static hipError_t launch_mid_checked(hipStream_t st, const PolymulChkArgs &k)
{
    constexpr int GEO = LOGN >= 13 ? 1 : 0;
    typedef typename MidPasses<A, LOGN, GEO>::Fwd FR;
    hipLaunchKernelGGL((k_polymul_mid_checked<A, LOGN, GEO>), dim3(k.a.units * FR::TILES), dim3(NTT_THREADS), 0, st, k);
    return hipGetLastError();
}

template <int LOGN> static void polymul_tiles_t(u32 *t_in, u32 *t_mid, u32 *t_out)
{
    constexpr int GEO = LOGN >= 13 ? 1 : 0;
    typedef MidPasses<ArithF64, LOGN, GEO> MP;
    *t_in = *t_mid = *t_out = MP::Fwd::TILES;
    if constexpr (MP::TWO) {
        *t_in = MP::F::Col::TILES;
        *t_out = MP::I::Col::TILES;
    }
}
void polymul_checked_tiles(int logn, u32 *t_in, u32 *t_mid, u32 *t_out)
{
    *t_in = *t_mid = *t_out = 1;
    switch (logn) {
#define FHE_CASE(L) case L: polymul_tiles_t<L>(t_in, t_mid, t_out); break;
        FHE_CASE(5) FHE_CASE(6) FHE_CASE(7) FHE_CASE(8) FHE_CASE(9) FHE_CASE(10) FHE_CASE(11) FHE_CASE(12) FHE_CASE(13)
        FHE_CASE(14) FHE_CASE(15) FHE_CASE(16) FHE_CASE(17) FHE_CASE(18) FHE_CASE(19) FHE_CASE(20)
#undef FHE_CASE
    default: break;
    }
}

hipError_t launch_polymul_checked(hipStream_t st, const PassArgs &a, u64 *b, u64 *c, int logn, int path, const PolymulChecks &k)
{
    if (a.units == 0) return hipSuccess;
    if (!polymul_fused_supported(logn) || a.map) return hipErrorInvalidValue;
    hipError_t e;
    PassArgs pb = a, pc = a;
    pb.data = b;
    pc.data = c;
    if (logn >= 13) {
        if ((e = launch_ntt_checked(st, a, k.win, k.wout, k.wout8, k.s.ain, nullptr, logn, path, 0)) != hipSuccess) return e;
        if (b != a.data && (e = launch_ntt_checked(st, pb, k.win, k.wout, k.wout8, k.s.bin, nullptr, logn, path, 0)) != hipSuccess) return e;
        if ((k.fault_point == 0 || k.fault_point == 1) && (e = launch_flip_bit(st, k.fault_at, 0, k.fault_bit)) != hipSuccess) return e;
    }
    const PolymulChkArgs pk{a, b, c, k.win, k.wout, k.wout8, logn / 2, k.s, k.fault_point == 2 ? k.fault_at : nullptr, k.fault_bit};
    switch (logn) {
#define FHE_CASE(L)                                                                                                  \
    case L:                                                                                                          \
        e = path == PATH_F64 ? launch_mid_checked<ArithF64, L>(st, pk) : launch_mid_checked<ArithU64, L>(st, pk);    \
        break;
        FHE_CASE(5) FHE_CASE(6) FHE_CASE(7) FHE_CASE(8) FHE_CASE(9) FHE_CASE(10) FHE_CASE(11) FHE_CASE(12) FHE_CASE(13)
        FHE_CASE(14) FHE_CASE(15) FHE_CASE(16) FHE_CASE(17) FHE_CASE(18) FHE_CASE(19) FHE_CASE(20)
#undef FHE_CASE
    default:
        return hipErrorInvalidValue;
    }
    if (e != hipSuccess) return e;
    if (logn >= 13) {
        if (k.fault_point == 3 && (e = launch_flip_bit(st, k.fault_at, 0, k.fault_bit)) != hipSuccess) return e;
        return launch_ntt_checked(st, pc, k.win, k.wout, k.wout8, nullptr, k.s.cout, logn, path, 1, true);
    }
    return hipSuccess;
}

}
```

Before: 2.824 million.

## Store forward NTT column-to-row hand-off in tiled layout and add optional LDS swizzle

```diff
diff --git a/fhe_reliability_gpu_amd/csrc/capi.cpp b/fhe_reliability_gpu_amd/csrc/capi.cpp
--- a/fhe_reliability_gpu_amd/csrc/capi.cpp
+++ b/fhe_reliability_gpu_amd/csrc/capi.cpp
@@ -63,6 +63,9 @@
     *out = t.release();
     return FHE_OK;
 }
+
+constexpr int NTT_HANDOFF_TILED_DEFAULT = 1;
+constexpr int NTT_LDS_SWIZZLE_DEFAULT = 0;
 
 SubBatchCut sub_batch_cut(const fhe_ctx *ctx, int log_n, size_t n_poly, size_t len, size_t bufs)
 {
@@ -246,6 +249,9 @@
             const bool want_pp = !galois && (ctx->pingpong < 0 ? cut.pc != 0 : ctx->pingpong != 0);
             const size_t pp_bytes = (cut.pc ? cut.pc * cut.lc : n_poly * limbs) * N * 8;
             if (want_pp && plain) HIP_TRY(handoff_scratch(ctx, st, pp_bytes, &pp));
+            const bool fwd_pair = plain && !inverse && ctx->geo == 1;
+            const bool tiled_on = fwd_pair && handoff_tiled_size(t->log_n) && (ctx->handoff_tiled < 0 ? NTT_HANDOFF_TILED_DEFAULT : ctx->handoff_tiled) != 0;
+            const bool swizzle_on = fwd_pair && lds_swizzle_size(t->log_n) && (ctx->lds_swizzle < 0 ? NTT_LDS_SWIZZLE_DEFAULT : ctx->lds_swizzle) != 0;
             if (cut.pc) {
                 const size_t npp = (n_poly + cut.pc - 1) / cut.pc, npl = (len + cut.lc - 1) / cut.lc;
                 return for_pieces(ctx, st, npp * npl, pp ? pp_bytes : 0, [&](hipStream_t s, size_t i, u64 *side_tmp) {
@@ -261,6 +267,8 @@
                     c.tmp = side_tmp ? side_tmp : pp;
                     c.tmp_stride = (u32)lc;
                     c.stream_hint = ctx->stream_hint != 0;
+                    if (tiled_on && c.tmp) c.fwd_opts |= FWD_HANDOFF_TILED;
+                    if (swizzle_on && c.stream_hint) c.fwd_opts |= FWD_LDS_SWIZZLE;
                     return launch_ntt(s, c, t->log_n, inverse, path, ctx->geo, -1, false);
                 });
             } else {
@@ -268,6 +276,7 @@
                 const bool streams = t->log_n < 13 && t->log_n >= 5 && ctx->stream_hint < 0 && ctx->only_pass < 0 &&
                                      (size_t)a.units * N * 8 > ((size_t)ctx->chunk_floor_mib << 20);
                 a.stream_hint = ctx->stream_hint > 0 || streams;
+                if (tiled_on && a.tmp) a.fwd_opts |= FWD_HANDOFF_TILED;
                 e = launch_ntt(st, a, t->log_n, inverse, path, ctx->geo, ctx->only_pass, ctx->resident);
             }
         }
@@ -423,6 +432,8 @@
     else if (!std::strcmp(name, "ntt_chunk_floor_mib")) ctx->chunk_floor_mib = (unsigned)std::max(0l, value);
     else if (!std::strcmp(name, "ntt_split")) ctx->split = value < 0 ? -1 : value ? 1 : 0;
     else if (!std::strcmp(name, "ntt_pingpong")) ctx->pingpong = value < 0 ? -1 : value ? 1 : 0;
+    else if (!std::strcmp(name, "ntt_handoff_tiled")) ctx->handoff_tiled = value < 0 ? -1 : value ? 1 : 0;
+    else if (!std::strcmp(name, "ntt_lds_swizzle")) ctx->lds_swizzle = value < 0 ? -1 : value ? 1 : 0;
     else if (!std::strcmp(name, "ntt_chunk_mib")) ctx->chunk_mib = (unsigned)std::max(0l, value);
     else if (!std::strcmp(name, "ks_fused")) ctx->ks_fused = value < 0 ? -1 : value ? 1 : 0;
     else if (!std::strcmp(name, "hmult_fused_rescale")) ctx->hmult_fused_rescale = value != 0;
diff --git a/fhe_reliability_gpu_amd/csrc/capi_internal.hpp b/fhe_reliability_gpu_amd/csrc/capi_internal.hpp
--- a/fhe_reliability_gpu_amd/csrc/capi_internal.hpp
+++ b/fhe_reliability_gpu_amd/csrc/capi_internal.hpp
@@ -116,6 +116,8 @@
     bool resident = false;
     int pingpong = -1;
     std::map<hipStream_t, std::unique_ptr<DevBuf>> pp_tmp;
+    int handoff_tiled = -1;
+    int lds_swizzle = -1;
     struct Side { hipStream_t s = nullptr; hipEvent_t fork = nullptr, join = nullptr; DevBuf tmp; };
     std::map<hipStream_t, std::unique_ptr<Side>> side;
     int split = -1;
diff --git a/fhe_reliability_gpu_amd/csrc/fourstep_checked.hip b/fhe_reliability_gpu_amd/csrc/fourstep_checked.hip
--- a/fhe_reliability_gpu_amd/csrc/fourstep_checked.hip
+++ b/fhe_reliability_gpu_amd/csrc/fourstep_checked.hip
@@ -139,6 +139,7 @@
                                  bool phases, int which)
 {
     if (a.units == 0) return hipSuccess;
+    if (!pass_args_plain(a)) return hipErrorInvalidValue;
     if (!a.src || a.map || a.limbs != 1 || !ntt_gs_supported(logn) || (phases && logn < 13)) return hipErrorInvalidValue;
     switch (logn) {
 #define FHE_CASE(L) \
diff --git a/fhe_reliability_gpu_amd/csrc/ntt_core.hpp b/fhe_reliability_gpu_amd/csrc/ntt_core.hpp
--- a/fhe_reliability_gpu_amd/csrc/ntt_core.hpp
+++ b/fhe_reliability_gpu_amd/csrc/ntt_core.hpp
@@ -258,8 +258,24 @@
     static constexpr bool STORES = false;
 };
 
+struct HandoffNatural {
+    static constexpr bool TILED = false;
+    FHE_HD static constexpr u32 at(u32 o) { return o; }
+};
+template <int LOGN, int PC, int TC> struct HandoffTiled {
+    static constexpr bool TILED = true;
+    static constexpr int PR = LOGN - PC;
+    static constexpr int LTC = TC == 1 ? 0 : TC == 2 ? 1 : TC == 4 ? 2 : TC == 8 ? 3 : TC == 16 ? 4 : TC == 32 ? 5 : TC == 64 ? 6 : -1;
+    static_assert(LTC >= 0 && LTC <= PR && PC > 0, "column tiles are a power of two of columns inside a row");
+    FHE_HD static constexpr u32 at(u32 o)
+    {
+        const u32 g = o >> PR, j = o & ((1u << PR) - 1u);
+        return ((j >> LTC) << (PC + LTC)) + (g << LTC) + (j & ((u32)TC - 1u));
+    }
+};
+
 template <class A, class ST, int LOGN, int S0, int TC, int NTHREADS, bool INVERSE, int IN_MODE, int OUT_MODE, u32 RED,
-          int SBLK, int COHERENT_IN = 0, bool STREAM = false>
+          int SBLK, int COHERENT_IN = 0, bool STREAM = false, bool SWZ = false>
 struct ColPass {
     typedef A Arith;
     typedef typename A::elem elem;
@@ -268,19 +284,28 @@
     static constexpr int NPTS = 1 << P;
     static constexpr int LOGSTRIDE = LOGN - S0 - P;
     static constexpr u32 STRIDE = 1u << LOGSTRIDE;
-    static constexpr int PADC = (TC < 32 && (NPTS * TC + ((NPTS + 15) / 16) * TC) * 8 <= 65536) ? TC : 0;
+    static constexpr int PADC = (!SWZ && TC < 32 && (NPTS * TC + ((NPTS + 15) / 16) * TC) * 8 <= 65536) ? TC : 0;
     static constexpr int LDS_ELEMS = NPTS * TC + ((NPTS + 15) / 16) * PADC;
     static constexpr int TCOLS = TC;
     static constexpr int NSTEP = ST::NSTEP;
     static constexpr int NPHASE = ST::NSTEP;
     static constexpr int TILES = (1 << (LOGN - P)) / TC;
-
-    static FHE_HD u32 lidx(u32 g, u32 col) { return g * TC + col + (g >> 4) * PADC; }
-
-    template <int E, class TAP = NoTap>
+    static constexpr int KL = ST::k(ST::NSTEP - 1);
+    static constexpr bool SWIZZLED = SWZ;
+    static_assert(!SWZ || (TC == 16 && KL >= 1 && P > KL), "the swizzle is derived for 16-column tiles (128-byte point rows)");
+    typedef HandoffTiled<LOGN, P, TC> Tiled;
+
+    static FHE_HD u32 lidx(u32 g, u32 col)
+    {
+        if (SWZ) return (g ^ ((g >> KL) & 1u)) * TC + col;
+        return g * TC + col + (g >> 4) * PADC;
+    }
+
+    template <int E, class TAP = NoTap, class HO = HandoffNatural>
     static FHE_D void phase(int tid, u64 *__restrict__ base, elem *__restrict__ lds, TwPtr tw, u32 hi_prefix,
-                            const typename A::Ctx &c, const Tw &inv_n, TAP *tap = nullptr, const u64 *src = nullptr)
-    {
+                            const typename A::Ctx &c, const Tw &inv_n, TAP *tap = nullptr, const u64 *src = nullptr, u32 tile = 0)
+    {
+        static_assert(!HO::TILED || (!INVERSE && S0 == 0 && !TAP::ACTIVE && OUT_MODE == IO_LAZY), "only the forward hand-off has a private layout");
         constexpr int F = INVERSE ? ST::NSTEP - 1 - E : E;
         constexpr int K = ST::k(F);
         constexpr int R = 1 << K;
@@ -341,7 +366,9 @@
                 }
 #pragma unroll
                 for (int r = 0; r < R; r++) {
-                    u64 *dst = base + (size_t)(g0 + ((u32)r << LOGS)) * STRIDE + col;
+                    u64 *dst;
+                    if constexpr (HO::TILED) dst = base + HO::at((g0 + ((u32)r << LOGS)) * STRIDE + tile * (u32)TC + col);
+                    else dst = base + (size_t)(g0 + ((u32)r << LOGS)) * STRIDE + col;
                     const u64 out = convert_out<A, OUT_MODE, INVERSE, FOLD>(x[r], c, inv_n);
                     if constexpr (TAP::ACTIVE && !TAP::STORES && OUT_MODE == IO_CANONICAL) tap->out((g0 + ((u32)r << LOGS)) * STRIDE + col, out, c);
                     if (STREAM && OUT_MODE == IO_CANONICAL) store_stream_u64(dst, out);
@@ -392,9 +419,17 @@
 }
 
 FHE_HD constexpr u32 row_pad(u32 g) { return g + ((g >> 4) << 1); }
+template <class T> struct alignas(16) LdsPair { T v[2]; };
+template <class T> FHE_HD void lds_load2(const T *p, T &a, T &b)
+{
+    const LdsPair<T> q = *reinterpret_cast<const LdsPair<T> *>(p);
+    a = q.v[0];
+    b = q.v[1];
+}
+template <class T> FHE_HD void lds_store2(T *p, const T &a, const T &b) { *reinterpret_cast<LdsPair<T> *>(p) = LdsPair<T>{{a, b}}; }
 
 template <class A, class ST, int LOGN, int TR, int NTHREADS, bool INVERSE, int IN_MODE, int OUT_MODE, u32 RED,
-          int SBLK, int COHERENT_IN = 0, bool STREAM = false, bool STAGE_BOTH = false, int ROWMODE = 0>
+          int SBLK, int COHERENT_IN = 0, bool STREAM = false, bool STAGE_BOTH = false, int ROWMODE = 0, bool SWZ = false>
 struct RowPass {
     typedef A Arith;
     typedef typename A::elem elem;
@@ -402,7 +437,7 @@
     static constexpr int P = ST::P;
     static constexpr int NPTS = 1 << P;
     static constexpr int S0 = LOGN - P;
-    static constexpr int ROW_LDS = NPTS + 2 * ((NPTS + 15) / 16);
+    static constexpr int ROW_LDS = SWZ ? NPTS : NPTS + 2 * ((NPTS + 15) / 16);
     static constexpr int LDS_ELEMS = ROW_LDS * TR;
     static constexpr int TROWS = TR;
     static constexpr int NSTEP = ST::NSTEP;
@@ -411,6 +446,16 @@
     static constexpr int NPHASE = ST::NSTEP + (STAGE_IN ? 1 : 0) + (STAGE_OUT ? 1 : 0);
     static constexpr int TILES = (1 << S0) / TR;
     static_assert(ROWMODE == 0 || (INVERSE && NPTS >= 32), "the gathering first launch belongs to the inverse-structured network");
+    static constexpr int KL = ST::k(ST::NSTEP - 1);
+    static constexpr bool SWIZZLED = SWZ;
+    static_assert(!SWZ || (!INVERSE && ROWMODE == 0 && !STAGE_BOTH && NPTS == 256 && KL == 4 && ST::NSTEP == 2),
+                  "the swizzle is derived for the forward pass on rows of 256 points in two radix-16 steps");
+
+    static FHE_HD constexpr u32 ridx(u32 g)
+    {
+        if (SWZ) return g ^ ((((g >> 4) & 7u) ^ ((g >> 7) & 1u)) << 1);
+        return row_pad(g);
+    }
 
     static FHE_HD u32 net_row(u32 row0, u32 row)
     {
@@ -425,7 +470,7 @@
             const u32 k = brev_bits(rho, P);
             const u64 *from = src + ((size_t)rho << S0) + row0 + ki;
             const u64 v = nt_src ? load_stream_u64(from) : *from;
-            lds[ki * ROW_LDS + row_pad(k)] = __builtin_bit_cast(elem, v);
+            lds[ki * ROW_LDS + ridx(k)] = __builtin_bit_cast(elem, v);
         }
     }
 
@@ -446,7 +491,7 @@
                 v0 = src[0];
                 v1 = src[1];
             }
-            elem *dst = lds + row * ROW_LDS + row_pad(g);
+            elem *dst = lds + row * ROW_LDS + ridx(g);
             dst[0] = __builtin_bit_cast(elem, v0);
             dst[1] = __builtin_bit_cast(elem, v1);
         }
@@ -457,7 +502,7 @@
         for (int i = tid; i < TR * NPTS; i += NTHREADS) {
             const u32 row = (u32)i / NPTS, g = (u32)i % NPTS;
             const u64 v = src_limb[galois_slot((row0 + row) * NPTS + g, LOGN, k)];
-            lds[row * ROW_LDS + row_pad(g)] = __builtin_bit_cast(elem, v);
+            lds[row * ROW_LDS + ridx(g)] = __builtin_bit_cast(elem, v);
             if (copy) copy[i] = v;
         }
     }
@@ -467,8 +512,21 @@
 #pragma unroll 2
         for (int i = tid; i < TR * NPTS / 2; i += NTHREADS) {
             const u32 row = (u32)i / (NPTS / 2), g = ((u32)i % (NPTS / 2)) * 2;
-            const elem *src = lds + row * ROW_LDS + row_pad(g);
+            const elem *src = lds + row * ROW_LDS + ridx(g);
             u64 *dst = base + (size_t)row * NPTS + g;
+            if constexpr (SWZ) {
+                static_assert(!SWZ || !TAP::ACTIVE, "observed passes keep the padded image");
+                elem e0, e1;
+                lds_load2(src, e0, e1);
+                if (STREAM && OUT_MODE == IO_CANONICAL) {
+                    store_stream_u64(dst, __builtin_bit_cast(u64, e0));
+                    store_stream_u64(dst + 1, __builtin_bit_cast(u64, e1));
+                } else {
+                    dst[0] = __builtin_bit_cast(u64, e0);
+                    dst[1] = __builtin_bit_cast(u64, e1);
+                }
+                continue;
+            }
             if constexpr (TAP::ACTIVE) {
                 if constexpr (TAP::STORES) {
                     tap->store(row * NPTS + g, __builtin_bit_cast(u64, src[0]), __builtin_bit_cast(u64, src[1]));
@@ -488,7 +546,7 @@
         }
     }
 
-    template <int E, class TAP = NoTap, class TWS = TwPtr>
+    template <int E, class TAP = NoTap, class TWS = TwPtr, class HO = HandoffNatural>
     static FHE_D void phase(int tid, u64 *__restrict__ base, elem *__restrict__ lds, const TWS &tw, u32 row0,
                             const typename A::Ctx &c, const Tw &inv_n, TAP *tap = nullptr, const u64 *src = nullptr, u32 galois = 0,
                             u64 *galois_copy = nullptr, bool nt_src = false)
@@ -512,6 +570,9 @@
             constexpr bool FROM_GLOBAL = FIRST && !STAGE_IN;
             constexpr bool TO_GLOBAL = LAST && !STAGE_OUT;
             constexpr int U0 = INVERSE ? (P - DONE - K) : DONE;
+            static_assert(!HO::TILED || (!INVERSE && ROWMODE == 0 && !STAGE_IN && !TAP::ACTIVE && IN_MODE == IO_LAZY),
+                          "only the forward hand-off has a private layout");
+            if constexpr (HO::TILED) static_assert(HO::PR == P, "the hand-off's rows are this pass's rows");
             FHE_ASSUME(tid >= 0 && tid < NTHREADS);
 #pragma unroll 1
             for (int u = tid; u < NSETS * TR; u += NTHREADS) {
@@ -526,10 +587,12 @@
 #pragma unroll
                     for (int r = 0; r < R; r++) {
                         if (FROM_GLOBAL) {
-                            const u64 *from = (src ? src + (size_t)row * NPTS : grow) + g0 + ((u32)r << LOGS);
+                            const u64 *from;
+                            if constexpr (HO::TILED) from = src + HO::at((row0 + row) * (u32)NPTS + g0 + ((u32)r << LOGS));
+                            else from = (src ? src + (size_t)row * NPTS : grow) + g0 + ((u32)r << LOGS);
                             raw[r] = COHERENT_IN == 1 ? load_coherent_u64(from) : (COHERENT_IN == 2 || (STREAM && IN_MODE == IO_CANONICAL)) ? load_stream_u64(from) : *from;
                         } else {
-                            raw[r] = __builtin_bit_cast(u64, lrow[row_pad(g0 + ((u32)r << LOGS))]);
+                            raw[r] = __builtin_bit_cast(u64, lrow[ridx(g0 + ((u32)r << LOGS))]);
                         }
                     }
                     convert_in<A, R, IN_MODE>(x, raw, c);
@@ -537,9 +600,12 @@
 #pragma unroll
                         for (int r = 0; r < R; r++) tap->in(row * NPTS + g0 + ((u32)r << LOGS), x[r], c);
                     }
+                } else if constexpr (SWZ && LOGS == 0) {
+#pragma unroll
+                    for (int r = 0; r < R; r += 2) lds_load2(lrow + ridx(g0 + (u32)r), x[r], x[r + 1]);
                 } else {
 #pragma unroll
-                    for (int r = 0; r < R; r++) x[r] = lrow[row_pad(g0 + ((u32)r << LOGS))];
+                    for (int r = 0; r < R; r++) x[r] = lrow[ridx(g0 + ((u32)r << LOGS))];
                 }
                 const u32 prefix = (net_row(row0, row) << DONE) | a;
                 constexpr bool FOLD = INVERSE && LAST && OUT_MODE == IO_CANONICAL && S0 + DONE == 0;
@@ -556,6 +622,12 @@
                             for (int r = 0; r < R; r++) tap->mid(row * NPTS + g0 + ((u32)r << LOGS), x[r], c);
                         }
                     }
+                    if constexpr (SWZ && LOGS == 0 && !TO_GLOBAL) {
+#pragma unroll
+                        for (int r = 0; r < R; r += 2)
+                            lds_store2(lrow + ridx(g0 + (u32)r), __builtin_bit_cast(elem, convert_out<A, OUT_MODE, INVERSE, FOLD>(x[r], c, inv_n)),
+                                       __builtin_bit_cast(elem, convert_out<A, OUT_MODE, INVERSE, FOLD>(x[r + 1], c, inv_n)));
+                    } else
 #pragma unroll
                     for (int r = 0; r < R; r++) {
                         const u64 out = convert_out<A, OUT_MODE, INVERSE, FOLD>(x[r], c, inv_n);
@@ -564,11 +636,11 @@
                             if (STREAM && OUT_MODE == IO_CANONICAL) store_stream_u64(grow + g0 + ((u32)r << LOGS), out);
                             else grow[g0 + ((u32)r << LOGS)] = out;
                         }
-                        else lrow[row_pad(g0 + ((u32)r << LOGS))] = __builtin_bit_cast(elem, out);
+                        else lrow[ridx(g0 + ((u32)r << LOGS))] = __builtin_bit_cast(elem, out);
                     }
                 } else {
 #pragma unroll
-                    for (int r = 0; r < R; r++) lrow[row_pad(g0 + ((u32)r << LOGS))] = x[r];
+                    for (int r = 0; r < R; r++) lrow[ridx(g0 + ((u32)r << LOGS))] = x[r];
                 }
             }
         }
diff --git a/fhe_reliability_gpu_amd/csrc/ntt_fused.hip b/fhe_reliability_gpu_amd/csrc/ntt_fused.hip
--- a/fhe_reliability_gpu_amd/csrc/ntt_fused.hip
+++ b/fhe_reliability_gpu_amd/csrc/ntt_fused.hip
@@ -217,6 +217,7 @@
                             int variant, u32 skip_teams)
 {
     if (a.units == 0) return hipSuccess;
+    if (!pass_args_plain(a)) return hipErrorInvalidValue;
     if (!fused_supported(logn) || dist < 1) return hipErrorInvalidValue;
     hipError_t e = hipMemsetAsync(ctl, 0, (size_t)fused_error_word() * sizeof(u32), st);
     if (e != hipSuccess) return e;
diff --git a/fhe_reliability_gpu_amd/csrc/ntt_kernels.hip b/fhe_reliability_gpu_amd/csrc/ntt_kernels.hip
--- a/fhe_reliability_gpu_amd/csrc/ntt_kernels.hip
+++ b/fhe_reliability_gpu_amd/csrc/ntt_kernels.hip
@@ -30,7 +30,7 @@
     return a.src + (base - a.data);
 }
 
-template <class PASS, int LOGN, bool INV, bool IS_COL>
+template <class PASS, int LOGN, bool INV, bool IS_COL, class HO = HandoffNatural>
 __global__ __launch_bounds__(NTT_THREADS) void k_ntt_pass(PassArgs a)
 {
     typedef typename PASS::Arith A;
@@ -45,6 +45,36 @@
     const Tw inv_n = p.inv_n;
     const int tid = threadIdx.x;
     const u64 *from = pass_source<PASS, LOGN, IS_COL>(a, base, row0);
+    if constexpr (HO::TILED) {
+        static_assert(!INV && PASS::NPHASE <= 4, "forward hand-off");
+        const u32 tile = blockIdx.x % PASS::TILES;
+        if constexpr (IS_COL) {
+            u64 *ubase = base - (size_t)tile * PASS_TCOLS<PASS, IS_COL>::value;
+            PASS::template phase<0, NoTap, HO>(tid, ubase, lds, tw, row0, ctx, inv_n, (NoTap *)nullptr, from, tile);
+            if constexpr (PASS::NPHASE > 1) {
+                __syncthreads();
+                PASS::template phase<1, NoTap, HO>(tid, ubase, lds, tw, row0, ctx, inv_n, (NoTap *)nullptr, from, tile);
+            }
+            if constexpr (PASS::NPHASE > 2) {
+                __syncthreads();
+                PASS::template phase<2, NoTap, HO>(tid, ubase, lds, tw, row0, ctx, inv_n, (NoTap *)nullptr, from, tile);
+            }
+        } else {
+            const u64 *ufrom = from - (size_t)row0 * PASS::NPTS;
+            PASS::template phase<0, NoTap, TwPtr, HO>(tid, base, lds, tw, row0, ctx, inv_n, (NoTap *)nullptr, ufrom);
+            __syncthreads();
+            PASS::template phase<1>(tid, base, lds, tw, row0, ctx, inv_n);
+            if constexpr (PASS::NPHASE > 2) {
+                __syncthreads();
+                PASS::template phase<2>(tid, base, lds, tw, row0, ctx, inv_n);
+            }
+            if constexpr (PASS::NPHASE > 3) {
+                __syncthreads();
+                PASS::template phase<3>(tid, base, lds, tw, row0, ctx, inv_n);
+            }
+        }
+        return;
+    }
     if constexpr (!IS_COL && INV) {
         PASS::template phase<0>(tid, base, lds, tw, row0, ctx, inv_n, (NoTap *)nullptr, from, a.galois, a.galois_copy ? a.galois_copy + (base - a.data) : nullptr);
     } else {
@@ -93,13 +123,21 @@
     }
 }
 
-template <class PASS, int LOGN, bool INV, bool IS_COL>
+template <class PASS, int LOGN, bool INV, bool IS_COL, class HO = HandoffNatural>
 static hipError_t launch_pass(hipStream_t st, const PassArgs &a)
 {
     const u32 blocks = a.units * PASS::TILES;
     static const u32 extra_lds = getenv("FHE_DBG_EXTRA_LDS") ? (u32)atoi(getenv("FHE_DBG_EXTRA_LDS")) : 0;
-    hipLaunchKernelGGL((k_ntt_pass<PASS, LOGN, INV, IS_COL>), dim3(blocks), dim3(NTT_THREADS), extra_lds, st, a);
+    hipLaunchKernelGGL((k_ntt_pass<PASS, LOGN, INV, IS_COL, HO>), dim3(blocks), dim3(NTT_THREADS), extra_lds, st, a);
     return hipGetLastError();
+}
+
+template <class CP, class RP, int LOGN, class TILED>
+static hipError_t launch_fwd_pair(hipStream_t st, const PassArgs &first, const PassArgs &second, bool tiled)
+{
+    const hipError_t e = tiled ? launch_pass<CP, LOGN, false, true, TILED>(st, first) : launch_pass<CP, LOGN, false, true>(st, first);
+    if (e != hipSuccess) return e;
+    return tiled ? launch_pass<RP, LOGN, false, false, TILED>(st, second) : launch_pass<RP, LOGN, false, false>(st, second);
 }
 
 template <class PASS, int LOGN>
@@ -221,6 +259,8 @@
     second.src = nullptr;
     second.galois = 0;
     second.galois_copy = nullptr;
+    first.fwd_opts = second.fwd_opts = 0;
+    bool tiled = false;
     if (a.tmp && which == -1) {
         if (!first.src) first.src = a.data;
         first.data = a.tmp;
@@ -229,6 +269,21 @@
             first.src_stride = a.poly_stride;
             first.poly_stride = a.tmp_stride;
             second.src_stride = a.tmp_stride;
+        }
+        tiled = (a.fwd_opts & FWD_HANDOFF_TILED) != 0;
+    } else if (a.fwd_opts & FWD_HANDOFF_TILED) return hipErrorInvalidValue;
+    constexpr bool FWD_PAIR = PS::G::TWO_PASS && !INV && GEO == 1;
+    if ((tiled && !(FWD_PAIR && handoff_tiled_size(LOGN))) ||
+        ((a.fwd_opts & FWD_LDS_SWIZZLE) && !(FWD_PAIR && lds_swizzle_size(LOGN) && a.stream_hint && which == -1)))
+        return hipErrorInvalidValue;
+    if constexpr (FWD_PAIR && handoff_tiled_size(LOGN)) {
+        if (a.fwd_opts && which == -1) {
+            if constexpr (lds_swizzle_size(LOGN)) {
+                if (a.fwd_opts & FWD_LDS_SWIZZLE)
+                    return launch_fwd_pair<typename PS::ColNtSw, typename PS::RowNtSw, LOGN, typename PS::Tiled>(st, first, second, tiled);
+            }
+            if (a.stream_hint) return launch_fwd_pair<typename PS::ColNt, typename PS::RowNt, LOGN, typename PS::Tiled>(st, first, second, tiled);
+            return launch_fwd_pair<typename PS::Col, typename PS::Row, LOGN, typename PS::Tiled>(st, first, second, tiled);
         }
     }
     if constexpr (!PS::G::TWO_PASS) {
@@ -294,6 +349,7 @@
 hipError_t launch_ntt_gs(hipStream_t st, const PassArgs &a, u64 *tmp, int logn, int path)
 {
     if (a.units == 0) return hipSuccess;
+    if (!pass_args_plain(a)) return hipErrorInvalidValue;
     if (!a.src || a.map || !ntt_gs_supported(logn)) return hipErrorInvalidValue;
     switch (logn) {
 #define FHE_CASE(L) \
@@ -507,6 +563,7 @@
 hipError_t launch_ntt_phases(hipStream_t st, const PassArgs &a, const PhaseArgs &p1, const PhaseArgs &p2, int logn, int path, int which)
 {
     if (a.units == 0) return hipSuccess;
+    if (!pass_args_plain(a)) return hipErrorInvalidValue;
     if (a.map || !ntt_phases_supported(logn)) return hipErrorInvalidValue;
     switch (logn) {
 #define FHE_CASE(L) \
@@ -548,6 +605,7 @@
                               int logn, int path, int which, bool inverse)
 {
     if (a.units == 0) return hipSuccess;
+    if (!pass_args_plain(a)) return hipErrorInvalidValue;
     if (a.map) return hipErrorInvalidValue;
     const AbftArgs ab{win, wout, wout8, logn / 2, sum_in, sum_out};
     switch (logn) {
@@ -652,6 +710,7 @@
 hipError_t launch_polymul(hipStream_t st, const PassArgs &a, u64 *b, u64 *c, int logn, int path)
 {
     if (a.units == 0) return hipSuccess;
+    if (!pass_args_plain(a)) return hipErrorInvalidValue;
     if (!polymul_fused_supported(logn)) return hipErrorInvalidValue;
     hipError_t e;
     PassArgs pb = a, pc = a;
@@ -869,6 +928,7 @@
 hipError_t launch_ntt_subscale(hipStream_t st, const PassArgs &a, const RowEpiArgs &ep, int logn, int path, const ColAddSrc *add_src)
 {
     if (a.units == 0) return hipSuccess;
+    if (!pass_args_plain(a)) return hipErrorInvalidValue;
     if (a.map || !ntt_subscale_supported(logn) || a.units / a.limbs > 3) return hipErrorInvalidValue;
     switch (logn) {
 #define FHE_CASE(L) \
@@ -1230,6 +1290,9 @@
         geo = 1;
         resident = false;
     }
+    if (a.fwd_opts && (inverse || which != -1 || a.scratch || resident || geo != 1 || a.galois || (a.fwd_opts & ~(FWD_HANDOFF_TILED | FWD_LDS_SWIZZLE)) ||
+                       ((a.fwd_opts & FWD_HANDOFF_TILED) && !a.tmp)))
+        return hipErrorInvalidValue;
     return path == PATH_F64 ? launch_size<ArithF64>(st, a, logn, inverse, geo, which, resident)
                             : launch_size<ArithU64>(st, a, logn, inverse, geo, which, resident);
 }
diff --git a/fhe_reliability_gpu_amd/csrc/ntt_plan.hpp b/fhe_reliability_gpu_amd/csrc/ntt_plan.hpp
--- a/fhe_reliability_gpu_amd/csrc/ntt_plan.hpp
+++ b/fhe_reliability_gpu_amd/csrc/ntt_plan.hpp
@@ -87,7 +87,13 @@
     u32 tmp_stride = 0;
     u32 galois = 0;
     u64 *galois_copy = nullptr;
-};
+    u32 fwd_opts = 0;
+};
+constexpr u32 FWD_HANDOFF_TILED = 1u;
+constexpr u32 FWD_LDS_SWIZZLE = 2u;
+inline bool pass_args_plain(const PassArgs &a) { return a.fwd_opts == 0; }
+constexpr bool handoff_tiled_size(int logn) { return logn >= 13 && logn <= 17; }
+constexpr bool lds_swizzle_size(int logn) { return logn == 16; }
 
 template <class A, int LOGN, bool INVERSE, int GEO = 0>
 struct Passes {
@@ -111,6 +117,11 @@
                     INVERSE ? IO_CANONICAL : IO_LAZY, INVERSE ? RED_SECOND : RED_FIRST, SB, 0, true> ColNt;
     typedef RowPass<A, typename PL::Row, LOGN, G::TR, NTT_THREADS, INVERSE, INVERSE ? IO_CANONICAL : IO_LAZY,
                     INVERSE ? IO_LAZY : IO_CANONICAL, INVERSE ? RED_FIRST : RED_SECOND, SB, 0, true> RowNt;
+    typedef ColPass<A, typename PL::Col, LOGN, 0, G::TC, NTT_THREADS, INVERSE, INVERSE ? IO_LAZY : IO_CANONICAL,
+                    INVERSE ? IO_CANONICAL : IO_LAZY, INVERSE ? RED_SECOND : RED_FIRST, SB, 0, true, true> ColNtSw;
+    typedef RowPass<A, typename PL::Row, LOGN, G::TR, NTT_THREADS, INVERSE, INVERSE ? IO_CANONICAL : IO_LAZY,
+                    INVERSE ? IO_LAZY : IO_CANONICAL, INVERSE ? RED_FIRST : RED_SECOND, SB, 0, true, false, 0, true> RowNtSw;
+    typedef HandoffTiled<LOGN, G::TWO_PASS ? G::PC : 1, G::TWO_PASS ? G::TC : 1> Tiled;
 };
 
 template <class A, int LOGN>
diff --git a/fhe_reliability_gpu_amd/csrc/polymul_checked.hip b/fhe_reliability_gpu_amd/csrc/polymul_checked.hip
--- a/fhe_reliability_gpu_amd/csrc/polymul_checked.hip
+++ b/fhe_reliability_gpu_amd/csrc/polymul_checked.hip
@@ -160,6 +160,7 @@
 hipError_t launch_polymul_checked(hipStream_t st, const PassArgs &a, u64 *b, u64 *c, int logn, int path, const PolymulChecks &k)
 {
     if (a.units == 0) return hipSuccess;
+    if (!pass_args_plain(a)) return hipErrorInvalidValue;
     if (!polymul_fused_supported(logn) || a.map) return hipErrorInvalidValue;
     hipError_t e;
     PassArgs pb = a, pc = a;
```

After: 2.835 million (median of 2 runs). No clear change (+0.4%).
